# tum-vision/tandem

Hardware: AMD Instinct MI355X
Metric: depth-maps/sec @ 640×480×7-view×3-stage; TSDF voxels integrated/sec (higher is better)
Workload: dtype f32; 1 GPU; 640x480 ref+6-src keyframe window, 3-stage cascade (48/32/8 hypotheses), view aggregation, fp32; independent windows, 4 in flight per GPU (one DrMvsnet engine each) x 1 GPU replica(s); trained weights recovered from the reference's exported tandem_512x320 model (same architecture), inputs resident in HBM; height=480, width=640, views=7, parallelism=replicas x1, 4 engines per GPU

## Files before the change

include/dr_mi355x.h:

```cpp
#ifndef DR_MI355X_H
#define DR_MI355X_H

#include <stddef.h>
#include <stdint.h>

#ifdef __cplusplus
extern "C" {
#endif

enum {
  DR_OK = 0,
  DR_ERR_ARG = 1,
  DR_ERR_PROTOCOL = 2,
  DR_ERR_DEVICE = 3,
  DR_ERR_IO = 4,
  DR_ERR_CAPACITY = 5,
  DR_ERR_UNSUPPORTED = 6
};

const char *dr_last_error(void);
const char *dr_version(void);

typedef struct drm_s drm_t;

int drm_create(const char *weights_path, int device, drm_t **out);
void drm_destroy(drm_t *h);
int drm_call_async(drm_t *h, int height, int width, int view_num, int ref_index,
                   const uint8_t *const *bgrs, const float *K9, const float *const *c2ws,
                   float depth_min, float depth_max, float discard_percentage);
int drm_ready(drm_t *h);
int drm_wait(drm_t *h);
int drm_get_result(drm_t *h, float *depth, float *confidence, float *depth_dense, float *confidence_dense);
int drm_get_result_view(drm_t *h, const float **depth, const float **confidence, const float **depth_dense, const float **confidence_dense);
void *drm_host_alloc(size_t bytes);
void drm_host_free(void *p);

int drm_set_feature_cache(drm_t *h, int capacity);
int drm_feature_cache_stats(drm_t *h, uint64_t out[6]);

int drm_upload(drm_t *h, int height, int width, int view_num, int ref_index, const uint8_t *const *bgrs,
               const float *K9, const float *const *c2ws, float depth_min, float depth_max,
               float discard_percentage);
int drm_forward(drm_t *h, int iters, float *ms_total);
int drm_autotune(drm_t *h, int max_candidates, float *before_ms, float *after_ms);
int drm_set_view_shard(drm_t *h, int nsrc_total);
int drm_forward_phase(drm_t *h, int phase);
int drm_comm_available(void);
int drm_comm_unique_id(uint8_t id[128]);
int drm_comm_init(drm_t *h, int rank, int world, const uint8_t id[128]);
int drm_comm_destroy(drm_t *h);
int drm_comm_count(drm_t *h, int *nranks);
int drm_device_tensor(drm_t *h, const char *name, void **dptr, size_t *nfloats);
int drm_download(drm_t *h, float *depth, float *confidence, float *depth_dense, float *confidence_dense);
int drm_get_stage_output(drm_t *h, int stage, float *depth, float *confidence);
int drm_get_tensor(drm_t *h, const char *name, float *out, size_t n_max, size_t *n, int dims[4]);
int drm_profile(drm_t *h, char *names, size_t names_cap, float *ms, int cap, int *count);
int drm_work(drm_t *h, double *flops, double *bytes);

int drm_debug_conv(int device, const float *in, int D, int H, int W, int Cin, const float *weight, int Cout,
                   int kd, int kh, int kw, int sd, int sh, int sw, int transposed, const float *scale,
                   const float *bias, int relu, const float *add, int add_up2, float *out, int out_dims[3]);

int drm_debug_tail(int device, const float *x, const float *skip, const float *w_deconv, const float *scale8, const float *bias8, const float *w_prob, int D,
                   int h, int w, int qy, int zchunk, int form, float *out);

typedef struct {
  float voxel_size;
  int num_buckets;
  int bucket_size;
  int num_blocks;
  int block_size;
  int max_sdf_weight;
  float truncation_distance;
  float max_sensor_depth;
  float min_sensor_depth;
  int num_render_streams;
  float fx, fy, cx, cy;
  int height, width;
} drf_options_t;

typedef struct drf_s drf_t;

int drf_create(const drf_options_t *opt, int device, drf_t **out);
void drf_destroy(drf_t *h);
int drf_integrate_scan_async(drf_t *h, const uint8_t *bgr, const float *depth, const float *pose16);
int drf_render_async(drf_t *h, const float *const *poses16, int n);
int drf_get_render_result(drf_t *h, uint8_t **bgr, float **depth, int n);
int drf_extract_mesh_async(drf_t *h, const float lower[3], const float upper[3]);
int drf_get_mesh_sync(drf_t *h, size_t num_max, size_t *num, float *vert, float *cols);
int drf_mesh_num_triangles(drf_t *h, size_t *ntri);
int drf_save_mesh(drf_t *h, const char *filename, const float lower[3], const float upper[3]);
int drf_get_render_device(drf_t *h, int stream, const uint8_t **d_bgr, const float **d_depth);
int drf_synchronize(drf_t *h);

int drf_stats(drf_t *h, uint64_t out[4]);
int drf_visited_blocks(drf_t *h, uint64_t *total);
int drf_export_blocks(drf_t *h, int max_blocks, int32_t *coords, uint8_t *voxels, int *n);
int drf_fast_div_status(drf_t *h, int *enabled, uint64_t *mismatches);
int drf_test_combine(drf_t *h, size_t n, const uint8_t *a, const uint8_t *b, int max_weight, uint8_t *out);
int drf_integrate_device(drf_t *h, const void *d_bgr, const void *d_depth, const float *pose16);
int dr_device_alloc(int device, size_t bytes, void **dptr);
int dr_device_free(void *dptr);
int dr_memcpy_h2d(void *dptr, const void *src, size_t bytes);
int dr_memcpy_d2h(void *dst, const void *dptr, size_t bytes);
int dr_memcpy_d2d(void *dst, const void *src, size_t bytes);
int drf_bench_integrate(drf_t *h, const void *d_bgr, const void *d_depth, const float *poses16, int nscans,
                        float *ms, float *kernel_ms);

int drf_bench_sequence(drf_t *h, const void *d_bgr, const void *d_depth, const float *poses16, int nframes, int render, float ms[6]);
int drf_bench_render_host(drf_t *h, int stream, int back, const uint8_t **bgr, const float **depth);

int drf_streaming_min_radius(const drf_options_t *o, float *radius);
int drf_set_streaming(drf_t *h, float radius, size_t host_capacity_blocks);
int drf_stream_out_region(drf_t *h, const float lower[3], const float upper[3]);
int drf_stream_in_region(drf_t *h, const float lower[3], const float upper[3]);
int drf_streaming_stats(drf_t *h, uint64_t out[6]);
int drf_export_host_blocks(drf_t *h, int max_blocks, int32_t *coords, uint8_t *voxels, int *n);
enum { DRF_MESH_RESIDENT = 0, DRF_MESH_MAP = 1 };
int drf_set_mesh_scope(drf_t *h, int scope);
enum { DRF_RENDER_RESIDENT = 0, DRF_RENDER_MAP = 1 };
int drf_set_render_scope(drf_t *h, int scope, size_t stage_capacity_blocks);
int drf_render_stats(drf_t *h, uint64_t out[4]);
int drf_mesh_stats(drf_t *h, uint64_t out[3]);

int drf_map_info(const char *path, float *voxel_size, uint64_t *n_blocks);
int drf_save_map(drf_t *h, const char *path, size_t chunk_blocks);
int drf_load_map(drf_t *h, const char *path, size_t chunk_blocks);

#define DRF_MESH_UPDATE_MAX_SCANS 16
int drf_extract_mesh_update_async(drf_t *h, const float lower[3], const float upper[3]);
int drf_mesh_update_size(drf_t *h, size_t *nblk, size_t *ntri, int *full);
int drf_get_mesh_update_sync(drf_t *h, size_t max_blocks, size_t num_max, size_t *nblk, int32_t *coords, uint64_t *first, size_t *num,
                             float *vert, float *cols, int *full);
int drf_mesh_update_reset(drf_t *h);
int drf_mesh_update_stats(drf_t *h, uint64_t out[4]);

typedef struct drt_s drt_t;
int drt_create(int w, int h, float setting_huberTH, float setting_coarseCutoffTH, int device, drt_t **out);
void drt_destroy(drt_t *t);
int drt_set_k(drt_t *t, int w, int h, float fx, float fy, float cx, float cy);
int drt_init(drt_t *t, int n_max);
int drt_set_reference(drt_t *t, int n, const float *pc_u, const float *pc_v, const float *pc_idepth, const float *pc_color,
                      float ref_exposure, const double ref_aff_g2l[2]);
int drt_set_new(drt_t *t, const float *dInew);
int drt_calc_res(drt_t *t, const double refToNew[16], float new_exposure, const double aff_g2l[2], float cutoffTH, double out6[6],
                 double sums7[7]);
int drt_calc_g(drt_t *t, double H_out[64], double b_out[8], float new_exposure, const double aff_g2l[2], double raw45[45]);
int drt_append_dense_reference(drt_t *t, const float *depth, const float KRKi[9], const float Kt[3], int step, int dense_only,
                               const float *idepth0, const float *dIp0, int on_device, int *n_out);
int drt_synchronize(drt_t *t);
int drt_start_timing(drt_t *t);
int drt_end_timing_ms(drt_t *t, float *ms);
int drt_get_points(drt_t *t, float *pc_u, float *pc_v, float *pc_idepth, float *pc_color, int cap, int *n);
int drt_get_warped(drt_t *t, int which, float *out, int cap);
int drt_get_zbuffer(drt_t *t, float *out);

#ifdef __cplusplus
}
#endif
#endif
```

tandem_amd/_lib.py:

```python
import ctypes as C
import os

_HERE = os.path.dirname(os.path.abspath(__file__))
LIB_PATH = os.environ.get("DR_MI355X_LIB") or os.path.join(_HERE, "libdr_mi355x.so")

DR_OK = 0
ERR_NAMES = {1: "DR_ERR_ARG", 2: "DR_ERR_PROTOCOL", 3: "DR_ERR_DEVICE", 4: "DR_ERR_IO", 5: "DR_ERR_CAPACITY",
             6: "DR_ERR_UNSUPPORTED"}


class DrError(RuntimeError):
    def __init__(self, code, msg):
        super().__init__("%s: %s" % (ERR_NAMES.get(code, code), msg))
        self.code = code


class FusionOptions(C.Structure):
    _fields_ = [("voxel_size", C.c_float), ("num_buckets", C.c_int), ("bucket_size", C.c_int),
                ("num_blocks", C.c_int), ("block_size", C.c_int), ("max_sdf_weight", C.c_int),
                ("truncation_distance", C.c_float), ("max_sensor_depth", C.c_float),
                ("min_sensor_depth", C.c_float), ("num_render_streams", C.c_int),
                ("fx", C.c_float), ("fy", C.c_float), ("cx", C.c_float), ("cy", C.c_float),
                ("height", C.c_int), ("width", C.c_int)]


_lib = None
u8p, f32p, vp = C.POINTER(C.c_uint8), C.POINTER(C.c_float), C.c_void_p
f64p = C.POINTER(C.c_double)

SIGNATURES = {
    "dr_last_error": (C.c_char_p, []),
    "dr_version": (C.c_char_p, []),
    "drm_create": (C.c_int, [C.c_char_p, C.c_int, C.POINTER(vp)]),
    "drm_destroy": (None, [vp]),
    "drm_call_async": (C.c_int, [vp, C.c_int, C.c_int, C.c_int, C.c_int, C.POINTER(u8p), f32p, C.POINTER(f32p),
                                 C.c_float, C.c_float, C.c_float]),
    "drm_ready": (C.c_int, [vp]),
    "drm_wait": (C.c_int, [vp]),
    "drm_get_result": (C.c_int, [vp, f32p, f32p, f32p, f32p]),
    "drm_get_result_view": (C.c_int, [vp, C.POINTER(f32p), C.POINTER(f32p), C.POINTER(f32p), C.POINTER(f32p)]),
    "drm_host_alloc": (vp, [C.c_size_t]),
    "drm_host_free": (None, [vp]),
    "drm_upload": (C.c_int, [vp, C.c_int, C.c_int, C.c_int, C.c_int, C.POINTER(u8p), f32p, C.POINTER(f32p),
                             C.c_float, C.c_float, C.c_float]),
    "drm_forward": (C.c_int, [vp, C.c_int, f32p]),
    "drm_download": (C.c_int, [vp, f32p, f32p, f32p, f32p]),
    "drm_get_stage_output": (C.c_int, [vp, C.c_int, f32p, f32p]),
    "drm_get_tensor": (C.c_int, [vp, C.c_char_p, f32p, C.c_size_t, C.POINTER(C.c_size_t), C.POINTER(C.c_int)]),
    "drm_profile": (C.c_int, [vp, C.c_char_p, C.c_size_t, f32p, C.c_int, C.POINTER(C.c_int)]),
    "drm_work": (C.c_int, [vp, C.POINTER(C.c_double), C.POINTER(C.c_double)]),
    "drm_debug_conv": (C.c_int, [C.c_int, f32p, C.c_int, C.c_int, C.c_int, C.c_int, f32p, C.c_int, C.c_int, C.c_int,
                                 C.c_int, C.c_int, C.c_int, C.c_int, C.c_int, f32p, f32p, C.c_int, f32p, C.c_int,
                                 f32p, C.POINTER(C.c_int)]),
    "drm_debug_tail": (C.c_int, [C.c_int, f32p, f32p, f32p, f32p, f32p, f32p, C.c_int, C.c_int, C.c_int, C.c_int, C.c_int, C.c_int, f32p]),
    "drm_autotune": (C.c_int, [vp, C.c_int, C.POINTER(C.c_float), C.POINTER(C.c_float)]),
    "drm_set_view_shard": (C.c_int, [vp, C.c_int]),
    "drm_forward_phase": (C.c_int, [vp, C.c_int]),
    "drm_comm_available": (C.c_int, []),
    "drm_comm_unique_id": (C.c_int, [u8p]),
    "drm_comm_init": (C.c_int, [vp, C.c_int, C.c_int, u8p]),
    "drm_comm_destroy": (C.c_int, [vp]),
    "drm_comm_count": (C.c_int, [vp, C.POINTER(C.c_int)]),
    "drm_device_tensor": (C.c_int, [vp, C.c_char_p, C.POINTER(vp), C.POINTER(C.c_size_t)]),
    "drf_create": (C.c_int, [C.POINTER(FusionOptions), C.c_int, C.POINTER(vp)]),
    "drf_destroy": (None, [vp]),
    "drf_integrate_scan_async": (C.c_int, [vp, u8p, f32p, f32p]),
    "drf_render_async": (C.c_int, [vp, C.POINTER(f32p), C.c_int]),
    "drf_get_render_result": (C.c_int, [vp, C.POINTER(u8p), C.POINTER(f32p), C.c_int]),
    "drf_extract_mesh_async": (C.c_int, [vp, f32p, f32p]),
    "drf_get_mesh_sync": (C.c_int, [vp, C.c_size_t, C.POINTER(C.c_size_t), f32p, f32p]),
    "drf_mesh_num_triangles": (C.c_int, [vp, C.POINTER(C.c_size_t)]),
    "drf_save_mesh": (C.c_int, [vp, C.c_char_p, f32p, f32p]),
    "drf_get_render_device": (C.c_int, [vp, C.c_int, C.POINTER(vp), C.POINTER(vp)]),
    "drf_synchronize": (C.c_int, [vp]),
    "drf_stats": (C.c_int, [vp, C.POINTER(C.c_uint64)]),
    "drf_export_blocks": (C.c_int, [vp, C.c_int, C.POINTER(C.c_int32), u8p, C.POINTER(C.c_int)]),
    "drf_fast_div_status": (C.c_int, [vp, C.POINTER(C.c_int), C.POINTER(C.c_uint64)]),
    "drf_test_combine": (C.c_int, [vp, C.c_size_t, u8p, u8p, C.c_int, u8p]),
    "drf_integrate_device": (C.c_int, [vp, vp, vp, f32p]),
    "drt_create": (C.c_int, [C.c_int, C.c_int, C.c_float, C.c_float, C.c_int, C.POINTER(vp)]),
    "drt_destroy": (None, [vp]),
    "drt_set_k": (C.c_int, [vp, C.c_int, C.c_int, C.c_float, C.c_float, C.c_float, C.c_float]),
    "drt_init": (C.c_int, [vp, C.c_int]),
    "drt_set_reference": (C.c_int, [vp, C.c_int, f32p, f32p, f32p, f32p, C.c_float, f64p]),
    "drt_set_new": (C.c_int, [vp, f32p]),
    "drt_calc_res": (C.c_int, [vp, f64p, C.c_float, f64p, C.c_float, f64p, f64p]),
    "drt_calc_g": (C.c_int, [vp, f64p, f64p, C.c_float, f64p, f64p]),
    "drt_append_dense_reference": (C.c_int, [vp, vp, f32p, f32p, C.c_int, C.c_int, vp, vp, C.c_int, C.POINTER(C.c_int)]),
    "drt_synchronize": (C.c_int, [vp]),
    "drt_start_timing": (C.c_int, [vp]),
    "drt_end_timing_ms": (C.c_int, [vp, C.POINTER(C.c_float)]),
    "drt_get_points": (C.c_int, [vp, f32p, f32p, f32p, f32p, C.c_int, C.POINTER(C.c_int)]),
    "drt_get_warped": (C.c_int, [vp, C.c_int, f32p, C.c_int]),
    "drt_get_zbuffer": (C.c_int, [vp, f32p]),
    "dr_device_alloc": (C.c_int, [C.c_int, C.c_size_t, C.POINTER(vp)]),
    "dr_device_free": (C.c_int, [vp]),
    "dr_memcpy_d2d": (C.c_int, [vp, vp, C.c_size_t]),
    "dr_memcpy_h2d": (C.c_int, [vp, vp, C.c_size_t]),
    "dr_memcpy_d2h": (C.c_int, [vp, vp, C.c_size_t]),
    "drm_set_feature_cache": (C.c_int, [vp, C.c_int]),
    "drm_feature_cache_stats": (C.c_int, [vp, C.POINTER(C.c_uint64)]),
    "drf_bench_sequence": (C.c_int, [vp, vp, vp, f32p, C.c_int, C.c_int, f32p]),
    "drf_visited_blocks": (C.c_int, [vp, C.POINTER(C.c_uint64)]),
    "drf_bench_render_host": (C.c_int, [vp, C.c_int, C.c_int, C.POINTER(vp), C.POINTER(vp)]),
    "drf_bench_integrate": (C.c_int, [vp, vp, vp, f32p, C.c_int, f32p, f32p]),
    "drf_streaming_min_radius": (C.c_int, [C.POINTER(FusionOptions), f32p]),
    "drf_set_streaming": (C.c_int, [vp, C.c_float, C.c_size_t]),
    "drf_stream_out_region": (C.c_int, [vp, f32p, f32p]),
    "drf_stream_in_region": (C.c_int, [vp, f32p, f32p]),
    "drf_streaming_stats": (C.c_int, [vp, C.POINTER(C.c_uint64)]),
    "drf_export_host_blocks": (C.c_int, [vp, C.c_int, C.POINTER(C.c_int32), u8p, C.POINTER(C.c_int)]),
    "drf_set_render_scope": (C.c_int, [vp, C.c_int, C.c_size_t]),
    "drf_render_stats": (C.c_int, [vp, C.POINTER(C.c_uint64)]),
    "drf_set_mesh_scope": (C.c_int, [vp, C.c_int]),
    "drf_mesh_stats": (C.c_int, [vp, C.POINTER(C.c_uint64)]),
    "drf_extract_mesh_update_async": (C.c_int, [vp, f32p, f32p]),
    "drf_mesh_update_size": (C.c_int, [vp, C.POINTER(C.c_size_t), C.POINTER(C.c_size_t), C.POINTER(C.c_int)]),
    "drf_get_mesh_update_sync": (C.c_int, [vp, C.c_size_t, C.c_size_t, C.POINTER(C.c_size_t), C.POINTER(C.c_int32), C.POINTER(C.c_uint64),
                                           C.POINTER(C.c_size_t), f32p, f32p, C.POINTER(C.c_int)]),
    "drf_mesh_update_reset": (C.c_int, [vp]),
    "drf_mesh_update_stats": (C.c_int, [vp, C.POINTER(C.c_uint64)]),
    "drf_map_info": (C.c_int, [C.c_char_p, f32p, C.POINTER(C.c_uint64)]),
    "drf_save_map": (C.c_int, [vp, C.c_char_p, C.c_size_t]),
    "drf_load_map": (C.c_int, [vp, C.c_char_p, C.c_size_t]),
}


HOOKS_LIB_PATH = os.path.join(_HERE, "libdr_mi355x_hooks.so")
_loaded = {}


def switch(path=None):
    global _lib, LIB_PATH
    LIB_PATH = path or os.environ.get("DR_MI355X_LIB") or os.path.join(_HERE, "libdr_mi355x.so")
    _lib = _loaded.get(LIB_PATH)


def lib():
    global _lib
    if _lib is None:
        if not os.path.isfile(LIB_PATH):
            raise ImportError("tandem_amd: %s not built -- run `python -c 'import __graft_entry__ as g; g.build()'` "
                              "(hipcc --offload-arch=gfx950). There is no CPU fallback." % LIB_PATH)
        L = C.CDLL(LIB_PATH, mode=C.RTLD_GLOBAL)
        for name, (res, args) in SIGNATURES.items():
            fn = getattr(L, name)
            fn.restype, fn.argtypes = res, args
        _lib = _loaded[LIB_PATH] = L
    return _lib


def check(code):
    if code != DR_OK:
        raise DrError(code, lib().dr_last_error().decode(errors="replace"))


def fptr(a):
    return a.ctypes.data_as(f32p)
```

tandem_amd/csrc/conv_mfma.h:

```cpp
#pragma once
#include <algorithm>
#include <atomic>
#include <functional>

#include "dr_common.h"

namespace dr {

typedef float floatx4 __attribute__((ext_vector_type(4)));

struct ConvClass {
  int NU;
  int tap_base;
  int w_base;
  int ooz, ooy, oox;
};

struct ConvArgs {
  const float *in;
  float *out;
  const float4 *wpk;
  const float *scale, *bias, *add;
  const int *tapoff;
  const ConvClass *cls;
  int inD, inH, inW, inC;
  int outD, outH, outW, outC;
  int nPD, nPH, nPW;
  int sz, sy, sx, pz, py, px;
  int omz, omy, omx;
  int TZ, TY, TXT, TZI, TYI, TXI;
  int npass, ctTot, rows_valid, relu, add_mode, addH, addW;
  int par_rows, par_map;
  unsigned magicX, magicY;
  int nuMax;
  int tilesD, tilesH, tilesW;
  const float *fz_x, *fz_w, *fz_b, *fz_coarse;
  int pass_stride;
  const float *zero16;
  int a_slots;
  int a_wbufs;
  int class_loop;
};

constexpr int kConvThreads = 256;
constexpr size_t kConvMaxLds = 160 * 1024;

template <int CT>
__device__ inline void conv_load_affine(const ConvArgs &a, int g, int ct0, float4 (&sc)[CT], float4 (&bi)[CT]) {
#pragma unroll
  for (int ct = 0; ct < CT; ++ct) {
    sc[ct] = *reinterpret_cast<const float4 *>(a.scale + (ct0 + ct) * 16 + 4 * g);
    bi[ct] = *reinterpret_cast<const float4 *>(a.bias + (ct0 + ct) * 16 + 4 * g);
  }
}
template <int CT, int PT, bool ADD = true>
__device__ inline void conv_epilogue(const ConvArgs &a, const ConvClass &cls, floatx4 (&acc)[CT][PT], const float4 (&scv)[CT], const float4 (&biv)[CT],
                                     int wave, int j, int g, int ct0, int pz0, int py0, int px0) {
#ifdef DR_EPILOGUE_PER_ENTRY
  constexpr int NE = CT * PT, GB = 1;
#else
  constexpr int NE = CT * PT, GB = NE < 4 ? NE : 4;
#endif
#pragma unroll
  for (int e0 = 0; e0 < NE; e0 += GB) {
    size_t obase[GB];
    float4 r[GB];
    bool ok[GB];
#pragma unroll
    for (int k = 0; k < GB; ++k) {
      const int e = e0 + k, pt = e / CT, ct = e - pt * CT;
      const int tau = wave * PT + pt;
      const int xt = tau % a.TXT, yt = (tau / a.TXT) % a.TY, zt = tau / (a.TXT * a.TY);
      const int qz = pz0 + zt, qy = py0 + yt, qx = px0 + xt * 16 + j;
      const int c0 = (ct0 + ct) * 16 + 4 * g;
      ok[k] = e < NE && qz < a.nPD && qy < a.nPH && qx < a.nPW && c0 < a.rows_valid;
      int oz = qz * a.omz + cls.ooz, oy = qy * a.omy + cls.ooy, ox = qx * a.omx + cls.oox, ch = c0;
      if (a.par_rows) {
        const int q = c0 / a.par_rows, bits = (a.par_map >> (3 * q)) & 7;
        ch = c0 - q * a.par_rows;
        oz += (bits >> 2) & 1; oy += (bits >> 1) & 1; ox += bits & 1;
      }
      obase[k] = (((size_t)oz * a.outH + oy) * a.outW + ox) * a.outC + ch;
      size_t abase = obase[k];
      if (a.add_mode == 2) abase = (((size_t)oz * a.addH + (oy >> 1)) * a.addW + (ox >> 1)) * a.outC + ch;
      r[k] = make_float4(0.f, 0.f, 0.f, 0.f);
      if (ADD && a.add_mode && ok[k]) r[k] = *reinterpret_cast<const float4 *>(a.add + abase);
    }
#pragma unroll
    for (int k = 0; k < GB; ++k) {
      const int e = e0 + k, pt = e / CT, ct = e - pt * CT;
      if (e >= NE || !ok[k]) continue;
      const float4 sc = scv[ct], bi = biv[ct];
      float4 v;
      v.x = acc[ct][pt][0] * sc.x + bi.x;
      v.y = acc[ct][pt][1] * sc.y + bi.y;
      v.z = acc[ct][pt][2] * sc.z + bi.z;
      v.w = acc[ct][pt][3] * sc.w + bi.w;
      if (a.relu) {
        v.x = fmaxf(v.x, 0.f); v.y = fmaxf(v.y, 0.f); v.z = fmaxf(v.z, 0.f); v.w = fmaxf(v.w, 0.f);
      }
      if (ADD && a.add_mode) { v.x += r[k].x; v.y += r[k].y; v.z += r[k].z; v.w += r[k].w; }
      *reinterpret_cast<float4 *>(a.out + obase[k]) = v;
    }
  }
}

template <int CT, int PT>
__device__ inline void conv_chunk_mfma(const float4 (&av)[CT], const float4 (&bv)[PT], floatx4 (&acc)[CT][PT]) {
#pragma unroll
  for (int ct = 0; ct < CT; ++ct)
#pragma unroll
    for (int pt = 0; pt < PT; ++pt) acc[ct][pt] = __builtin_amdgcn_mfma_f32_16x16x4f32(av[ct].x, bv[pt].x, acc[ct][pt], 0, 0, 0);
#pragma unroll
  for (int ct = 0; ct < CT; ++ct)
#pragma unroll
    for (int pt = 0; pt < PT; ++pt) acc[ct][pt] = __builtin_amdgcn_mfma_f32_16x16x4f32(av[ct].y, bv[pt].y, acc[ct][pt], 0, 0, 0);
#pragma unroll
  for (int ct = 0; ct < CT; ++ct)
#pragma unroll
    for (int pt = 0; pt < PT; ++pt) acc[ct][pt] = __builtin_amdgcn_mfma_f32_16x16x4f32(av[ct].z, bv[pt].z, acc[ct][pt], 0, 0, 0);
#pragma unroll
  for (int ct = 0; ct < CT; ++ct)
#pragma unroll
    for (int pt = 0; pt < PT; ++pt) acc[ct][pt] = __builtin_amdgcn_mfma_f32_16x16x4f32(av[ct].w, bv[pt].w, acc[ct][pt], 0, 0, 0);
}
template <int CT, int PT>
__device__ inline void conv_chunk_load(const float *lds, const float4 *wp, int toff, int u, const int (&base)[PT], float4 (&av)[CT],
                                       float4 (&bv)[PT]) {
#pragma unroll
  for (int ct = 0; ct < CT; ++ct) av[ct] = wp[(u * CT + ct) * 64];
#pragma unroll
  for (int pt = 0; pt < PT; ++pt) bv[pt] = *reinterpret_cast<const float4 *>(lds + base[pt] + toff);
}
template <int CT, int PT>
__device__ inline void conv_chunk_anchor(const float4 (&av)[CT], const float4 (&bv)[PT], int toff) {
#pragma unroll
  for (int ct = 0; ct < CT; ++ct) asm volatile("" ::"v"(av[ct].x), "v"(av[ct].y), "v"(av[ct].z), "v"(av[ct].w));
#pragma unroll
  for (int pt = 0; pt < PT; ++pt) asm volatile("" ::"v"(bv[pt].x), "v"(bv[pt].y), "v"(bv[pt].z), "v"(bv[pt].w));
  asm volatile("" ::"v"(toff));
}
template <int CT, int PT>
__device__ inline void conv_kloop(const float *lds, const float4 *wl, const int *tp, int TPC, int NU, int lane, const int (&base)[PT],
                                  floatx4 (&acc)[CT][PT]) {
  const float4 *wp = wl + lane;
  float4 a0[CT], b0[PT], a1[CT], b1[PT];
  int tA = tp[0], tB = tp[min(1, NU - 1) * TPC];
  conv_chunk_load<CT, PT>(lds, wp, tA, 0, base, a0, b0);
  int u = 0;
  for (; u + 1 < NU; u += 2) {
    conv_chunk_load<CT, PT>(lds, wp, tB, u + 1, base, a1, b1);
    tA = tp[min(u + 2, NU - 1) * TPC];
    __builtin_amdgcn_sched_barrier(0);
    conv_chunk_mfma<CT, PT>(a0, b0, acc);
    __builtin_amdgcn_sched_barrier(0);
    conv_chunk_anchor<CT, PT>(a1, b1, tA);
    conv_chunk_load<CT, PT>(lds, wp, tA, min(u + 2, NU - 1), base, a0, b0);
    tB = tp[min(u + 3, NU - 1) * TPC];
    __builtin_amdgcn_sched_barrier(0);
    conv_chunk_mfma<CT, PT>(a1, b1, acc);
    __builtin_amdgcn_sched_barrier(0);
    conv_chunk_anchor<CT, PT>(a0, b0, tB);
  }
  if (u < NU) conv_chunk_mfma<CT, PT>(a0, b0, acc);
}

template <int CT, int PT>
__device__ inline void conv_chunk_mfma2(const float4 (&av)[CT], const float4 (&bv)[PT], floatx4 (&acc)[CT][PT], floatx4 (&acc2)[CT][PT]) {
  if constexpr (CT * PT == 1) {
    acc[0][0] = __builtin_amdgcn_mfma_f32_16x16x4f32(av[0].x, bv[0].x, acc[0][0], 0, 0, 0);
    acc2[0][0] = __builtin_amdgcn_mfma_f32_16x16x4f32(av[0].y, bv[0].y, acc2[0][0], 0, 0, 0);
    acc[0][0] = __builtin_amdgcn_mfma_f32_16x16x4f32(av[0].z, bv[0].z, acc[0][0], 0, 0, 0);
    acc2[0][0] = __builtin_amdgcn_mfma_f32_16x16x4f32(av[0].w, bv[0].w, acc2[0][0], 0, 0, 0);
  } else conv_chunk_mfma<CT, PT>(av, bv, acc);
}
template <int CT, int PT, class Load>
__device__ inline void conv_kloop_narrow(const int *tp, int TPC, int NU, floatx4 (&acc)[CT][PT], Load load) {
  float4 a0[CT], b0[PT], a1[CT], b1[PT], a2[CT], b2[PT];
  floatx4 acc2[CT][PT];
#pragma unroll
  for (int ct = 0; ct < CT; ++ct)
#pragma unroll
    for (int pt = 0; pt < PT; ++pt) acc2[ct][pt] = floatx4{0.f, 0.f, 0.f, 0.f};
  auto tap = [&](int u) { return tp[min(u, NU - 1) * TPC]; };
  int t0 = tap(0), t1 = tap(1), t2 = tap(2);
  load(t0, 0, a0, b0);
  load(t1, min(1, NU - 1), a1, b1);
  int u = 0;
  for (; u + 2 < NU; u += 3) {
    load(t2, u + 2, a2, b2);
    t0 = tap(u + 3);
    __builtin_amdgcn_sched_barrier(0);
    conv_chunk_mfma2<CT, PT>(a0, b0, acc, acc2);
    __builtin_amdgcn_sched_barrier(0);
// ... 391 lines not shown
    conv_a_load<CI, CT, PT>(tile, wp, tB, u + 1, c4, bpos, a1, b1);
    tA = tp[min(u + 2, NU - 1) * TPC];
    __builtin_amdgcn_sched_barrier(0);
    conv_chunk_mfma<CT, PT>(a0, b0, acc);
    __builtin_amdgcn_sched_barrier(0);
    conv_chunk_anchor<CT, PT>(a1, b1, tA);
    conv_a_load<CI, CT, PT>(tile, wp, tA, min(u + 2, NU - 1), c4, bpos, a0, b0);
    tB = tp[min(u + 3, NU - 1) * TPC];
    __builtin_amdgcn_sched_barrier(0);
    conv_chunk_mfma<CT, PT>(a1, b1, acc);
    __builtin_amdgcn_sched_barrier(0);
    conv_chunk_anchor<CT, PT>(a0, b0, tB);
  }
  if (u < NU) conv_chunk_mfma<CT, PT>(a0, b0, acc);
}

template <int CI, int CT, int PT>
__global__ __launch_bounds__(kConvAThreads) void k_conv_a(const ConvArgs a) {
  extern __shared__ float4 lds4[];
  constexpr int TPC = 16 / CI;
  const int tid = threadIdx.x, lane = tid & 63, wave = __builtin_amdgcn_readfirstlane(tid >> 6), j = lane & 15, g = lane >> 4;
  const ConvClass cls = a.cls[0];
  const int ct0 = blockIdx.z * CT;
  const int NP = a.TZI * a.TYI * a.TXI, NU = cls.NU, n_w = NU * CT * 64;

  float4 *tile0 = lds4, *tile1 = lds4 + a.a_slots;
  float4 *wb0 = lds4 + 2 * (size_t)a.a_slots;
  int *tapl = reinterpret_cast<int *>(wb0 + (size_t)a.a_wbufs * n_w);
  for (int i = tid; i < NU * TPC; i += kConvAThreads) tapl[i] = a.tapoff[cls.tap_base + i];
  const int *tp = tapl + (4 * g) / CI;
  const int c4 = ((4 * g) % CI) / 4;

  int bpos[PT];
#pragma unroll
  for (int pt = 0; pt < PT; ++pt) {
    const int tau = wave * PT + pt;
    const int xt = tau % a.TXT, yt = (tau / a.TXT) % a.TY, zt = tau / (a.TXT * a.TY);
    bpos[pt] = ((zt * a.sz) * a.TYI + yt * a.sy) * a.TXI + (xt * 16 + j) * a.sx;
  }

  const int ntiles = a.tilesD * a.tilesH * a.tilesW, per_xcd = (ntiles + 7) >> 3;
  const int xcd = blockIdx.x & 7, wi = blockIdx.x >> 3, nw = gridDim.x >> 3;
  const int t_lo = xcd * per_xcd, t_hi = min(ntiles, t_lo + per_xcd);
  const int my_tiles = t_lo + wi < t_hi ? (t_hi - t_lo - wi + nw - 1) / nw : 0;
  const int n_units = my_tiles * a.npass;
  auto tile_origin = [&](int k, int &pz0, int &py0, int &px0) {
    int b = t_lo + wi + k * nw;
    const int tw = b % a.tilesW;
    b /= a.tilesW;
    pz0 = (b / a.tilesH) * a.TZ; py0 = (b % a.tilesH) * a.TY; px0 = tw * a.TXT * 16;
  };
  auto issue = [&](int unit) {
    const int k = unit / a.npass, p = unit - k * a.npass;
    int pz0, py0, px0;
    tile_origin(k, pz0, py0, px0);
    conv_a_issue<CI, CT>(a, (unit & 1) ? tile1 : tile0, wb0 + (size_t)(p % a.a_wbufs) * n_w, unit < a.npass || a.npass > a.a_wbufs, NP, NU, p, ct0, cls.w_base,
                         pz0 * a.sz - a.pz, py0 * a.sy - a.py, px0 * a.sx - a.px, wave, lane);
  };

  floatx4 acc[CT][PT];
#pragma unroll
  for (int ct = 0; ct < CT; ++ct)
#pragma unroll
    for (int pt = 0; pt < PT; ++pt) acc[ct][pt] = floatx4{0.f, 0.f, 0.f, 0.f};

  float4 scv[CT], biv[CT];
  conv_load_affine<CT>(a, g, ct0, scv, biv);
  if (n_units > 0) issue(0);
  int done_tile = -1;
  for (int i = 0; i < n_units; ++i) {
    conv_a_wait_dma();
    __syncthreads();
#ifndef DR_ABL_NO_STAGE
#ifndef DR_CONV_A_ISSUE_LATE
    const bool early = a.add_mode == 0;
#else
    const bool early = false;
#endif
    if (early && i + 1 < n_units) issue(i + 1);
#endif
#ifdef DR_ABL_NO_EPI
    if (done_tile >= 0 && a.npass < 0) {
#else
    if (done_tile >= 0) {
#endif
      int pz0, py0, px0;
      tile_origin(done_tile, pz0, py0, px0);
      if (a.add_mode) conv_epilogue<CT, PT, true>(a, cls, acc, scv, biv, wave, j, g, ct0, pz0, py0, px0);
      else conv_epilogue<CT, PT, false>(a, cls, acc, scv, biv, wave, j, g, ct0, pz0, py0, px0);
#pragma unroll
      for (int ct = 0; ct < CT; ++ct)
#pragma unroll
        for (int pt = 0; pt < PT; ++pt) acc[ct][pt] = floatx4{0.f, 0.f, 0.f, 0.f};
      done_tile = -1;
    }
#ifndef DR_ABL_NO_STAGE
    if (!early && i + 1 < n_units) issue(i + 1);
#endif
#ifndef DR_ABL_NO_KLOOP
#ifdef DR_NO_NARROW_KLOOP
    if constexpr (false) {
#else
    if constexpr (CT * PT <= 2) {
#endif
      const float4 *tile = (i & 1) ? tile1 : tile0, *wp = wb0 + (size_t)((i % a.npass) % a.a_wbufs) * n_w + lane;
      conv_kloop_narrow<CT, PT>(tp, TPC, NU, acc, [&](int toff, int u, float4 (&av)[CT], float4 (&bv)[PT]) { conv_a_load<CI, CT, PT>(tile, wp, toff, u, c4, bpos, av, bv); });
    } else conv_a_kloop<CI, CT, PT>((i & 1) ? tile1 : tile0, wb0 + (size_t)((i % a.npass) % a.a_wbufs) * n_w, tp, TPC, NU, lane, c4, bpos, acc);
#endif
    if ((i + 1) % a.npass == 0) done_tile = i / a.npass;
  }
  if (done_tile >= 0) {
    int pz0, py0, px0;
    tile_origin(done_tile, pz0, py0, px0);
    conv_epilogue<CT, PT>(a, cls, acc, scv, biv, wave, j, g, ct0, pz0, py0, px0);
  }
}

}
#include "conv_wino.h"
namespace dr {
template <int CI> __host__ __device__ inline int conv_a_unit(int pos, int c4);
}
#include "conv_march.h"
namespace dr {


enum ConvMode { CONV_NORMAL = 0, CONV_XPAIR = 1, CONV_X8 = 2 };

struct ConvLayer {
  int Cin = 0, Cout = 0;
  int kd = 1, kh = 1, kw = 1;
  int sd = 1, sh = 1, sw = 1;
  bool transposed = false;
  int up2 = 0;
  const float *weight = nullptr;
  std::vector<float> scale, bias;
  bool relu = false;
  int out_pad = 0;
};

struct ConvFuse {
  const float *x, *w, *b, *coarse;
  int cin;
};

struct ConvLaunch {
  ConvArgs args;
  int ci, ct, pt, fz = 0;
  int async = 0;
  MarchArgs march{};
  int nup = 0;
  int ncw = 8;
  int bf3 = 0;
  dim3 grid;
  size_t lds_bytes;
  double flops;
};

struct DimTaps {
  std::vector<int> t, off;
  int s = 1, p = 0, om = 1, oo = 0, npos = 0;
  int par = -1;
};

inline int parity_kernel_index(int parity, int off) {
  if (parity == 0) return off == 0 ? 1 : -1;
  return off == 0 ? 2 : 0;
}
inline std::vector<DimTaps> axis_classes_up2(int in_size, bool split) {
  std::vector<DimTaps> r;
  if (!split) { DimTaps d; d.t = {0, 1, 2}; d.off = {0, 1, 2}; d.p = 1; d.om = 2; d.npos = in_size; r.push_back(d); return r; }
  DimTaps e; e.t = {0, 1}; e.off = {0, 1}; e.p = 1; e.om = 2; e.oo = 0; e.npos = in_size; e.par = 0; r.push_back(e);
  DimTaps o; o.t = {1, 2}; o.off = {1, 2}; o.p = 1; o.om = 2; o.oo = 1; o.npos = in_size; o.par = 1; r.push_back(o);
  return r;
}
inline int up2_kernel_set(int parity, int off, int (&k)[2]) {
  if (parity == 0) { if (off == 0) { k[0] = 0; return 1; } if (off == 1) { k[0] = 1; k[1] = 2; return 2; } return 0; }
  if (off == 1) { k[0] = 0; k[1] = 1; return 2; }
  if (off == 2) { k[0] = 2; return 1; }
  return 0;
}
inline void prune_taps(DimTaps &d, int in_size) {
  std::vector<int> t, off;
  for (size_t i = 0; i < d.t.size(); ++i) {
    bool used = false;
    for (int pos = 0; pos < d.npos && !used; ++pos) { const int x = pos * d.s - d.p + d.off[i]; used = x >= 0 && x < in_size; }
    if (used) { t.push_back(d.t[i]); off.push_back(d.off[i]); }
  }
  if (t.empty() || t.size() == d.t.size()) return;
  const int mo = *std::min_element(off.begin(), off.end());
  for (int &o : off) o -= mo;
  d.p -= mo;
  d.t = t; d.off = off;
}
inline std::vector<DimTaps> axis_classes_unpruned(int k, int s, bool transposed, int in_size, bool split);
inline std::vector<DimTaps> axis_classes(int k, int s, bool transposed, int in_size, bool split = false, bool prune = false) {
  std::vector<DimTaps> r = axis_classes_unpruned(k, s, transposed, in_size, split);
  if (prune && !hook_env("DR_CONV_NO_TAP_PRUNE"))
    for (DimTaps &d : r) prune_taps(d, in_size);
  return r;
}
inline std::vector<DimTaps> axis_classes_unpruned(int k, int s, bool transposed, int in_size, bool split) {
  std::vector<DimTaps> r;
  if (!transposed) {
    DimTaps d;
    for (int t = 0; t < k; ++t) { d.t.push_back(t); d.off.push_back(t); }
    d.s = s; d.p = k / 2; d.npos = (in_size + 2 * (k / 2) - k) / s + 1;
    r.push_back(d);
  } else if (k == 1) {
    DimTaps d; d.t = {0}; d.off = {0}; d.npos = in_size; r.push_back(d);
  } else if (s == 1) {
    DimTaps d;
    for (int t = 0; t < k; ++t) { d.t.push_back(t); d.off.push_back(2 - t); }
    d.p = 1; d.npos = in_size;
    r.push_back(d);
  } else if (!split) {
    DimTaps d; d.t = {0, 1}; d.off = {0, 1}; d.om = 2; d.oo = 0; d.npos = in_size; r.push_back(d);
  } else {
    DimTaps e; e.t = {0}; e.off = {0}; e.om = 2; e.oo = 0; e.npos = in_size; e.par = 0; r.push_back(e);
    DimTaps o; o.t = {0, 1}; o.off = {0, 1}; o.om = 2; o.oo = 1; o.npos = in_size; o.par = 1; r.push_back(o);
  }
  return r;
}

struct ConvPlanOut {
  std::vector<ConvLaunch> launches;
  int outD, outH, outW;
  int ncand = 0;
};

struct DeviceArena {
  std::vector<void *> ptrs;
  int *err_flag = nullptr;
  bool host_only = false;
  template <class T>
  T *upload(const std::vector<T> &h) {
    if (host_only) {
      T *d = static_cast<T *>(malloc(std::max<size_t>(h.size() * sizeof(T), 16)));
      memcpy(d, h.data(), h.size() * sizeof(T));
      ptrs.push_back(d);
      return d;
    }
    T *d = dalloc<T>(h.size());
    DR_HIP(hipMemcpy(d, h.data(), h.size() * sizeof(T), hipMemcpyHostToDevice));
    ptrs.push_back(d);
    return d;
  }
  ~DeviceArena() { for (void *p : ptrs) { if (host_only) free(p); else (void)hipFree(p); } }
};

struct ConvTuned {
  int Cin, Cout, kd, kh, kw, sd, sh, sw, transposed, mode, inD, inH, inW;
  int ci, ct, pt, tz, ty, txt;
  int async_;
};
#include "conv_tuned.h"

inline bool conv_instance_exists(int ci, int ct) {
  return (ci == 4 && ct == 1) || ((ci == 8 || ci == 16) && (ct == 1 || ct == 2 || ct == 4));
}
inline bool conv_a_instance_exists(int ci, int ct, int pt) {
  return (pt == 1 || pt == 2 || pt == 4) && ((ci == 4 && ct == 1 && pt != 1) || ((ci == 8 || ci == 16) && (ct == 1 || ct == 2)));
}
#define DR_MARCH_INSTANCES(X)                                                                                         \
  X(8, 6, 1, 2, 8) X(8, 6, 1, 4, 8) X(8, 6, 1, 1, 12) X(8, 6, 1, 2, 12)                                               \
  X(16, 12, 1, 2, 8) X(16, 12, 1, 4, 8) X(16, 12, 1, 1, 12) X(16, 12, 1, 2, 12)                                       \
  X(16, 9, 1, 2, 8) X(16, 9, 1, 4, 8) X(16, 9, 1, 1, 12) X(16, 9, 1, 2, 12) X(16, 9, 2, 2, 8)                         \
  X(8, 2, 1, 1, 8) X(8, 2, 1, 2, 8) X(8, 2, 1, 4, 8) X(8, 2, 1, 1, 10) X(8, 2, 1, 2, 10)                              \
  X(16, 4, 1, 1, 8) X(16, 4, 1, 2, 8) X(16, 4, 1, 4, 8) X(16, 4, 1, 1, 10) X(16, 4, 1, 2, 10)                         \
  X(16, 3, 1, 1, 8) X(16, 3, 1, 2, 8) X(16, 3, 1, 4, 8) X(16, 3, 1, 1, 10) X(16, 3, 1, 2, 10)                         \
  X(16, 3, 2, 1, 8) X(16, 3, 2, 2, 8) X(16, 3, 2, 1, 10) X(16, 3, 2, 2, 10)
#define DR_MARCH_W_INSTANCES(X) X(8, 6, 1, 1, 8) X(16, 12, 1, 1, 8) X(16, 9, 1, 1, 8)
inline bool conv_m_instance_exists(int ci, int nup, int ct, int pt, int ncw, bool wino = false) {
#define DR_X(CI_, NUP_, CT_, PT_, NCW_) if (ci == CI_ && nup == NUP_ && ct == CT_ && pt == PT_ && ncw == NCW_) return true;
  if (wino) { DR_MARCH_W_INSTANCES(DR_X) return false; }
  DR_MARCH_INSTANCES(DR_X)
#undef DR_X
  return false;
}
inline int conv_march_policy() {
  if (const char *e = getenv("DR_CONV_MARCH")) return atoi(e);
  return 1;
}
inline int conv_rowmarch_policy() {
  if (const char *e = getenv("DR_CONV_ROWMARCH")) return atoi(e);
  return 1;
}
struct MarchShape {
  int nup, npi, npo, ns, tyi, txi, np, ps, r, ncw;
  size_t wbytes, lds_bytes;
  long long steps;
  int grid;
  bool ok;
};
inline MarchShape march_shape(int KZ, int ntp, int Cin, int ci, int ct, int pt, int ty, int txt, int SX, int exy, int exx, int nPD, int nPH, int nPW, int CTtot,
                              bool rm = false, bool wino = false) {
  MarchShape m{};
  const int tpc = 16 / ci;
  if (Cin % ci || ntp % tpc || CTtot % ct || (ty * txt) % pt || (rm && (ty != 1 || KZ != 1)) || (wino && (KZ != 3 || rm || (ntp / 3) % tpc))) return m;
  m.ncw = ty * txt / pt;
  m.nup = ntp / tpc;
  if (!conv_m_instance_exists(ci, m.nup, ct, pt, m.ncw, wino)) return m;
  const int npass = Cin / ci, kz = rm ? 3 : KZ;
  if (npass > 2) return m;
  m.npi = KZ == 1 ? npass : 1; m.npo = KZ == 1 ? 1 : npass; m.ns = kz * m.npi;
  m.tyi = rm ? 1 : (wino ? 2 * ty + 2 : ty - 1 + exy); m.txi = (txt * 16 - 1) * SX + exx; m.np = m.tyi * m.txi;
// ... 401 lines not shown
          if (kx >= 0 && kx < L.kw) v = weight_at(co, cin, tz[tap], ky >= 0 ? ky : ty[tap], kx);
        }
      }
      return v;
    };
    pk.resize(w0 + (size_t)npass * NU * CTtot * 64 * 4 * (bf3 ? 2 : 1), 0.f);
    if (bf3) {
      unsigned short *pb = reinterpret_cast<unsigned short *>(pk.data() + w0);
      for (int p = 0; p < npass; ++p) for (int u = 0; u < NU; ++u) for (int ct = 0; ct < CTtot; ++ct)
        for (int l = 0; l < 64; ++l) for (int s = 0; s < 8; ++s) {
          const int g = l >> 4, i = l & 15, k32 = 8 * g + s;
          const float v = weight_of(u * TPC + k32 / CI, p * CI + k32 % CI, ct * 16 + i);
          const unsigned short hi = bf16_rne(v), lo = bf16_rne(v - bf16_value(hi));
          const size_t frag = (((size_t)p * NU + u) * CTtot + ct) * 2;
          pb[((frag + 0) * 64 + l) * 8 + s] = hi;
          pb[((frag + 1) * 64 + l) * 8 + s] = lo;
        }
    } else if (wino_raw) {
      for (int p = 0; p < npass; ++p) for (int u = 0; u < NR; ++u) for (int k = 0; k < 3; ++k) for (int ct = 0; ct < CTtot; ++ct)
        for (int l = 0; l < 64; ++l) for (int s = 0; s < 4; ++s) {
          const int g = l >> 4, i = l & 15, k16 = 4 * g + s;
          pk[w0 + ((((size_t)p * NU + u * 3 + k) * CTtot + ct) * 64 + l) * 4 + s] = (k == 1 ? 0.5f : 1.f) * weight_of(u * TPC + k16 / CI, p * CI + k16 % CI, ct * 16 + i, k);
        }
    } else if (wino) {
      for (int p = 0; p < npass; ++p) for (int u = 0; u < NR; ++u) for (int pp = 0; pp < 4; ++pp) for (int ct = 0; ct < CTtot; ++ct)
        for (int l = 0; l < 64; ++l) for (int s = 0; s < 4; ++s) {
          const int g = l >> 4, i = l & 15, k16 = 4 * g + s;
          double v = 0;
          for (int ky = 0; ky < 3; ++ky) v += conv_wino_g(pp, ky) * (double)weight_of(u * TPC + k16 / CI, p * CI + k16 % CI, ct * 16 + i, ky);
          pk[w0 + ((((size_t)p * NU + u * 4 + pp) * CTtot + ct) * 64 + l) * 4 + s] = (float)v;
        }
    } else
    for (int p = 0; p < npass; ++p) for (int u = 0; u < NU; ++u) for (int ct = 0; ct < CTtot; ++ct)
      for (int l = 0; l < 64; ++l) for (int s = 0; s < 4; ++s) {
        const int g = l >> 4, i = l & 15, k16 = 4 * g + s;
        pk[w0 + ((((size_t)p * NU + u) * CTtot + ct) * 64 + l) * 4 + s] = weight_of(u * TPC + k16 / CI, p * CI + k16 % CI, ct * 16 + i);
      }
    if (L.up2) flops += ic == 0 ? 2.0 * nPD * nPH * nPW * 16.0 * L.Cin * L.Cout : 0.0;
    else if (L.transposed) flops += ic == 0 ? 2.0 * nPD * nPH * nPW * (double)L.kd * L.kh * L.kw * L.Cin * L.Cout : 0.0;
    else flops += 2.0 * nPD * (wino ? 2 * nPH : nPH) * nPW * (mode == CONV_NORMAL ? 1 : shifts) * (double)ntz * (wino ? 3 : nty) * (mode == CONV_NORMAL ? ntx : L.kw) * L.Cin * L.Cout;
  }

  ConvLaunch cl{};
  ConvArgs &a = cl.args;
  a.in = in; a.out = out; a.wpk = reinterpret_cast<const float4 *>(arena.upload(pk));
  a.scale = arena.upload(sc); a.bias = arena.upload(bi); a.add = add; a.tapoff = arena.upload(tapoff);
  a.cls = arena.upload(cls);
  a.inD = inD; a.inH = inH; a.inW = inW; a.inC = in_split ? in_split : inC;
  a.pass_stride = in_split ? (int)((size_t)inD * inH * inW * in_split) : CI;
  if (in_split && (size_t)inD * inH * inW * in_split >= (1ull << 31)) fail(DR_ERR_ARG, "plan_conv: split input too large");
  a.outD = R.outD; a.outH = R.outH + 2 * L.out_pad; a.outW = outWv; a.outC = outCv;
  if (L.out_pad) {
    if ((2 * L.out_pad) % shifts) fail(DR_ERR_ARG, "plan_conv: an output border of %d pixels does not fit the %d-wide output groups", L.out_pad, shifts);
    a.outW = outWv + 2 * L.out_pad / shifts;
  }
  a.nPD = nPD; a.nPH = nPH; a.nPW = nPW;
  a.sz = SZ; a.sy = SY; a.sx = SX; a.pz = PZ; a.py = PY; a.px = PX;
  a.omz = cz[0].om; a.omy = cy[0].om; a.omx = cx[0].om;
  a.par_rows = parity_layer ? L.Cout : 0; a.par_map = par_map;
  a.TZ = TZ; a.TY = TY; a.TXT = TXT; a.TZI = TZI; a.TYI = TYI; a.TXI = TXI;
  a.magicX = TXI == 1 ? 0u : (unsigned)((0x100000000ull + TXI - 1) / TXI);
  a.magicY = TYI == 1 ? 0u : (unsigned)((0x100000000ull + TYI - 1) / TYI);
  if ((size_t)TZI * TYI * TXI >= 65536) fail(DR_ERR_ARG, "plan_conv: halo tile too large");
  a.npass = npass; a.ctTot = CTtot; a.rows_valid = rows_valid; a.relu = L.relu ? 1 : 0;
  a.add_mode = add ? add_mode : 0;
  a.addH = R.outH / 2; a.addW = (mode == CONV_NORMAL ? R.outW : outWv) / 2;
  a.tilesD = cdiv(nPD, TZ); a.tilesH = cdiv(nPH, TY); a.tilesW = cdiv(nPW, TXT * 16);
  cl.ci = CI; cl.ct = CT; cl.pt = PT;
  a.fz_x = a.fz_w = a.fz_b = a.fz_coarse = nullptr;
  if (fz) {
    if (fz->cin != 8 || L.transposed || SZ != 1 || SY != 1) fail(DR_ERR_ARG, "plan_conv: fused skip needs an 8-channel source and a stride-1 layer");
    a.fz_x = fz->x; a.fz_w = fz->w; a.fz_b = fz->b; a.fz_coarse = fz->coarse; cl.fz = fz->cin;
  }
  cl.grid = dim3(8 * cdiv(a.tilesD * a.tilesH * a.tilesW, 8), ncls, CTtot / CT);
  int nu_max = 0;
  for (auto &c : cls) nu_max = std::max(nu_max, c.NU);
  a.nuMax = nu_max;
  cl.lds_bytes = (size_t)TZI * TYI * TXI * CIS * 4 + (size_t)nu_max * CT * (bf3 ? 2048 : 1024) + (size_t)nu_max * TPC * 4 + 64;
  cl.bf3 = bf3 ? 1 : 0;
  a.zero16 = nullptr; a.a_slots = 0; a.a_wbufs = 1; a.class_loop = 0;
  if (ASYNC == 0 && !bf3 && !fz && ncls > 1 && npass == 1 && conv_c_instance_exists(CI, CT, PT) && !hook_env("DR_CONV_NO_CLASS_LOOP")) {
    const size_t with_loop = cl.lds_bytes + (size_t)nu_max * CT * 1024 + (size_t)(ncls - 1) * nu_max * TPC * 4;
    if (with_loop <= kConvMaxLds) {
      a.class_loop = ncls;
      cl.lds_bytes = with_loop;
      cl.grid.y = 1;
    }
  }
  if (ASYNC == 0 && !bf3 && !fz && PT == 1 && CT <= 2 && npass >= 2 && (size_t)TZI * TYI * TXI * (CI / 4) <= 6 * kConvThreads && !hook_env("DR_CONV_NO_PIPE") &&
      cl.lds_bytes + (size_t)nu_max * CT * 1024 <= kConvMaxLds) {
    a.a_wbufs = 2;
    cl.lds_bytes += (size_t)nu_max * CT * 1024;
  }
  if (ASYNC == 4) cl.async = 4;
  if (ASYNC == 1) {
    cl.async = 1;
    a.zero16 = arena.upload(std::vector<float>(4, 0.f));
    a.a_slots = (int)conv_a_slots(TZI * TYI * TXI, CI);
    a.a_wbufs = npass;
    cl.lds_bytes = 2 * (size_t)a.a_slots * 16 + (size_t)a.a_wbufs * nu_max * CT * 1024 + (size_t)nu_max * TPC * 4 + 64;
    if (cl.lds_bytes > kConvMaxLds) {
      a.a_wbufs = std::min(npass, 2);
      cl.lds_bytes = 2 * (size_t)a.a_slots * 16 + (size_t)a.a_wbufs * nu_max * CT * 1024 + (size_t)nu_max * TPC * 4 + 64;
    }
    const int ntiles = a.tilesD * a.tilesH * a.tilesW, split = CTtot / CT;
    const int wpc = cl.lds_bytes * 2 <= kConvMaxLds ? 2 : 1;
    const int want = std::max(1, std::min(ntiles, 256 * wpc / split));
    cl.grid = dim3(8 * cdiv(want, 8), 1, split);
  }
  if (ASYNC == 2 || ASYNC == 3 || ASYNC == 5) {
    const bool rm = ASYNC == 3;
    const MarchShape ms = rm ? march_shape(L.kd, row_ntp, L.Cin, CI, CT, PT, 1, TXT, SX, exy, exx, nPD, nPH, nPW, CTtot, true)
                             : march_shape(L.kd, march_ntp, L.Cin, CI, CT, PT, TY, TXT, SX, exy, exx, nPD, nPH, nPW, CTtot, false, wino_raw);
    if (!ms.ok) fail(DR_ERR_ARG, "plan_conv: inconsistent k_conv_m plan");
    cl.async = 2; cl.nup = ms.nup; cl.ncw = ms.ncw;
    a.zero16 = arena.upload(std::vector<float>(4, 0.f));
    a.a_slots = 0; a.a_wbufs = 0;
    MarchArgs &m = cl.march;
    const int kz = rm ? 3 : L.kd;
    std::vector<int> tap2d((size_t)ms.nup * TPC, 0);
    {
      const DimTaps &Y = *classes[0].y, &X = *classes[0].x;
      int n = 0;
      if (rm) for (size_t ix = 0; ix < X.t.size(); ++ix, ++n) tap2d[n] = X.off[ix];
      else for (size_t iy = 0; iy < Y.t.size(); ++iy) for (size_t ix = 0; ix < X.t.size(); ++ix, ++n) tap2d[n] = Y.off[iy] * TXI + X.off[ix];
    }
    m.tap2d = arena.upload(tap2d);
    m.geo.KZ = kz; m.geo.NPI = ms.npi; m.geo.Dc = rm ? nPH : (L.kd == 3 ? nPD : 1);
    m.NPO = ms.npo;
    m.colsH = rm ? 1 : cdiv(nPH, TY); m.colsW = cdiv(nPW, TXT * 16);
    m.ncols = (L.kd == 3 ? 1 : nPD) * m.colsH * m.colsW;
    m.R = ms.r; m.PS = ms.ps; m.NP = ms.np; m.nit = ms.ps / 128;
    m.wsec = ms.nup * CT * 64; m.NU = kz * ms.nup;
    m.steps = (int)ms.steps;
    m.ncw = ms.ncw;
    m.rm = rm ? 1 : 0;
    m.wino = wino_raw ? 1 : 0;
    const long long iplane = (long long)a.inH * a.inW * a.inC, oplane = (long long)a.outH * a.outW * a.outC;
    if (iplane * std::max(1, a.inD) >= (1ll << 31) || oplane * std::max(1, a.outD) >= (1ll << 31)) fail(DR_ERR_ARG, "plan_conv: tensor too large for k_conv_m's 32-bit strides");
    m.i_sv = L.kd == 3 ? 0 : (int)iplane; m.i_sz = rm ? a.inW * a.inC : (L.kd == 3 ? (int)iplane : 0); m.i_sy = rm ? 0 : a.inW * a.inC;
    m.o_sv = L.kd == 3 ? 0 : (int)oplane; m.o_sz = rm ? a.outW * a.outC : (L.kd == 3 ? (int)oplane : 0); m.o_sy = rm ? 0 : a.outW * a.outC;
    m.inHp = rm ? 1 : a.inH;
    m.err = arena.err_flag;
    m.depth = rm ? 3 : 2;
    if (const char *e = hook_env("DR_MARCH_PDEPTH")) m.depth = std::max(1, std::min(4, atoi(e)));
    cl.lds_bytes = ms.lds_bytes;
    cl.grid = dim3(ms.grid, 1, CTtot / CT);
  }
  cl.flops = flops;
  R.launches.push_back(cl);
  return R;
}

inline void conv_allow_big_lds(const void *fn, std::atomic<unsigned long long> &done, size_t lds_bytes) {
  if (lds_bytes <= 64 * 1024) return;
  int dev = 0;
  DR_HIP(hipGetDevice(&dev));
  const unsigned long long bit = 1ull << (dev & 63);
  if (done.load(std::memory_order_acquire) & bit) return;
  DR_HIP(hipFuncSetAttribute(fn, hipFuncAttributeMaxDynamicSharedMemorySize, (int)kConvMaxLds));
  done.fetch_or(bit, std::memory_order_release);
}
template <int CI, int CT, int PT, int FZ = 0>
inline void launch_conv_inst(const ConvLaunch &c, hipStream_t st) {
  static std::atomic<unsigned long long> done{0};
  conv_allow_big_lds(reinterpret_cast<const void *>(&k_conv<CI, CT, PT, FZ>), done, c.lds_bytes);
  hipLaunchKernelGGL((k_conv<CI, CT, PT, FZ>), c.grid, dim3(kConvThreads), c.lds_bytes, st, c.args);
}
#ifdef DR_PARITY_HOOKS
template <int CI, int CT, int PT>
inline void launch_conv_b_inst(const ConvLaunch &c, hipStream_t st) {
  static std::atomic<unsigned long long> done{0};
  conv_allow_big_lds(reinterpret_cast<const void *>(&k_conv_b<CI, CT, PT>), done, c.lds_bytes);
  hipLaunchKernelGGL((k_conv_b<CI, CT, PT>), c.grid, dim3(kConvThreads), c.lds_bytes, st, c.args);
}
#endif
template <int CI, int CT, int PT>
inline void launch_conv_c_inst(const ConvLaunch &c, hipStream_t st) {
  static std::atomic<unsigned long long> done{0};
  conv_allow_big_lds(reinterpret_cast<const void *>(&k_conv_c<CI, CT, PT>), done, c.lds_bytes);
  hipLaunchKernelGGL((k_conv_c<CI, CT, PT>), c.grid, dim3(kConvThreads), c.lds_bytes, st, c.args);
}
template <int CI, int CT, int PT>
inline void launch_conv_a_inst(const ConvLaunch &c, hipStream_t st) {
  static std::atomic<unsigned long long> done{0};
  conv_allow_big_lds(reinterpret_cast<const void *>(&k_conv_a<CI, CT, PT>), done, c.lds_bytes);
  hipLaunchKernelGGL((k_conv_a<CI, CT, PT>), c.grid, dim3(kConvAThreads), c.lds_bytes, st, c.args);
}
template <int CI, int CT, int PT>
inline void launch_conv_w_inst(const ConvLaunch &c, hipStream_t st) {
  static std::atomic<unsigned long long> done{0};
  conv_allow_big_lds(reinterpret_cast<const void *>(&k_conv_w<CI, CT, PT>), done, c.lds_bytes);
  hipLaunchKernelGGL((k_conv_w<CI, CT, PT>), c.grid, dim3(kConvThreads), c.lds_bytes, st, c.args);
}
template <int CI, int NUP, int CT, int PT, int FZ = 0, int NCW = 8, int W = 0>
inline void launch_conv_m_inst(const ConvLaunch &c, hipStream_t st) {
  static std::atomic<unsigned long long> done{0};
  conv_allow_big_lds(reinterpret_cast<const void *>(&k_conv_m<CI, NUP, CT, PT, FZ, NCW, W>), done, c.lds_bytes);
  hipLaunchKernelGGL((k_conv_m<CI, NUP, CT, PT, FZ, NCW, W>), c.grid, dim3(64 * (NCW + (FZ ? kMarchFzProducers : kMarchProducers))), c.lds_bytes, st, c.args, c.march);
}
inline void launch_conv(const ConvLaunch &c, hipStream_t st) {
#ifndef DR_PARITY_HOOKS
  if (c.bf3) fail(DR_ERR_UNSUPPORTED, "launch_conv: the bf16 x 3 kernel is built with -DDR_PARITY_HOOKS only");
#else
  if (c.bf3) {
#define DR_CONV_B_CASE(CI_, CT_)                                                \
  if (c.ci == CI_ && c.ct == CT_ && !c.async && !c.fz) {                        \
    if (c.pt == 4) launch_conv_b_inst<CI_, CT_, 4>(c, st);                      \
    else launch_conv_b_inst<CI_, CT_, 1>(c, st);                                \
    return;                                                                     \
  }
    DR_CONV_B_CASE(8, 1)
    DR_CONV_B_CASE(8, 2)
    DR_CONV_B_CASE(8, 4)
    DR_CONV_B_CASE(16, 1)
    DR_CONV_B_CASE(16, 2)
    DR_CONV_B_CASE(16, 4)
#undef DR_CONV_B_CASE
    fail(DR_ERR_ARG, "launch_conv: no bf16x3 instance CI=%d CT=%d", c.ci, c.ct);
  }
#endif
#ifndef DR_PARITY_HOOKS
  if (c.fz) fail(DR_ERR_UNSUPPORTED, "launch_conv: fused-skip kernels are built with -DDR_PARITY_HOOKS only");
#else
  if (c.async == 2 && c.fz) {
    if (c.fz != 8 || c.ci != 16 || c.nup != 12 || c.ct != 1 || c.ncw != 8) fail(DR_ERR_ARG, "launch_conv: no fused-skip marching instance FZ=%d CI=%d NUP=%d CT=%d", c.fz, c.ci, c.nup, c.ct);
    if (c.pt == 4) launch_conv_m_inst<16, 12, 1, 4, 8>(c, st);
    else launch_conv_m_inst<16, 12, 1, 2, 8>(c, st);
    return;
  }
#endif
  if (c.async == 2 && c.march.wino) {
#define DR_X(CI_, NUP_, CT_, PT_, NCW_) \
  if (c.ci == CI_ && c.nup == NUP_ && c.ct == CT_ && c.pt == PT_ && c.ncw == NCW_) { launch_conv_m_inst<CI_, NUP_, CT_, PT_, 0, NCW_, 1>(c, st); return; }
    DR_MARCH_W_INSTANCES(DR_X)
#undef DR_X
    fail(DR_ERR_ARG, "launch_conv: no Winograd marching instance CI=%d NUP=%d CT=%d PT=%d waves=%d", c.ci, c.nup, c.ct, c.pt, c.ncw);
  }
  if (c.async == 2) {
#define DR_X(CI_, NUP_, CT_, PT_, NCW_) \
  if (c.ci == CI_ && c.nup == NUP_ && c.ct == CT_ && c.pt == PT_ && c.ncw == NCW_) { launch_conv_m_inst<CI_, NUP_, CT_, PT_, 0, NCW_>(c, st); return; }
    DR_MARCH_INSTANCES(DR_X)
#undef DR_X
    fail(DR_ERR_ARG, "launch_conv: no marching instance CI=%d NUP=%d CT=%d PT=%d waves=%d", c.ci, c.nup, c.ct, c.pt, c.ncw);
  }
  if (c.async == 4) {
#define DR_CONV_W_CASE(CI_, CT_, PT_) if (c.ci == CI_ && c.ct == CT_ && c.pt == PT_) { launch_conv_w_inst<CI_, CT_, PT_>(c, st); return; }
    DR_CONV_W_CASE(16, 1, 1) DR_CONV_W_CASE(16, 1, 2) DR_CONV_W_CASE(16, 2, 1) DR_CONV_W_CASE(16, 2, 2)
    DR_CONV_W_CASE(8, 1, 1) DR_CONV_W_CASE(8, 1, 2)
#undef DR_CONV_W_CASE
    fail(DR_ERR_ARG, "launch_conv: no Winograd instance CI=%d CT=%d PT=%d", c.ci, c.ct, c.pt);
  }
  if (c.async) {
#define DR_CONV_A_CASE(CI_, CT_)                                                \
  if (c.ci == CI_ && c.ct == CT_) {                                             \
    if (c.pt == 4) launch_conv_a_inst<CI_, CT_, 4>(c, st);                      \
    else if (c.pt == 2) launch_conv_a_inst<CI_, CT_, 2>(c, st);                 \
    else launch_conv_a_inst<CI_, CT_, 1>(c, st);                                \
    return;                                                                     \
  }
    if (c.ci == 4 && c.ct == 1 && c.pt == 1) fail(DR_ERR_ARG, "launch_conv: no async instance CI=4 PT=1");
    DR_CONV_A_CASE(4, 1)
    DR_CONV_A_CASE(8, 1)
    DR_CONV_A_CASE(8, 2)
    DR_CONV_A_CASE(16, 1)
    DR_CONV_A_CASE(16, 2)
#undef DR_CONV_A_CASE
    fail(DR_ERR_ARG, "launch_conv: no async instance CI=%d CT=%d PT=%d", c.ci, c.ct, c.pt);
  }
#ifdef DR_PARITY_HOOKS
  if (c.fz) {
    if (c.fz != 8 || c.ci != 16 || c.ct != 1) fail(DR_ERR_ARG, "launch_conv: no fused-skip instance FZ=%d CI=%d CT=%d", c.fz, c.ci, c.ct);
    if (c.pt == 4) launch_conv_inst<16, 1, 4, 8>(c, st);
    else launch_conv_inst<16, 1, 1, 8>(c, st);
    return;
  }
#endif
  if (c.args.class_loop > 0) {
#define DR_CONV_C_CASE(CI_, CT_)                                                \
  if (c.ci == CI_ && c.ct == CT_) {                                             \
    if (c.pt == 4) launch_conv_c_inst<CI_, CT_, 4>(c, st);                      \
    else launch_conv_c_inst<CI_, CT_, 1>(c, st);                                \
    return;                                                                     \
  }
    DR_CONV_C_CASE(8, 1)
    DR_CONV_C_CASE(8, 2)
    DR_CONV_C_CASE(16, 1)
    DR_CONV_C_CASE(16, 2)
#undef DR_CONV_C_CASE
    fail(DR_ERR_ARG, "launch_conv: no class-loop instance CI=%d CT=%d PT=%d", c.ci, c.ct, c.pt);
  }
#define DR_CONV_CASE(CI_, CT_)                                                  \
  if (c.ci == CI_ && c.ct == CT_) {                                             \
    if (c.pt == 4) launch_conv_inst<CI_, CT_, 4>(c, st);                        \
    else launch_conv_inst<CI_, CT_, 1>(c, st);                                  \
    return;                                                                     \
  }
  DR_CONV_CASE(4, 1)
  DR_CONV_CASE(8, 1)
  DR_CONV_CASE(8, 2)
  DR_CONV_CASE(8, 4)
  DR_CONV_CASE(16, 1)
  DR_CONV_CASE(16, 2)
  DR_CONV_CASE(16, 4)
#undef DR_CONV_CASE
  fail(DR_ERR_ARG, "launch_conv: no instance CI=%d CT=%d", c.ci, c.ct);
}

}
```

tandem_amd/csrc/conv_wino.h:

```cpp
#pragma once

namespace dr {

template <int CT, int PT>
__device__ inline void conv_w_load(const float *lds, const float4 *wp, int toff, int r, const int (&base)[PT], int rs, float4 (&av)[4][CT], float4 (&dv)[4][PT]) {
#pragma unroll
  for (int p = 0; p < 4; ++p)
#pragma unroll
    for (int ct = 0; ct < CT; ++ct) av[p][ct] = wp[((r * 4 + p) * CT + ct) * 64];
#pragma unroll
  for (int pt = 0; pt < PT; ++pt) {
    const float *b = lds + base[pt] + toff;
#pragma unroll
    for (int q = 0; q < 4; ++q) dv[q][pt] = *reinterpret_cast<const float4 *>(b + q * rs);
  }
}
template <int CT, int PT>
__device__ inline void conv_w_anchor(const float4 (&av)[4][CT], const float4 (&dv)[4][PT], int toff) {
#pragma unroll
  for (int p = 0; p < 4; ++p) {
#pragma unroll
    for (int ct = 0; ct < CT; ++ct) asm volatile("" ::"v"(av[p][ct].x), "v"(av[p][ct].y), "v"(av[p][ct].z), "v"(av[p][ct].w));
#pragma unroll
    for (int pt = 0; pt < PT; ++pt) asm volatile("" ::"v"(dv[p][pt].x), "v"(dv[p][pt].y), "v"(dv[p][pt].z), "v"(dv[p][pt].w));
  }
  asm volatile("" ::"v"(toff));
}
template <int PT>
__device__ inline void conv_w_transform(float4 (&d)[4][PT]) {
#pragma unroll
  for (int pt = 0; pt < PT; ++pt) {
    const float4 d1 = d[1][pt], d2 = d[2][pt];
    d[0][pt] = make_float4(d[0][pt].x - d2.x, d[0][pt].y - d2.y, d[0][pt].z - d2.z, d[0][pt].w - d2.w);
    d[3][pt] = make_float4(d1.x - d[3][pt].x, d1.y - d[3][pt].y, d1.z - d[3][pt].z, d1.w - d[3][pt].w);
    d[1][pt] = make_float4(d1.x + d2.x, d1.y + d2.y, d1.z + d2.z, d1.w + d2.w);
    d[2][pt] = make_float4(d2.x - d1.x, d2.y - d1.y, d2.z - d1.z, d2.w - d1.w);
  }
}
template <int CT, int PT>
__device__ inline void conv_w_mfma(const float4 (&av)[4][CT], const float4 (&v)[4][PT], floatx4 (&acc)[4][CT][PT]) {
#define DR_W_STEP(S)                                                                                                        \
  _Pragma("unroll") for (int p = 0; p < 4; ++p) _Pragma("unroll") for (int ct = 0; ct < CT; ++ct) _Pragma("unroll") for (int pt = 0; pt < PT; ++pt) \
      acc[p][ct][pt] = __builtin_amdgcn_mfma_f32_16x16x4f32(av[p][ct].S, v[p][pt].S, acc[p][ct][pt], 0, 0, 0);
  DR_W_STEP(x) DR_W_STEP(y) DR_W_STEP(z) DR_W_STEP(w)
#undef DR_W_STEP
}
template <int CT, int PT>
__device__ inline void conv_w_kloop(const float *lds, const float4 *wl, const int *tp, int TPC, int NR, int lane, const int (&base)[PT], int rs,
                                    floatx4 (&acc)[4][CT][PT]) {
  const float4 *wp = wl + lane;
  float4 a0[4][CT], d0[4][PT], a1[4][CT], d1[4][PT];
  int tA = tp[0], tB = tp[min(1, NR - 1) * TPC];
  conv_w_load<CT, PT>(lds, wp, tA, 0, base, rs, a0, d0);
  int r = 0;
  for (; r + 1 < NR; r += 2) {
    conv_w_load<CT, PT>(lds, wp, tB, r + 1, base, rs, a1, d1);
    tA = tp[min(r + 2, NR - 1) * TPC];
    __builtin_amdgcn_sched_barrier(0);
    conv_w_transform<PT>(d0);
    conv_w_mfma<CT, PT>(a0, d0, acc);
    __builtin_amdgcn_sched_barrier(0);
    conv_w_anchor<CT, PT>(a1, d1, tA);
    conv_w_load<CT, PT>(lds, wp, tA, min(r + 2, NR - 1), base, rs, a0, d0);
    tB = tp[min(r + 3, NR - 1) * TPC];
    __builtin_amdgcn_sched_barrier(0);
    conv_w_transform<PT>(d1);
    conv_w_mfma<CT, PT>(a1, d1, acc);
    __builtin_amdgcn_sched_barrier(0);
    conv_w_anchor<CT, PT>(a0, d0, tB);
  }
  if (r < NR) {
    conv_w_transform<PT>(d0);
    conv_w_mfma<CT, PT>(a0, d0, acc);
  }
}

template <int CT, int PT>
__device__ inline void conv_w_epilogue(const ConvArgs &a, const ConvClass &cls, floatx4 (&acc)[4][CT][PT], const float4 (&scv)[CT], const float4 (&biv)[CT],
                                       int wave, int j, int g, int ct0, int pz0, int py0, int px0) {
#pragma unroll
  for (int pt = 0; pt < PT; ++pt) {
    const int tau = wave * PT + pt;
    const int xt = tau % a.TXT, yt = (tau / a.TXT) % a.TY, zt = tau / (a.TXT * a.TY);
    const int qz = pz0 + zt, qy = py0 + yt, qx = px0 + xt * 16 + j;
    if (qz >= a.nPD || qy >= a.nPH || qx >= a.nPW) continue;
#pragma unroll
    for (int ct = 0; ct < CT; ++ct) {
      const int c0 = (ct0 + ct) * 16 + 4 * g;
      if (c0 >= a.rows_valid) continue;
      const floatx4 m0 = acc[0][ct][pt], m1 = acc[1][ct][pt], m2 = acc[2][ct][pt], m3 = acc[3][ct][pt];
      const floatx4 o[2] = {(m0 + m1) + m2, (m1 - m2) - m3};
      const float4 sc = scv[ct], bi = biv[ct];
      const int oz = qz * a.omz + cls.ooz, ox = qx * a.omx + cls.oox;
      size_t obase[2];
      float4 ad[2];
#pragma unroll
      for (int r = 0; r < 2; ++r) {
        const int oy = qy * 2 + r;
        obase[r] = (((size_t)oz * a.outH + oy) * a.outW + ox) * a.outC + c0;
        size_t abase = obase[r];
        if (a.add_mode == 2) abase = (((size_t)oz * a.addH + (oy >> 1)) * a.addW + (ox >> 1)) * a.outC + c0;
        ad[r] = make_float4(0.f, 0.f, 0.f, 0.f);
        if (a.add_mode) ad[r] = *reinterpret_cast<const float4 *>(a.add + abase);
      }
#pragma unroll
      for (int r = 0; r < 2; ++r) {
        float4 v;
        v.x = o[r][0] * sc.x + bi.x;
        v.y = o[r][1] * sc.y + bi.y;
        v.z = o[r][2] * sc.z + bi.z;
        v.w = o[r][3] * sc.w + bi.w;
        if (a.relu) { v.x = fmaxf(v.x, 0.f); v.y = fmaxf(v.y, 0.f); v.z = fmaxf(v.z, 0.f); v.w = fmaxf(v.w, 0.f); }
        if (a.add_mode) { v.x += ad[r].x; v.y += ad[r].y; v.z += ad[r].z; v.w += ad[r].w; }
        *reinterpret_cast<float4 *>(a.out + obase[r]) = v;
      }
    }
  }
}

template <int CI, int CT, int PT>
__global__ __launch_bounds__(kConvThreads, (CT * PT == 1 ? 4 : (CT * PT == 2 ? 3 : 2))) void k_conv_w(const ConvArgs a) {
  extern __shared__ float4 lds4[];
  float *lds = reinterpret_cast<float *>(lds4);
  constexpr int CIS = CI + 4, TPC = 16 / CI, C4 = CI / 4;
  const int tid = threadIdx.x, lane = tid & 63, wave = tid >> 6, j = lane & 15, g = lane >> 4;
  const ConvClass cls = a.cls[0];
  const int ct0 = blockIdx.z * CT;
  const int ntiles = a.tilesD * a.tilesH * a.tilesW, per_xcd = (ntiles + 7) >> 3;
  int b = (int)(blockIdx.x & 7u) * per_xcd + (int)(blockIdx.x >> 3);
  if (b >= ntiles) return;
  const int tw = b % a.tilesW;
  b /= a.tilesW;
  const int th = b % a.tilesH, td = b / a.tilesH;
  const int pz0 = td * a.TZ, py0 = th * a.TY, px0 = tw * a.TXT * 16;
  const int iz0 = pz0 * a.sz - a.pz, iy0 = py0 * a.sy - a.py, ix0 = px0 * a.sx - a.px;
  const int rs = a.TXI * CIS;

  int base[PT];
#pragma unroll
  for (int pt = 0; pt < PT; ++pt) {
    const int tau = wave * PT + pt;
    const int xt = tau % a.TXT, yt = (tau / a.TXT) % a.TY, zt = tau / (a.TXT * a.TY);
    base[pt] = (((zt * a.sz) * a.TYI + yt * a.sy) * a.TXI + (xt * 16 + j) * a.sx) * CIS + (4 * g) % CI;
  }
  const int sub = (4 * g) / CI;

  floatx4 acc[4][CT][PT];
#pragma unroll
  for (int p = 0; p < 4; ++p)
#pragma unroll
    for (int ct = 0; ct < CT; ++ct)
#pragma unroll
      for (int pt = 0; pt < PT; ++pt) acc[p][ct][pt] = floatx4{0.f, 0.f, 0.f, 0.f};

  const int NP = a.TZI * a.TYI * a.TXI, NU = cls.NU, NR = NU >> 2;
  float4 *wl = lds4 + ((size_t)NP * CIS) / 4;
  int *tapl = reinterpret_cast<int *>(wl + (size_t)a.nuMax * CT * 64);
  for (int i = tid; i < NR * TPC; i += kConvThreads) tapl[i] = a.tapoff[cls.tap_base + i] * CIS;
  const int *tp = tapl + sub;
  const unsigned total = (unsigned)NP * C4;
  for (int p = 0; p < a.npass; ++p) {
    __builtin_amdgcn_s_setprio(2);
    const float4 *wsrc = a.wpk + cls.w_base + ((size_t)p * NU * a.ctTot + ct0) * 64;
    for (int e = wave; e < NU * CT; e += kConvThreads / 64) {
      const int u = e / CT, ct = e - u * CT;
      conv_a_dma16(wsrc + ((size_t)u * a.ctTot + ct) * 64 + lane, __builtin_amdgcn_readfirstlane(conv_a_lds_addr(wl + (size_t)e * 64)));
    }
    constexpr int kStageBatch = 12;
    for (unsigned e0 = 0; e0 < total; e0 += kConvThreads * kStageBatch) {
      float4 v[kStageBatch];
      int dst[kStageBatch];
#pragma unroll
      for (int k = 0; k < kStageBatch; ++k) {
        const unsigned e = e0 + k * kConvThreads + tid;
        const unsigned pos = e / C4, c4 = e - pos * C4;
        const unsigned t = a.magicX ? __umulhi(pos, a.magicX) : pos, x = pos - t * a.TXI;
        const unsigned z = a.magicY ? __umulhi(t, a.magicY) : t, y = t - z * a.TYI;
        const int gz = iz0 + (int)z, gy = iy0 + (int)y, gx = ix0 + (int)x;
        v[k] = make_float4(0.f, 0.f, 0.f, 0.f);
        dst[k] = e < total ? (int)(pos * CIS + c4 * 4) : -1;
        if (e < total && gz >= 0 && gz < a.inD && gy >= 0 && gy < a.inH && gx >= 0 && gx < a.inW)
          v[k] = *reinterpret_cast<const float4 *>(a.in + (((size_t)gz * a.inH + gy) * a.inW + gx) * a.inC + (size_t)p * a.pass_stride + c4 * 4);
      }
#pragma unroll
      for (int k = 0; k < kStageBatch; ++k)
        if (dst[k] >= 0) *reinterpret_cast<float4 *>(lds + dst[k]) = v[k];
    }
    conv_a_wait_dma();
    __builtin_amdgcn_s_setprio(0);
    __syncthreads();
    conv_w_kloop<CT, PT>(lds, wl, tp, TPC, NR, lane, base, rs, acc);
    __syncthreads();
  }
  float4 scv[CT], biv[CT];
  conv_load_affine<CT>(a, g, ct0, scv, biv);
  conv_w_epilogue<CT, PT>(a, cls, acc, scv, biv, wave, j, g, ct0, pz0, py0, px0);
}

}
```

tandem_amd/csrc/dr_mvsnet.hip:

```cpp
#include <cmath>
#include <atomic>
#include <condition_variable>
#include <functional>
#include <map>
#include <memory>
#include <mutex>
#include <thread>

#include <dlfcn.h>
#include <rccl/rccl.h>

#include "conv_mfma.h"
#include "mvs_kernels.h"
#ifdef DR_PARITY_HOOKS
#include "tail_kernels.h"
#endif
#include "fn_front.h"
#include "fn_head3.h"

namespace dr {

std::string &last_error_slot() {
  thread_local std::string s;
  return s;
}

struct HostTensor {
  std::vector<int> dims;
  std::vector<float> data;
};
struct Blob {
  int depth_num[3];
  float ratio[3];
  int view_aggregation, base;
  std::map<std::string, HostTensor> t;
  const HostTensor &at(const std::string &k) const {
    auto it = t.find(k);
    if (it == t.end()) fail(DR_ERR_IO, "weight blob: missing tensor %s", k.c_str());
    return it->second;
  }
};

static Blob load_blob(const char *path) {
  FILE *f = fopen(path, "rb");
  if (!f) fail(DR_ERR_IO, "cannot open weight blob %s", path);
  Blob b;
  char magic[8];
  auto rd = [&](void *p, size_t n) {
    if (fread(p, 1, n, f) != n) { fclose(f); fail(DR_ERR_IO, "weight blob %s truncated", path); }
  };
  rd(magic, 8);
  if (memcmp(magic, "TDMW0001", 8)) { fclose(f); fail(DR_ERR_IO, "%s is not a TDMW blob", path); }
  rd(b.depth_num, 12); rd(b.ratio, 12); rd(&b.view_aggregation, 4); rd(&b.base, 4);
  uint32_t n;
  rd(&n, 4);
  for (uint32_t i = 0; i < n; ++i) {
    uint32_t ln, nd;
    rd(&ln, 4);
    std::string name(ln, '\0');
    rd(&name[0], ln);
    rd(&nd, 4);
    HostTensor t;
    size_t cnt = 1;
    for (uint32_t k = 0; k < nd; ++k) { uint32_t d; rd(&d, 4); t.dims.push_back((int)d); cnt *= d; }
    t.data.resize(cnt);
    rd(t.data.data(), cnt * 4);
    b.t[name] = std::move(t);
  }
  fclose(f);
  if (b.base != 8) fail(DR_ERR_UNSUPPORTED, "only feature_net_base_channels=8 is supported (got %d)", b.base);
  return b;
}

static void inv4(const double *m, double *o) {
  double a[4][8];
  for (int i = 0; i < 4; ++i) for (int j = 0; j < 4; ++j) { a[i][j] = m[4 * i + j]; a[i][4 + j] = i == j; }
  for (int c = 0; c < 4; ++c) {
    int piv = c;
    for (int r = c + 1; r < 4; ++r) if (std::fabs(a[r][c]) > std::fabs(a[piv][c])) piv = r;
    if (piv != c) for (int j = 0; j < 8; ++j) std::swap(a[c][j], a[piv][j]);
    const double d = a[c][c];
    for (int j = 0; j < 8; ++j) a[c][j] /= d;
    for (int r = 0; r < 4; ++r) if (r != c) { const double f = a[r][c]; for (int j = 0; j < 8; ++j) a[r][j] -= f * a[c][j]; }
  }
  for (int i = 0; i < 4; ++i) for (int j = 0; j < 4; ++j) o[4 * i + j] = a[i][4 + j];
}
static void mul4(const double *a, const double *b, double *o) {
  for (int i = 0; i < 4; ++i) for (int j = 0; j < 4; ++j) { double s = 0; for (int k = 0; k < 4; ++k) s += a[4 * i + k] * b[4 * k + j]; o[4 * i + j] = s; }
}
static void world_to_pixel(const float *K9, const double *w2c, double *o) {
  for (int i = 0; i < 3; ++i) for (int j = 0; j < 4; ++j) { double s = 0; for (int k = 0; k < 3; ++k) s += (double)K9[3 * i + k] * w2c[4 * k + j]; o[4 * i + j] = s; }
  o[12] = w2c[12]; o[13] = w2c[13]; o[14] = w2c[14]; o[15] = w2c[15];
}

struct DevTensor {
  float *d = nullptr;
  int D = 0, H = 0, W = 0, C = 0;
  int pad = 0;
  int split = 0;
  size_t n() const { return (size_t)D * (H + 2 * pad) * (W + 2 * pad) * C; }
  float *interior() const { return d + ((size_t)pad * (W + 2 * pad) + pad) * C; }
};

struct Op {
  enum Kind { PREPROCESS, CONV, SKIPUP, PROB, COSTVOL, REGRESS, EDGE, HIST, SCAN, APPLY, BORDERFIX, TAIL, FRONT, HEAD3 } kind;
  const float *p0 = nullptr, *p1 = nullptr, *p3 = nullptr, *p4 = nullptr;
  float *p2 = nullptr;
  int d0 = 0, d1 = 0, d2 = 0;
  std::string name;
  ConvLaunch conv;
#ifdef DR_PARITY_HOOKS
  TailArgs tail{};
#endif
  FrontArgs front{};
  Head3Args head3{};
  std::function<ConvLaunch(int)> replan;
  std::string sig;
  int ncand = 0;
  int stage = 0, shift = 0, bits = 0;
  double flops = 0, bytes = 0;
};

struct Rccl {
  void *lib = nullptr;
  decltype(&ncclGetUniqueId) GetUniqueId = nullptr;
  decltype(&ncclCommInitRank) CommInitRank = nullptr;
  decltype(&ncclCommDestroy) CommDestroy = nullptr;
  decltype(&ncclAllReduce) AllReduce = nullptr;
  decltype(&ncclReduce) Reduce = nullptr;
  decltype(&ncclBroadcast) Broadcast = nullptr;
  decltype(&ncclGetErrorString) GetErrorString = nullptr;
  decltype(&ncclCommCount) CommCount = nullptr;
  static Rccl &get() {
    static Rccl r;
    static std::mutex m;
    std::lock_guard<std::mutex> g(m);
    if (!r.lib) {
      if (const char *e = getenv("DR_RCCL_LIB")) r.lib = dlopen(e, RTLD_NOW | RTLD_GLOBAL);
      else
      for (const char *n : {"librccl.so.1", "librccl.so", "/opt/rocm/lib/librccl.so.1"})
        if ((r.lib = dlopen(n, RTLD_NOW | RTLD_GLOBAL))) break;
      if (!r.lib) fail(DR_ERR_UNSUPPORTED, "RCCL not found (librccl.so.1): %s", dlerror());
      r.GetUniqueId = reinterpret_cast<decltype(r.GetUniqueId)>(dlsym(r.lib, "ncclGetUniqueId"));
      r.CommInitRank = reinterpret_cast<decltype(r.CommInitRank)>(dlsym(r.lib, "ncclCommInitRank"));
      r.CommDestroy = reinterpret_cast<decltype(r.CommDestroy)>(dlsym(r.lib, "ncclCommDestroy"));
      r.AllReduce = reinterpret_cast<decltype(r.AllReduce)>(dlsym(r.lib, "ncclAllReduce"));
      r.Reduce = reinterpret_cast<decltype(r.Reduce)>(dlsym(r.lib, "ncclReduce"));
      r.Broadcast = reinterpret_cast<decltype(r.Broadcast)>(dlsym(r.lib, "ncclBroadcast"));
      r.GetErrorString = reinterpret_cast<decltype(r.GetErrorString)>(dlsym(r.lib, "ncclGetErrorString"));
      r.CommCount = reinterpret_cast<decltype(r.CommCount)>(dlsym(r.lib, "ncclCommCount"));
      if (!r.GetUniqueId || !r.CommInitRank || !r.CommDestroy || !r.AllReduce || !r.Reduce || !r.Broadcast || !r.GetErrorString) {
        r.lib = nullptr;
        fail(DR_ERR_UNSUPPORTED, "RCCL: missing symbols in librccl");
      }
    }
    return r;
  }
  void check(ncclResult_t e, const char *what) const {
    if (e != ncclSuccess) fail(DR_ERR_DEVICE, "RCCL %s: %s", what, GetErrorString(e));
  }
};

__global__ __launch_bounds__(256) void k_publish4(const float4 *__restrict__ a, const float4 *__restrict__ b, const float4 *__restrict__ c,
                                                  const float4 *__restrict__ d, float4 *__restrict__ host, size_t n4) {
  const size_t nt = (size_t)gridDim.x * blockDim.x;
  for (size_t i = (size_t)blockIdx.x * blockDim.x + threadIdx.x; i < 4 * n4; i += nt) {
    const size_t k = i / n4, j = i - k * n4;
    host[i] = (k == 0 ? a : (k == 1 ? b : (k == 2 ? c : d)))[j];
  }
}

struct MvsSwitches {
  static int num(const char *name, int dflt) { const char *e = getenv(name); return e ? atoi(e) : dflt; }
  static bool on(const char *name) { return getenv(name) != nullptr; }
  static int hnum(const char *name, int dflt) { const char *e = hook_env(name); return e ? atoi(e) : dflt; }
  static bool hon(const char *name) { return hook_env(name) != nullptr; }
  bool side_stream = !on("DR_MVS_NO_SIDE_STREAM");
  int conv_print = num("DR_CONV_PRINT", 0);
  std::string autotune_only = getenv("DR_AUTOTUNE_ONLY") ? getenv("DR_AUTOTUNE_ONLY") : "";
  int cv_dchunk[3] = {num("DR_CV_DCHUNK1", 0), num("DR_CV_DCHUNK2", 0), num("DR_CV_DCHUNK3", 0)};
  int prob_zchunk = num("DR_PROB_ZCHUNK", 0);
  int hist_blocks = std::max(1, num("DR_HIST_BLOCKS", 128));
  int prob_rows = hnum("DR_PROB_ROWS", 0);
  bool costvol_v2 = hon("DR_COSTVOL_V2");
  bool regress_generic = hon("DR_REGRESS_GENERIC");
  bool shard_allreduce = hon("DR_SHARD_ALLREDUCE");
  int tail_fused = hnum("DR_TAIL_FUSED", 0);
  int tail_qy = hnum("DR_TAIL_QY", 0), tail_zchunk = hnum("DR_TAIL_ZCHUNK", 0);
  bool fn_front = hnum("DR_FN_FRONT", 1) != 0;
  bool fn_head3 = hnum("DR_FN_HEAD3", 1) != 0;
  bool filter_fused = hnum("DR_FILTER_FUSED", 1) != 0;
  bool prob_regress = hnum("DR_PROB_REGRESS", 1) != 0;
  bool vol_split = !hon("DR_VOL_NO_SPLIT");
  bool costvol_v1 = hon("DR_COSTVOL_V1");
  bool costvol_v3 = hon("DR_COSTVOL_V3");
  int costvol_cpl = hnum("DR_COSTVOL_CPL", 4) == 8 ? 8 : 4;
  bool prob_v1 = hon("DR_PROB_V1");
  int prob_block = std::max(64, std::min(256, hnum("DR_PROB_BLOCK", 256) / 64 * 64)), prob_xo = hnum("DR_PROB_XO", 1);
  bool prob_launch_order = hon("DR_PROB_LAUNCH_ORDER"), prob_on_conv = hon("DR_PROB_ON_CONV");
  bool skip_on_conv = hon("DR_SKIP_ON_CONV"), no_skip_fusion = hon("DR_NO_SKIP_FUSION");
  bool out3_folded = hnum("DR_OUT3_FOLDED", 1) != 0;
  bool d2h_copy = hook_env("DR_MVS_D2H") && !strcmp(hook_env("DR_MVS_D2H"), "copy");
  int cv5_rows = hnum("DR_CV5_ROWS", 0);
  bool cv5_reuse = hnum("DR_CV5_REUSE", 1) != 0;
  int cv5_abl = hnum("DR_CV5_ABL", 0);
  int cv4_stages = hnum("DR_CV4_STAGES", 0);
  int cv4_sp8 = hnum("DR_CV4_SP8", 0);
};

class HostCopier {
 public:
  HostCopier() : th_(&HostCopier::loop, this) {}
  ~HostCopier() {
    { std::lock_guard<std::mutex> lk(mu_); quit_ = true; }
    cv_.notify_all();
    th_.join();
  }
  void run(std::function<void()> job) {
    { std::lock_guard<std::mutex> lk(mu_); job_ = std::move(job); busy_ = true; }
    cv_.notify_all();
  }
  void wait() {
    std::unique_lock<std::mutex> lk(mu_);
    done_.wait(lk, [&] { return !busy_; });
    if (!error_.empty()) { std::string e = error_; error_.clear(); fail(DR_ERR_DEVICE, "%s", e.c_str()); }
  }
  void wait_quiet() {
    std::unique_lock<std::mutex> lk(mu_);
    done_.wait(lk, [&] { return !busy_; });
    error_.clear();
  }

 private:
  void loop() {
    std::unique_lock<std::mutex> lk(mu_);
    for (;;) {
      cv_.wait(lk, [&] { return busy_ || quit_; });
      if (quit_) return;
      std::function<void()> job = std::move(job_);
      lk.unlock();
      std::string err;
      try { job(); } catch (const std::exception &e) { err = e.what(); }
      lk.lock();
      error_ = err;
      busy_ = false;
      done_.notify_all();
    }
  }
  std::mutex mu_;
  std::condition_variable cv_, done_;
  std::function<void()> job_;
  std::string error_;
  bool busy_ = false, quit_ = false;
  std::thread th_;
};

static const char *conv_kind_name(const ConvLaunch &c) {
  return c.async == 2 ? (c.march.rm ? "rowmarch" : (c.march.wino ? "winomarch" : "march")) : (c.async == 4 ? "wino" : (c.async ? "async" : ""));
}

class MvsEngine {
 public:
  MvsEngine(const char *path, int device) : device_(device), blob_(load_blob(path)) {
    int n = 0;
    if (hipGetDeviceCount(&n) != hipSuccess || n <= device) fail(DR_ERR_DEVICE, "DrMvsnet: no HIP device %d (found %d) -- the MI355X path has no CPU fallback", device, n);
    DR_HIP(hipSetDevice(device_));
    DR_HIP(hipStreamCreateWithFlags(&stream_, hipStreamNonBlocking));
    DR_HIP(hipStreamCreateWithFlags(&side_, hipStreamNonBlocking));
    for (auto *e : {&ev_fork_, &ev_feat2_, &ev_feat3_}) DR_HIP(hipEventCreateWithFlags(e, hipEventDisableTiming));
    side_enabled_ = sw_.side_stream;
    std::vector<float> lut(256);
    for (int i = 0; i < 256; ++i) lut[i] = (float)((double)(float)i / 255.0);
    lut_ = consts_.upload(lut);
    DR_HIP(hipHostMalloc((void **)&march_err_, sizeof(int), hipHostMallocDefault));
    *march_err_ = 0;
    worker_ = std::thread(&MvsEngine::loop, this);
  }
  ~MvsEngine() {
    {
      std::unique_lock<std::mutex> lk(mu_);
      done_cv_.wait(lk, [&] { return !unprocessed_; });
      running_ = false;
      input_cv_.notify_all();
    }
    worker_.join();
    (void)hipSetDevice(device_);
    (void)hipStreamSynchronize(stream_);
    if (comm_) { Rccl::get().CommDestroy(comm_); comm_ = nullptr; }
    release();
    for (float *&h : h_out_) if (h) (void)hipHostFree(h);
    if (h_in_) (void)hipHostFree(h_in_);
    if (ev_h2d_) (void)hipEventDestroy(ev_h2d_);
    if (march_err_) (void)hipHostFree(march_err_);
    if (fc_flag_) (void)hipHostFree(fc_flag_);
    if (up_stream_) { (void)hipStreamSynchronize(up_stream_); (void)hipEventDestroy(ev_hits_); (void)hipStreamDestroy(up_stream_); }
    (void)hipStreamSynchronize(side_);
    for (auto e : {ev_fork_, ev_feat2_, ev_feat3_}) (void)hipEventDestroy(e);
    (void)hipStreamDestroy(side_);
    (void)hipStreamDestroy(stream_);
  }

  void call_async(int H, int W, int V, int ref, const uint8_t *const *bgrs, const float *K9, const float *const *c2ws,
                  float dmin, float dmax, float disc) {
    check_args(H, W, V, ref, bgrs, K9, c2ws);
    std::unique_lock<std::mutex> lk(mu_);
    done_cv_.wait(lk, [&] { return !unprocessed_; });
    stage_inputs(H, W, V, ref, bgrs, K9, c2ws, dmin, dmax, disc, true);
    unprocessed_ = true;
    input_cv_.notify_all();
  }
  bool ready() { return !unprocessed_; }
  void wait() {
    std::unique_lock<std::mutex> lk(mu_);
    done_cv_.wait(lk, [&] { return !unprocessed_; });
    rethrow_worker_error();
  }
  void get_result(float *depth, float *conf, float *depth_dense, float *conf_dense) {
    std::unique_lock<std::mutex> lk(mu_);
    done_cv_.wait(lk, [&] { return !unprocessed_; });
    rethrow_worker_error();
    if (!has_output_) fail(DR_ERR_PROTOCOL, "Output should be valid. Maybe you called GetResult more than once?");
    const size_t n = (size_t)H_ * W_;
    const float *src = h_out_[out_cur_];
    copier_.run([=] { memcpy(depth_dense, src + 2 * n, n * 4); memcpy(conf_dense, src + 3 * n, n * 4); });
    memcpy(depth, src, n * 4); memcpy(conf, src + n, n * 4);
    copier_.wait();
    has_output_ = false;
  }
  void get_result_view(const float **depth, const float **conf, const float **depth_dense, const float **conf_dense) {
    std::unique_lock<std::mutex> lk(mu_);
    done_cv_.wait(lk, [&] { return !unprocessed_; });
    rethrow_worker_error();
    if (!has_output_) fail(DR_ERR_PROTOCOL, "Output should be valid. Maybe you called GetResult more than once?");
    const size_t n = (size_t)H_ * W_;
    const float *src = h_out_[out_cur_];
    if (depth) *depth = src;
    if (conf) *conf = src + n;
    if (depth_dense) *depth_dense = src + 2 * n;
    if (conf_dense) *conf_dense = src + 3 * n;
    has_output_ = false;
  }

  void set_feature_cache(int capacity) {
    if (capacity < 0 || capacity > 64) fail(DR_ERR_ARG, "drm_set_feature_cache: capacity %d out of range (0 = off, up to 64 key frames)", capacity);
    std::unique_lock<std::mutex> lk(mu_);
    done_cv_.wait(lk, [&] { return !unprocessed_; });
    if (capacity == fcache_cap_) return;
    fcache_cap_ = capacity;
    if (H_) {
      DR_HIP(hipSetDevice(device_));
      const int H = H_, W = W_, V = V_;
      H_ = W_ = V_ = 0;
      configure(H, W, V);
      has_output_ = false;
// ... 41 lines not shown
      for (int i = 0; i < 2; ++i) launch_conv(c, stream_);
      DR_HIP(hipEventRecord(e0, stream_));
      for (int i = 0; i < 8; ++i) launch_conv(c, stream_);
      DR_HIP(hipEventRecord(e1, stream_));
      DR_HIP(hipEventSynchronize(e1));
      float t = 0;
      DR_HIP(hipEventElapsedTime(&t, e0, e1));
      return t / 8;
    };
    double t_before = 0, t_after = 0;
    const bool print = sw_.conv_print > 0;
    const char *only = sw_.autotune_only.empty() ? nullptr : sw_.autotune_only.c_str();
    for (Op &o : ops_) {
      if (o.kind != Op::CONV || !o.replan || (only && o.name.find(only) == std::string::npos)) continue;
      const float t0 = time_launch(o.conv);
      float best = t0;
      int best_rank = 0;
      ConvLaunch best_c = o.conv;
      for (int r = 1; r < std::min(k, o.ncand); ++r) {
        const ConvLaunch c = o.replan(r);
        const float t = time_launch(c);
        if (sw_.conv_print > 1)
          fprintf(stderr, "  cand %-12s rank %2d %s<%d,%d,%d> tile %dx%dx%d lds %zu KB grid %u: %.4f ms\n", o.name.c_str(), r, conv_kind_name(c), c.ci, c.ct, c.pt,
                  c.args.TZ, c.args.TY, c.args.TXT * 16, c.lds_bytes >> 10, c.grid.x, t);
        if (t < best * 0.98f) { best = t; best_rank = r; best_c = c; }
      }
      if (print) fprintf(stderr, "autotune %-12s model %.4f ms %s<%d,%d,%d> tile %dx%dx%d -> rank %d %.4f ms %s<%d,%d,%d> tile %dx%dx%d\n", o.name.c_str(), t0,
                         conv_kind_name(o.conv), o.conv.ci, o.conv.ct, o.conv.pt, o.conv.args.TZ, o.conv.args.TY, o.conv.args.TXT * 16, best_rank, best,
                         conv_kind_name(best_c), best_c.ci, best_c.ct, best_c.pt, best_c.args.TZ, best_c.args.TY, best_c.args.TXT * 16);
      if (print && best_rank != 0)
        fprintf(stderr, "TUNED    {%s,   %d, %d, %d, %d, %d, %d, %d},  // %s %.4f -> %.4f ms\n", o.sig.c_str(), best_c.ci, best_c.ct, best_c.pt, best_c.args.TZ,
                best_c.args.TY, best_c.args.TXT, best_c.async == 2 ? (best_c.march.rm ? 3 : (best_c.march.wino ? 5 : 2)) : best_c.async, o.name.c_str(), t0, best);
      o.conv = best_c;
      t_before += t0; t_after += best;
    }
    (void)hipEventDestroy(e0); (void)hipEventDestroy(e1);
    DR_HIP(hipStreamSynchronize(stream_));
    check_march();
    if (before_ms) *before_ms = (float)t_before;
    if (after_ms) *after_ms = (float)t_after;
    if (fn1_ok_ && !match_fn1()) { fn1_ok_ = false; fc_fast_ = false; }
  }

  void set_view_shard(int nsrc_total) {
    std::unique_lock<std::mutex> lk(mu_);
    if (nsrc_total < 0 || nsrc_total > kMaxSrc) fail(DR_ERR_ARG, "set_view_shard: %d source views unsupported (0..%d)", nsrc_total, kMaxSrc);
    shard_nsrc_ = nsrc_total;
  }
  void comm_init(int rank, int world, const void *unique_id) {
    std::unique_lock<std::mutex> lk(mu_);
    if (comm_) fail(DR_ERR_PROTOCOL, "comm_init: a communicator is already set");
    if (!unique_id || rank < 0 || rank >= world) fail(DR_ERR_ARG, "comm_init: bad rank %d of %d", rank, world);
    Rccl &r = Rccl::get();
    DR_HIP(hipSetDevice(device_));
    ncclUniqueId id;
    memcpy(&id, unique_id, sizeof id);
    r.check(r.CommInitRank(&comm_, world, id, rank), "ncclCommInitRank");
    comm_world_ = world;
    comm_rank_ = rank;
  }
  int comm_count() {
    std::unique_lock<std::mutex> lk(mu_);
    if (!comm_) return 0;
    Rccl &r = Rccl::get();
    if (!r.CommCount) return -1;
    int n = 0;
    r.check(r.CommCount(comm_, &n), "ncclCommCount");
    return n;
  }
  void comm_destroy() {
    std::unique_lock<std::mutex> lk(mu_);
    if (!comm_) return;
    (void)hipSetDevice(device_);
    (void)hipStreamSynchronize(stream_);
    Rccl::get().CommDestroy(comm_);
    comm_ = nullptr;
    comm_world_ = 0;
  }
  void forward_phase(int phase) {
    std::unique_lock<std::mutex> lk(mu_);
    require_config();
    if (phase < 0 || phase > 3) fail(DR_ERR_ARG, "forward_phase: phase must be 0..3");
    DR_HIP(hipSetDevice(device_));
    std::vector<size_t> cut{0};
    for (size_t i = 0; i < ops_.size(); ++i) if (ops_[i].kind == Op::COSTVOL) cut.push_back(i + 1);
    cut.push_back(ops_.size());
    phase_mode_ = true;
    try { forward(nullptr, cut[phase], cut[phase + 1]); } catch (...) { phase_mode_ = false; throw; }
    phase_mode_ = false;
    DR_HIP(hipStreamSynchronize(stream_));
    check_march();
  }
  void device_tensor(const char *name, void **dptr, size_t *n) {
    std::unique_lock<std::mutex> lk(mu_);
    require_config();
    const DevTensor &t = T(name);
    if (dptr) *dptr = t.d;
    if (n) *n = t.n();
  }
  void download(float *depth, float *conf, float *depth_dense, float *conf_dense) {
    std::unique_lock<std::mutex> lk(mu_);
    require_config();
    DR_HIP(hipSetDevice(device_));
    const size_t n = (size_t)H_ * W_ * 4;
    DR_HIP(hipMemcpyAsync(depth, T("depth").d, n, hipMemcpyDeviceToHost, stream_));
    DR_HIP(hipMemcpyAsync(conf, T("confidence").d, n, hipMemcpyDeviceToHost, stream_));
    DR_HIP(hipMemcpyAsync(depth_dense, T("depth3").d, n, hipMemcpyDeviceToHost, stream_));
    DR_HIP(hipMemcpyAsync(conf_dense, T("conf3").d, n, hipMemcpyDeviceToHost, stream_));
    DR_HIP(hipStreamSynchronize(stream_));
    check_march();
  }
  void get_tensor(const char *name, float *out, size_t n_max, size_t *n, int dims[4]) {
    std::unique_lock<std::mutex> lk(mu_);
    require_config();
    DR_HIP(hipSetDevice(device_));
    const DevTensor &t = T(name);
    const size_t logical = (size_t)t.D * t.H * t.W * t.C;
    if (n) *n = logical;
    if (dims) { dims[0] = t.D; dims[1] = t.H; dims[2] = t.W; dims[3] = t.C; }
    if (out) {
      if (logical > n_max) fail(DR_ERR_ARG, "get_tensor(%s): need %zu floats, have %zu", name, logical, n_max);
      DR_HIP(hipStreamSynchronize(stream_));
      check_march();
      if (t.split) {
        const size_t npos = (size_t)t.D * t.H * t.W;
        for (int k = 0; k < t.C / t.split; ++k)
          DR_HIP(hipMemcpy2D(out + (size_t)k * t.split, (size_t)t.C * 4, t.d + (size_t)k * npos * t.split, (size_t)t.split * 4, (size_t)t.split * 4, npos, hipMemcpyDeviceToHost));
      } else if (!t.pad) DR_HIP(hipMemcpy(out, t.d, logical * 4, hipMemcpyDeviceToHost));
      else
        for (int z = 0; z < t.D; ++z)
          DR_HIP(hipMemcpy2D(out + (size_t)z * t.H * t.W * t.C, (size_t)t.W * t.C * 4, t.interior() + (size_t)z * (t.H + 2 * t.pad) * (t.W + 2 * t.pad) * t.C,
                             (size_t)(t.W + 2 * t.pad) * t.C * 4, (size_t)t.W * t.C * 4, t.H, hipMemcpyDeviceToHost));
    }
  }
  void profile(std::string &names, std::vector<float> &ms) {
    std::unique_lock<std::mutex> lk(mu_);
    require_config();
    if (comm_ && shard_nsrc_) fail(DR_ERR_PROTOCOL, "profile(): a view-sharded engine enqueues collectives -- every rank would have to profile in lockstep");
    DR_HIP(hipSetDevice(device_));
    forward(nullptr);
    std::vector<hipEvent_t> ev(ops_.size() + 1);
    for (auto &e : ev) DR_HIP(hipEventCreate(&e));
    forward(&ev);
    DR_HIP(hipStreamSynchronize(stream_));
    check_march();
    names.clear(); ms.clear();
    for (size_t i = 0; i < ops_.size(); ++i) {
      float t = 0;
      DR_HIP(hipEventElapsedTime(&t, ev[i], ev[i + 1]));
      ms.push_back(t);
      const Op &o = ops_[i];
      char kn[64] = "misc";
      if (o.kind == Op::CONV && o.conv.async == 2) snprintf(kn, sizeof kn, "k_conv_m<%d,%d,%d,%d,%d,%d,%d>", o.conv.ci, o.conv.nup, o.conv.ct, o.conv.pt, o.conv.fz, o.conv.ncw, o.conv.march.wino);
      else if (o.kind == Op::CONV && o.conv.async == 4) snprintf(kn, sizeof kn, "k_conv_w<%d,%d,%d>", o.conv.ci, o.conv.ct, o.conv.pt);
      else if (o.kind == Op::CONV && o.conv.async) snprintf(kn, sizeof kn, "k_conv_a<%d,%d,%d>", o.conv.ci, o.conv.ct, o.conv.pt);
      else if (o.kind == Op::CONV && o.conv.bf3) snprintf(kn, sizeof kn, "k_conv_b<%d,%d,%d>", o.conv.ci, o.conv.ct, o.conv.pt);
      else if (o.kind == Op::CONV && o.conv.args.class_loop > 0) snprintf(kn, sizeof kn, "k_conv_c<%d,%d,%d>", o.conv.ci, o.conv.ct, o.conv.pt);
      else if (o.kind == Op::CONV) snprintf(kn, sizeof kn, "k_conv<%d,%d,%d,%d>", o.conv.ci, o.conv.ct, o.conv.pt, o.conv.fz);
      else if (o.kind == Op::COSTVOL) {
        const CostVolArgs &ca = cv_[o.stage - 1];
        const int Cc = 32 >> (o.stage - 1), dch = ca.planes.D >= 8 ? 8 : 4;
        const bool v4 = cv4_applies(o.stage);
        if (v4) snprintf(kn, sizeof kn, "k_costvol4<%d,%d>", Cc, dch);
        else if (cv5_applies(o.stage)) snprintf(kn, sizeof kn, "k_costvol5<%d,%d>", Cc, cv_[o.stage - 1].dchunk);
        else snprintf(kn, sizeof kn, sw_.costvol_v1 ? "k_costvol<%d>" : (sw_.costvol_v2 ? "k_costvol2<%d>" : "k_costvol3<%d>"), Cc);
      }
      else if (o.kind == Op::PROB) {
        if (sw_.prob_v1) snprintf(kn, sizeof kn, "k_prob");
        else if (o.stage >= 1 && o.stage <= 3 && prob_fused_last_[o.stage - 1]) snprintf(kn, sizeof kn, "k_prob2_regress<8>");
        else snprintf(kn, sizeof kn, "k_prob2<%d>", sw_.prob_rows == 2 || sw_.prob_rows == 4 ? sw_.prob_rows : 1);
      }
#ifdef DR_PARITY_HOOKS
      else if (o.kind == Op::TAIL) snprintf(kn, sizeof kn, o.tail.wmf ? "k_tail_m<%d>" : "k_tail<%d>", std::max(3, tail_nout(o.tail.QY, o.tail.QX)));
#endif
      else if (o.kind == Op::REGRESS) snprintf(kn, sizeof kn, "k_regress");
      else if (o.kind == Op::PREPROCESS) snprintf(kn, sizeof kn, "k_preprocess");
      else if (o.kind == Op::FRONT) snprintf(kn, sizeof kn, "k_fn_front");
      else if (o.kind == Op::HEAD3) snprintf(kn, sizeof kn, "k_fn_head3");
      else if (o.kind == Op::SKIPUP) snprintf(kn, sizeof kn, "k_skip_up<%d>", o.stage);
      else if (o.kind == Op::BORDERFIX) snprintf(kn, sizeof kn, "k_out3_border");
      else snprintf(kn, sizeof kn, "k_filter");
      char line[256];
      snprintf(line, sizeof line, "%s\t%s\t%.6e\t%.6e\n", o.name.c_str(), kn, o.flops, o.bytes);
      names += line;
    }
    for (auto &e : ev) (void)hipEventDestroy(e);
  }
  void work(double *flops, double *bytes) {
    std::unique_lock<std::mutex> lk(mu_);
    require_config();
    double f = 0, b = 0;
    for (auto &o : ops_) { f += o.flops; b += o.bytes; }
    if (flops) *flops = f;
    if (bytes) *bytes = b;
  }

 private:
  void check_args(int H, int W, int V, int ref, const uint8_t *const *bgrs, const float *K9, const float *const *c2ws) {
    if (!bgrs || !K9 || !c2ws) fail(DR_ERR_ARG, "CallAsync: null pointer argument");
    const int vmin = shard_nsrc_ ? 1 : 2;
    if (V < vmin || V > kMaxSrc + 1) fail(DR_ERR_ARG, "CallAsync: view_num=%d unsupported (%d..%d)", V, vmin, kMaxSrc + 1);
    if (ref < 0 || ref >= V) fail(DR_ERR_ARG, "CallAsync: ref_index=%d out of range", ref);
    if (H <= 0 || W <= 0 || H % 32 || W % 32) fail(DR_ERR_ARG, "CallAsync: height/width must be positive multiples of 32 (got %dx%d)", H, W);
    for (int i = 0; i < V - 1; ++i) for (int j = i + 1; j < V; ++j)
      if (bgrs[i] == bgrs[j] || c2ws[i] == c2ws[j])
        fail(DR_ERR_ARG, "ERROR: In Call Async passing the same data for index %d and %d", i, j);
  }
  void require_config() { if (!H_) fail(DR_ERR_PROTOCOL, "no window uploaded yet"); }
  void rethrow_worker_error() {
    if (!worker_error_.empty()) { std::string e = worker_error_; worker_error_.clear(); fail(DR_ERR_DEVICE, "%s", e.c_str()); }
  }
  static std::atomic<int> &windows_in_flight(int device) {
    static std::atomic<int> n[16];
    return n[device & 15];
  }
  struct InFlight {
    int dev;
    InFlight(int d, bool counted_already) : dev(d) { if (!counted_already) windows_in_flight(dev).fetch_add(1, std::memory_order_relaxed); }
    ~InFlight() { windows_in_flight(dev).fetch_sub(1, std::memory_order_relaxed); }
  };
  void loop() {
    std::unique_lock<std::mutex> lk(mu_);
    while (running_) {
      if (unprocessed_) {
        try {
          DR_HIP(hipSetDevice(device_));
          InFlight window(device_, prelaunched_);
          if (prelaunched_) prelaunched_ = false;
          else forward(nullptr);
          const size_t n = (size_t)H_ * W_ * 4;
          const int blk = out_cur_ ^ 1;
          float *ho = h_out_[blk];
          if (sw_.d2h_copy) {
            DR_HIP(hipMemcpyAsync(ho, T("depth").d, n, hipMemcpyDeviceToHost, stream_));
            DR_HIP(hipMemcpyAsync(ho + n / 4, T("confidence").d, n, hipMemcpyDeviceToHost, stream_));
            DR_HIP(hipMemcpyAsync(ho + 2 * (n / 4), T("depth3").d, n, hipMemcpyDeviceToHost, stream_));
            DR_HIP(hipMemcpyAsync(ho + 3 * (n / 4), T("conf3").d, n, hipMemcpyDeviceToHost, stream_));
          } else {
            hipLaunchKernelGGL(k_publish4, dim3(256), dim3(256), 0, stream_, (const float4 *)T("depth").d, (const float4 *)T("confidence").d,
                               (const float4 *)T("depth3").d, (const float4 *)T("conf3").d, (float4 *)h_out_dev_[blk], n / 16);
          }
          DR_HIP(hipStreamSynchronize(stream_));
          if (cache_mismatch_recovered()) {
            hipLaunchKernelGGL(k_publish4, dim3(256), dim3(256), 0, stream_, (const float4 *)T("depth").d, (const float4 *)T("confidence").d,
                               (const float4 *)T("depth3").d, (const float4 *)T("conf3").d, (float4 *)h_out_dev_[blk], n / 16);
            DR_HIP(hipStreamSynchronize(stream_));
          }
          check_march();
          out_cur_ = blk;
          has_output_ = true;
        } catch (const std::exception &e) { worker_error_ = e.what(); }
        unprocessed_ = false;
        done_cv_.notify_all();
      }
      input_cv_.wait(lk, [&] { return unprocessed_ || !running_; });
    }
  }

  DevTensor &T(const std::string &name) {
    auto it = tensors_.find(tprefix_.empty() ? name : tprefix_ + name);
    if (it == tensors_.end()) fail(DR_ERR_ARG, "unknown tensor '%s'", name.c_str());
    return it->second;
  }
  DevTensor &alloc(const std::string &name, int D, int H, int W, int C, int pad = 0) {
    DevTensor t; t.D = D; t.H = H; t.W = W; t.C = C; t.pad = pad;
    t.d = dalloc<float>(t.n());
    if (pad) DR_HIP(hipMemset(t.d, 0, t.n() * 4));
    const std::string key = tprefix_.empty() ? name : tprefix_ + name;
    tensors_[key] = t;
    return tensors_[key];
  }
  void release() {
    for (auto &kv : tensors_) (void)hipFree(kv.second.d);
    tensors_.clear();
    ops_.clear();
    ops1_.clear(); fcache_.clear(); fn1_ok_ = false; fc_fast_ = fc_fill_ = false;
    plan_arena_.reset();
    for (void *p : misc_) (void)hipFree(p);
    misc_.clear();
  }

  void fold_bn(const std::string &p, int C, std::vector<float> &sc, std::vector<float> &bi) {
    const auto &g = blob_.at(p + ".weight").data, &b = blob_.at(p + ".bias").data;
    const auto &m = blob_.at(p + ".running_mean").data, &v = blob_.at(p + ".running_var").data;
    sc.resize(C); bi.resize(C);
    for (int c = 0; c < C; ++c) {
      const double s = (double)g[c] / std::sqrt((double)v[c] + 1e-5);
      sc[c] = (float)s;
      bi[c] = (float)((double)b[c] - (double)m[c] * s);
    }
  }
  DevTensor &add_skip(const std::string &opname, const std::string &wname, const DevTensor &in, const std::string &outname, const DevTensor &coarse) {
    const HostTensor &w = blob_.at(wname + ".weight");
    if (!kParityHooks || sw_.skip_on_conv || w.dims[0] != 32 || w.dims[1] != in.C || in.C != 8 || coarse.C != 32 ||
        coarse.H * 2 != in.H || coarse.W * 2 != in.W)
      return add_conv(opname, wname, "", true, false, in, outname, 1, 1, 1, 1, 1, 1, false, CONV_NORMAL, &coarse, 2);
    DevTensor &out = alloc(outname, in.D, in.H, in.W, 32);
    Op o; o.kind = Op::SKIPUP; o.name = opname;
    o.p0 = in.d; o.p1 = plan_arena_->upload(w.data); o.p2 = out.d; o.d0 = in.D; o.d1 = in.H; o.d2 = in.W; o.stage = in.C;
    o.p3 = plan_arena_->upload(blob_.at(wname + ".bias").data); o.p4 = coarse.d;
    o.flops = 2.0 * in.C * 32 * in.n() / in.C; o.bytes = 4.0 * (in.n() + coarse.n() + out.n());
    ops_.push_back(o);
    return out;
  }
  DevTensor &add_conv(const std::string &opname, const std::string &wname, const std::string &bnname, bool conv_bias, bool relu,
                      const DevTensor &in, const std::string &outname, int k3d, int kh, int kw, int sd, int sh, int sw,
                      bool transposed, ConvMode mode, const DevTensor *add, int add_mode, const ConvFuse *fz = nullptr, int out_pad = 0) {
    const HostTensor &w = blob_.at(wname + ".weight");
    ConvLayer L;
    L.transposed = transposed;
    const int c_out = transposed ? w.dims[1] : w.dims[0], c_in_real = transposed ? w.dims[0] : w.dims[1];
    L.Cout = c_out; L.Cin = in.C;
    L.kd = k3d; L.kh = kh; L.kw = kw; L.sd = sd; L.sh = sh; L.sw = sw; L.relu = relu; L.out_pad = out_pad;
    std::vector<float> padded;
    if (c_in_real != in.C) {
      if (transposed || c_in_real > in.C) fail(DR_ERR_ARG, "%s: channel mismatch", opname.c_str());
      const int taps = k3d * kh * kw;
      padded.assign((size_t)c_out * in.C * taps, 0.f);
      for (int co = 0; co < c_out; ++co) for (int ci = 0; ci < c_in_real; ++ci) for (int t = 0; t < taps; ++t)
        padded[((size_t)co * in.C + ci) * taps + t] = w.data[((size_t)co * c_in_real + ci) * taps + t];
      L.weight = padded.data();
    } else L.weight = w.data.data();
    if (!bnname.empty()) fold_bn(bnname, c_out, L.scale, L.bias);
    else if (conv_bias) L.bias = blob_.at(wname + ".bias").data;
    ConvPlanOut P0;
    {
      auto cz = axis_classes(k3d, sd, transposed, in.D), cy = axis_classes(kh, sh, transposed, in.H), cx = axis_classes(kw, sw, transposed, in.W);
      P0.outD = transposed ? in.D * sd : cz[0].npos; P0.outH = transposed ? in.H * sh : cy[0].npos; P0.outW = transposed ? in.W * sw : cx[0].npos;
    }
    DevTensor &out = alloc(outname, P0.outD, P0.outH, P0.outW, c_out, out_pad);
    emit_conv(opname, L, mode, in, out, add ? add->d : nullptr, add_mode, add ? (add_mode == 2 ? add->n() : out.n()) : 0, fz);
    return out;
  }
  void emit_conv(const std::string &opname, const ConvLayer &L, ConvMode mode, const DevTensor &in, DevTensor &out, const float *add_d, int add_mode,
                 size_t add_n, const ConvFuse *fz = nullptr) {
    const int k3d = L.kd, kh = L.kh, kw = L.kw;
    ConvFuse fzc{};
    if (fz) fzc = *fz;
    const bool fused = fz != nullptr;
    ConvPlanOut P = plan_conv(L, mode, in.d, in.D, in.H, in.W, in.C, out.interior(), add_d, add_mode, *plan_arena_, 0, fz, in.split);
    auto keep = std::make_shared<std::vector<float>>(L.weight, L.weight + (size_t)L.Cout * L.Cin * k3d * kh * kw);
    ConvLayer Lc = L;
    const float *in_d = in.d;
    float *out_d = out.interior();
    const int iD = in.D, iH = in.H, iW = in.W, iC = in.C, iS = in.split, ncand = P.ncand;
    auto replan = [this, keep, Lc, mode, in_d, iD, iH, iW, iC, iS, out_d, add_d, add_mode, fzc, fused](int rank) mutable {
      Lc.weight = keep->data();
      return plan_conv(Lc, mode, in_d, iD, iH, iW, iC, out_d, add_d, add_mode, *plan_arena_, rank, fused ? &fzc : nullptr, iS).launches.at(0);
    };
    int idx = 0;
    for (auto &cl : P.launches) {
      Op o; o.kind = Op::CONV; o.conv = cl; o.name = opname + (P.launches.size() > 1 ? "." + std::to_string(idx) : "");
      if (P.launches.size() == 1) {
        o.replan = replan; o.ncand = ncand;
        char sig[160];
        snprintf(sig, sizeof sig, "%d, %d, %d, %d, %d, %d, %d, %d, %d, %d, %d, %d, %d", L.Cin, L.Cout, k3d, kh, kw, L.sd, L.sh, L.sw, L.transposed ? 1 : (L.up2 ? 1 + L.up2 : 0),
                 (int)mode + (fused ? 8 : 0) + (iS ? 16 : 0), iD, iH, iW);
        o.sig = sig;
      }
      o.flops = cl.flops;
      if (idx == 0) o.bytes = 4.0 * ((fused ? in.n() / in.C * fzc.cin + in.n() / 4 : in.n()) + out.n() + add_n);
      if (fused) o.flops += 2.0 * fzc.cin * in.C * (in.n() / in.C);
      ops_.push_back(o);
      ++idx;
    }
  }
  bool lds_fits(size_t bytes) const {
    int optin = 0;
    if (hipDeviceGetAttribute(&optin, hipDeviceAttributeSharedMemPerBlockOptin, device_) != hipSuccess || optin <= 0) {
      (void)hipGetLastError();
      if (hipDeviceGetAttribute(&optin, hipDeviceAttributeMaxSharedMemoryPerBlock, device_) != hipSuccess) { (void)hipGetLastError(); return false; }
    }
    return (size_t)optin >= bytes;
  }
  DevTensor &front_block(const std::string &fn, int V, int H, int W) {
    const HostTensor &wa = blob_.at(fn + "conv0.0.conv.weight"), &wb = blob_.at(fn + "conv0.1.conv.weight");
    const bool shape_ok = wa.dims.size() == 4 && wa.dims[0] == 8 && wa.dims[1] == 3 && wa.dims[2] == 3 && wa.dims[3] == 3 &&
                          wb.dims.size() == 4 && wb.dims[0] == 8 && wb.dims[1] == 8 && wb.dims[2] == 3 && wb.dims[3] == 3;
    const bool fits32 = (double)V * H * W * 32.0 < 2147483648.0 && ((uintptr_t)d_bgr_ & 3) == 0;
    if (!sw_.fn_front || conv_bf3_policy() || !shape_ok || !fits32 || !lds_fits(kFrontLdsBytes)) {
      DevTensor &img = alloc("image", V, H, W, 4);
      { Op o; o.kind = Op::PREPROCESS; o.name = "preprocess"; o.bytes = (double)V * H * W * (3 + 16); ops_.push_back(o); }
      DevTensor &c3a = cbr2("fn.conv0.0", fn + "conv0.0", img, 3, 1, CONV_XPAIR);
      return cbr2("fn.conv0.1", fn + "conv0.1", c3a, 3, 1, CONV_XPAIR);
    }
    DevTensor &c3 = alloc("fn.conv0.1", V, H, W, 8);
    Op o; o.kind = Op::FRONT; o.name = "fn.front";
    FrontArgs &a = o.front;
    a.bgr = d_bgr_; a.lut = lut_; a.out = c3.d;
    a.w1 = reinterpret_cast<const float4 *>(plan_arena_->upload(front_pack(wa.data.data(), 3, 4)));
    a.w2 = reinterpret_cast<const float4 *>(plan_arena_->upload(front_pack(wb.data.data(), 8, 8)));
    auto affine = [&](const std::string &bn) {
      std::vector<float> sc, bi, sb(32);
      fold_bn(bn, 8, sc, bi);
      for (int r = 0; r < 16; ++r) { sb[r] = sc[r & 7]; sb[16 + r] = bi[r & 7]; }
      return plan_arena_->upload(sb);
    };
    a.sb1 = affine(fn + "conv0.0.bn"); a.sb2 = affine(fn + "conv0.1.bn");
    a.V = V; a.H = H; a.W = W;
    a.tilesY = cdiv(H, kFrontTY); a.tilesX = cdiv(W, kFrontTXP); a.ntiles = V * a.tilesY * a.tilesX;
    o.flops = 2.0 * V * H * W * 9.0 * (4 * 8 + 8 * 8);
    o.bytes = (double)V * H * W * (3 + 32);
    ops_.push_back(o);
    return c3;
  }
  DevTensor &cbr2(const std::string &name, const std::string &p, const DevTensor &in, int k, int s, ConvMode m) {
    return add_conv(name, p + ".conv", p + ".bn", false, true, in, name, 1, k, k, 1, s, s, false, m, nullptr, 0);
  }
  DevTensor &cbr3(const std::string &name, const std::string &p, const DevTensor &in, int sd, int shw, ConvMode m) {
    return add_conv(name, p + ".conv", p + ".bn", false, true, in, name, 3, 3, 3, sd, shw, shw, false, m, nullptr, 0);
  }
  DevTensor &dbr3(const std::string &name, const std::string &p, const DevTensor &in, int sd, const DevTensor &skip) {
    return add_conv(name, p + ".conv", p + ".bn", false, true, in, name, 3, 3, 3, sd, 2, 2, true, CONV_NORMAL, &skip, 1);
  }

  void configure(int H, int W, int V) {
    if (H == H_ && W == W_ && V == V_) return;
    DR_HIP(hipStreamSynchronize(stream_));
    release();
    H_ = W_ = V_ = 0;
    memset(cv_, 0, sizeof cv_);
    memset(rg_, 0, sizeof rg_);
    try {
      build_plan(H, W, V);
    } catch (...) {
      release();
      throw;
    }
    H_ = H; W_ = W; V_ = V;
  }
  void build_featurenet(int V, int H, int W) {
    const std::string fn = "feature_net.";
    DevTensor &c3 = front_block(fn, V, H, W);
    DevTensor &c2a = cbr2("fn.conv1.0", fn + "conv1.0", c3, 5, 2, CONV_NORMAL);
    DevTensor &c2b = cbr2("fn.conv1.1", fn + "conv1.1", c2a, 3, 1, CONV_NORMAL);
    DevTensor &c2 = cbr2("fn.conv1.2", fn + "conv1.2", c2b, 3, 1, CONV_NORMAL);
    DevTensor &c1a = cbr2("fn.conv2.0", fn + "conv2.0", c2, 5, 2, CONV_NORMAL);
    DevTensor &c1b = cbr2("fn.conv2.1", fn + "conv2.1", c1a, 3, 1, CONV_NORMAL);
    DevTensor &c1 = cbr2("fn.conv2.2", fn + "conv2.2", c1b, 3, 1, CONV_NORMAL);
    const int fpad = sw_.costvol_v1 ? 0 : 1;
    add_conv("fn.out1", fn + "out.stage1", "", false, false, c1, "feat1", 1, 1, 1, 1, 1, 1, false, CONV_NORMAL, nullptr, 0, nullptr, fpad);
    fork_lo_ = ops_.size();
    DevTensor &i2 = add_skip("fn.skip2", fn + "skip.stage2", c2, "inter2", c1);
    add_conv("fn.out2", fn + "out.stage2", "", false, false, i2, "feat2", 1, 3, 3, 1, 1, 1, false, CONV_NORMAL, nullptr, 0, nullptr, fpad);
    feat2_op_ = ops_.size() - 1;
    const HostTensor &w3 = blob_.at(fn + "skip.stage3.weight");
    const HostTensor &wo3 = blob_.at(fn + "out.stage3.weight");
    if (sw_.out3_folded && !sw_.no_skip_fusion && !sw_.skip_on_conv && w3.dims[0] == 32 && w3.dims[1] == 8 && c3.C == 8 &&
        i2.C == 32 && wo3.dims[0] == 8 && wo3.dims[1] == 32 && i2.H * 2 == c3.H && i2.W * 2 == c3.W) {
      const std::vector<float> &b3 = blob_.at(fn + "skip.stage3.bias").data;
      std::vector<float> wa((size_t)8 * 8 * 9), T(9 * 8), bint(8, 0.f);
      for (int co = 0; co < 8; ++co)
        for (int t = 0; t < 9; ++t) {
          for (int c8 = 0; c8 < 8; ++c8) {
            double acc = 0;
            for (int c = 0; c < 32; ++c) acc += (double)wo3.data[((size_t)co * 32 + c) * 9 + t] * (double)w3.data[(size_t)c * 8 + c8];
            wa[((size_t)co * 8 + c8) * 9 + t] = (float)acc;
          }
          double tb = 0;
          for (int c = 0; c < 32; ++c) tb += (double)wo3.data[((size_t)co * 32 + c) * 9 + t] * (double)b3[c];
          T[t * 8 + co] = (float)tb;
        }
      for (int co = 0; co < 8; ++co) { double b = 0; for (int t = 0; t < 9; ++t) b += (double)T[t * 8 + co]; bint[co] = (float)b; }
      DevTensor &f3 = alloc("feat3", c3.D, c3.H, c3.W, 8, fpad);
      if (sw_.fn_head3 && !conv_bf3_policy() && (double)f3.n() * 4.0 < 2147483648.0 && (double)i2.n() * 4.0 < 2147483648.0 && lds_fits(kH3LdsBytes)) {
        Op o; o.kind = Op::HEAD3; o.name = "fn.head3";
        Head3Args &a = o.head3;
        a.c0 = c3.d; a.i2 = i2.d;
        a.wa = reinterpret_cast<const float4 *>(plan_arena_->upload(h3_pack_a(wa.data())));
        a.wb = reinterpret_cast<const float4 *>(plan_arena_->upload(h3_pack_b(wo3.data.data())));
        std::vector<float> b16(16);
        for (int r = 0; r < 16; ++r) b16[r] = bint[r & 7];
        a.bias16 = plan_arena_->upload(b16); a.T = plan_arena_->upload(T);
        a.out = f3.interior(); a.V = c3.D; a.H = c3.H; a.W = c3.W;
        a.out_row = (f3.W + 2 * f3.pad) * 8; a.out_plane = (f3.H + 2 * f3.pad) * a.out_row;
        a.tilesY = cdiv(c3.H, kH3TY); a.tilesX = cdiv(c3.W, kH3TXP); a.ntiles = c3.D * a.tilesY * a.tilesX;
        o.flops = 2.0 * c3.D * c3.H * c3.W * (9.0 * 8 * 8 + 4.0 * 32 * 8);
        o.bytes = 4.0 * (c3.n() + i2.n() + (double)c3.D * c3.H * c3.W * 8);
        ops_.push_back(o);
      } else {
      ConvLayer LA; LA.Cin = 8; LA.Cout = 8; LA.kd = 1; LA.kh = 3; LA.kw = 3; LA.weight = wa.data(); LA.bias = bint; LA.out_pad = fpad;
      emit_conv("fn.out3a", LA, CONV_XPAIR, c3, f3, nullptr, 0, 0);
      for (int py = 0; py < 2; ++py) {
        ConvLayer LB; LB.Cin = 32; LB.Cout = 8; LB.kd = 1; LB.kh = 3; LB.kw = 3; LB.weight = wo3.data.data(); LB.up2 = 1 + py; LB.out_pad = fpad;
        emit_conv(py ? "fn.out3c" : "fn.out3b", LB, CONV_NORMAL, i2, f3, f3.interior(), 1, f3.n() / 2);
      }
      Op o; o.kind = Op::BORDERFIX; o.name = "fn.out3d"; o.p2 = f3.interior(); o.p1 = plan_arena_->upload(T); o.d0 = c3.D; o.d1 = c3.H; o.d2 = c3.W;
      o.stage = fpad; o.bytes = 64.0 * c3.D * (c3.H + c3.W);
      ops_.push_back(o);
      }
    } else
    if (!sw_.no_skip_fusion && !sw_.skip_on_conv && kParityHooks && w3.dims[0] == 32 && w3.dims[1] == 8 && c3.C == 8 && i2.C == 32 &&
        i2.H * 2 == c3.H && i2.W * 2 == c3.W) {
      ConvFuse fz{c3.d, plan_arena_->upload(w3.data), plan_arena_->upload(blob_.at(fn + "skip.stage3.bias").data), i2.d, 8};
      DevTensor virt; virt.D = c3.D; virt.H = c3.H; virt.W = c3.W; virt.C = 32; virt.d = nullptr;
      add_conv("fn.out3", fn + "out.stage3", "", false, false, virt, "feat3", 1, 3, 3, 1, 1, 1, false, CONV_XPAIR, nullptr, 0, &fz, fpad);
    } else {
      DevTensor &i3 = add_skip("fn.skip3", fn + "skip.stage3", c3, "inter3", i2);
      add_conv("fn.out3", fn + "out.stage3", "", false, false, i3, "feat3", 1, 3, 3, 1, 1, 1, false, CONV_XPAIR, nullptr, 0, nullptr, fpad);
    }
    fork_hi_ = ops_.size();
  }

  struct FnOut { size_t op; int stage; size_t offset; };
  struct FcEntry { uint64_t key[2] = {0, 0}; float *feat[3] = {nullptr, nullptr, nullptr}; uint8_t *bgr = nullptr; uint64_t used = 0; bool valid = false; };
  static bool same_instance(const ConvLaunch &a, const ConvLaunch &b) {
    return a.async == b.async && a.ci == b.ci && a.ct == b.ct && a.pt == b.pt && a.fz == b.fz && a.bf3 == b.bf3 && a.nup == b.nup && a.ncw == b.ncw &&
           a.march.wino == b.march.wino && a.march.rm == b.march.rm;
  }
  void build_fn1(int H, int W) {
    fn1_ok_ = false; ops1_.clear(); fcache_.clear();
    if (ops_.empty() || ops_[0].kind != Op::FRONT || sw_.costvol_v1 || shard_nsrc_) return;
    const size_t lo = fork_lo_, hi = fork_hi_, f2 = feat2_op_;
    std::vector<Op> batch;
    batch.swap(ops_);
    tprefix_ = "c1.";
    try { build_featurenet(1, H, W); } catch (...) { tprefix_.clear(); ops_.swap(batch); fork_lo_ = lo; fork_hi_ = hi; feat2_op_ = f2; throw; }
    tprefix_.clear();
    ops1_.swap(ops_); ops_.swap(batch);
    fork_lo_ = lo; fork_hi_ = hi; feat2_op_ = f2;
    if (!match_fn1()) { ops1_.clear(); return; }
    const size_t img_bytes = (size_t)H * W * 3;
    fcache_.resize(fcache_cap_);
    for (FcEntry &e : fcache_) {
      for (int s = 0; s < 3; ++s) {
        const DevTensor &t = T("c1.feat" + std::to_string(s + 1));
        e.feat[s] = dalloc<float>(t.n()); misc_.push_back(e.feat[s]);
        DR_HIP(hipMemset(e.feat[s], 0, t.n() * 4));
      }
      e.bgr = dalloc<uint8_t>(img_bytes + 16); misc_.push_back(e.bgr);
    }
    if (!fc_flag_) { DR_HIP(hipHostMalloc((void **)&fc_flag_, sizeof(int), hipHostMallocDefault)); *fc_flag_ = 0; }
    if (!up_stream_) { DR_HIP(hipStreamCreateWithFlags(&up_stream_, hipStreamNonBlocking)); DR_HIP(hipEventCreateWithFlags(&ev_hits_, hipEventDisableTiming)); }
    fn1_out_.clear();
    for (size_t i = 0; i < ops1_.size(); ++i) {
      Op &o = ops1_[i];
      float *out = o.kind == Op::CONV ? o.conv.args.out : (o.kind == Op::HEAD3 ? o.head3.out : nullptr);
      for (int s = 0; s < 3 && out; ++s) {
        const DevTensor &t = T("c1.feat" + std::to_string(s + 1));
        if (out >= t.d && out < t.d + t.n()) fn1_out_.push_back({i, s, (size_t)(out - t.d)});
      }
    }
    if (fn1_out_.size() != 3) { ops1_.clear(); fcache_.clear(); return; }
    fn1_ok_ = true;
  }
  bool match_fn1() {
    for (Op &o : ops1_) {
      const Op *b = nullptr;
      for (size_t i = 0; i < fork_hi_ && i < ops_.size(); ++i) if (ops_[i].name == o.name) b = &ops_[i];
      if (!b || b->kind != o.kind) return false;
      if (o.kind == Op::FRONT || o.kind == Op::HEAD3) continue;
      if (o.kind != Op::CONV) return false;
      if (same_instance(o.conv, b->conv)) continue;
      if (!o.replan) return false;
      bool found = false;
      for (int r = 0; r < o.ncand && !found; ++r) {
        const ConvLaunch c = o.replan(r);
        if (same_instance(c, b->conv)) { o.conv = c; found = true; }
      }
      if (!found) return false;
    }
    return true;
  }
  static void image_key(const uint8_t *p, size_t n, int H, int W, uint64_t key[2]) {
    uint64_t a = 0xcbf29ce484222325ull ^ (uint64_t)H, b = 0x9e3779b97f4a7c15ull ^ (uint64_t)W;
    auto mix = [&](uint64_t w) { a = (a ^ w) * 0x100000001b3ull; b = (b + w) * 0xff51afd7ed558ccdull; b ^= b >> 29; };
    auto word = [&](size_t off) { uint64_t w; memcpy(&w, p + off, 8); return w; };
    for (size_t o = 0; o < 64; o += 8) { mix(word(o)); mix(word(n - 64 + o)); }
    const size_t step = (n / 512) & ~(size_t)7;
    for (size_t k = 1; k < 512 && step; ++k) mix(word(k * step));
    key[0] = a; key[1] = b;
  }
  void plan_cache_use(int H, int W, int V, const uint8_t *const *bgrs, const std::vector<int> &order) {
    fc_fast_ = false; fc_fill_ = false; fc_miss_ = -1;
    if (!fn1_ok_ || (int)fcache_.size() < V + 1 || shard_nsrc_ || comm_ || phase_mode_) return;
    for (int s = 1; s <= 3; ++s) if (!cv5_applies(s)) return;
    const size_t img_bytes = (size_t)H * W * 3;
    uint64_t keys[8][2];
    int nmiss = 0;
    ++fc_clock_;
    for (int v = 0; v < V; ++v) {
      image_key(bgrs[order[v]], img_bytes, H, W, keys[v]);
      fc_slot_[v] = -1;
      for (size_t e = 0; e < fcache_.size(); ++e)
        if (fcache_[e].valid && fcache_[e].key[0] == keys[v][0] && fcache_[e].key[1] == keys[v][1]) { fc_slot_[v] = (int)e; break; }
      for (int u = 0; u < v; ++u) if (fc_slot_[v] >= 0 && fc_slot_[u] == fc_slot_[v]) fc_slot_[v] = -1;
      if (fc_slot_[v] < 0) { ++nmiss; fc_miss_ = v; } else fcache_[fc_slot_[v]].used = fc_clock_;
    }
    auto evict = [&]() {
      int best = -1;
      for (size_t e = 0; e < fcache_.size(); ++e) {
        bool in_window = false;
        for (int v = 0; v < V; ++v) in_window |= fc_slot_[v] == (int)e;
        if (!in_window && (best < 0 || !fcache_[e].valid || (fcache_[best].valid && fcache_[e].used < fcache_[best].used))) best = (int)e;
        if (best >= 0 && !fcache_[best].valid) break;
      }
      return best;
    };
    if (nmiss <= 1) {
      fc_fast_ = true;
      if (nmiss == 1) {
        const int e = evict();
        fcache_[e].valid = false;
        fcache_[e].key[0] = keys[fc_miss_][0]; fcache_[e].key[1] = keys[fc_miss_][1]; fcache_[e].used = fc_clock_;
        fc_slot_[fc_miss_] = e;
      }
      fc_hits_ += V - nmiss; fc_misses_ += nmiss;
    } else {
      fc_fill_ = true; fc_miss_ = -1;
      for (int v = 0; v < V; ++v) {
        if (fc_slot_[v] >= 0) continue;
        const int e = evict();
        fcache_[e].valid = false;
        fcache_[e].key[0] = keys[v][0]; fcache_[e].key[1] = keys[v][1]; fcache_[e].used = fc_clock_;
        fc_slot_[v] = e;
      }
      fc_misses_ += V; ++fc_batch_windows_;
    }
    for (int s = 0; s < 3; ++s)
      for (int v = 0; v < V; ++v)
        if (fc_fast_) cv_[s].vfeat[v] = fcache_[fc_slot_[v]].feat[s];
  }
  void launch_fn_op(const Op &o, hipStream_t st) {
    if (o.kind == Op::CONV) launch_conv(o.conv, st);
    else if (o.kind == Op::FRONT) launch_fn_front(o.front, st);
    else if (o.kind == Op::HEAD3) launch_fn_head3(o.head3, st);
    else fail(DR_ERR_UNSUPPORTED, "feature cache: op kind %d in the single-view plan", (int)o.kind);
  }
  void launch_cache_io() {
    const size_t img_bytes = (size_t)H_ * W_ * 3;
    CacheIoArgs io{};
    for (int v = 0; v < V_; ++v) {
      io.img[v] = reinterpret_cast<const uint4 *>(d_bgr_ + v * img_bytes);
      io.entry[v] = reinterpret_cast<uint4 *>(fcache_[fc_slot_[v]].bgr);
    }
    io.miss = fc_miss_; io.flag = fc_flag_dev(); io.n16 = img_bytes / 16;
    hipLaunchKernelGGL(k_cache_io, dim3(32, V_), dim3(256), 0, stream_, io);
  }
  void forward_cached_features() {
    const size_t img_bytes = (size_t)H_ * W_ * 3;
    if (!defer_cache_io_) launch_cache_io();
    if (fc_miss_ >= 0) {
      FcEntry &e = fcache_[fc_slot_[fc_miss_]];
      for (const FnOut &p : fn1_out_) {
        Op &o = ops1_[p.op];
        (o.kind == Op::CONV ? o.conv.args.out : o.head3.out) = e.feat[p.stage] + p.offset;
      }
      for (Op &o : ops1_) {
        if (o.kind == Op::FRONT) o.front.bgr = d_bgr_ + fc_miss_ * img_bytes;
        launch_fn_op(o, stream_);
      }
      e.valid = true;
    }
  }
  void fill_cache_from_batch() {
    const size_t img_bytes = (size_t)H_ * W_ * 3;
    for (int v = 0; v < V_; ++v) {
      FcEntry &e = fcache_[fc_slot_[v]];
      if (e.valid) continue;
      for (int s = 0; s < 3; ++s) {
        const DevTensor &t = T("feat" + std::to_string(s + 1));
        const size_t n1 = t.n() / t.D;
        DR_HIP(hipMemcpyAsync(e.feat[s], t.d + v * n1, n1 * 4, hipMemcpyDeviceToDevice, stream_));
      }
      DR_HIP(hipMemcpyAsync(e.bgr, d_bgr_ + v * img_bytes, img_bytes, hipMemcpyDeviceToDevice, stream_));
      e.valid = true;
    }
  }
  int *fc_flag_dev() { int *d = nullptr; DR_HIP(hipHostGetDevicePointer((void **)&d, fc_flag_, 0)); return d; }
  bool cache_mismatch_recovered() {
    if (!fc_flag_ || !*fc_flag_) return false;
    *fc_flag_ = 0;
    ++fc_collisions_;
    for (FcEntry &e : fcache_) e.valid = false;
    fc_fast_ = false; fc_fill_ = false;
    for (int s = 0; s < 3; ++s) set_batch_vfeat(s);
    forward(nullptr);
    DR_HIP(hipStreamSynchronize(stream_));
    return true;
  }
  void set_batch_vfeat(int s) {
    const DevTensor &t = T("feat" + std::to_string(s + 1));
    for (int v = 0; v < V_ && v <= kMaxSrc; ++v) cv_[s].vfeat[v] = t.d + (size_t)v * (t.n() / t.D);
  }

  void build_plan(int H, int W, int V) {
    plan_arena_.reset(new DeviceArena());
    plan_arena_->err_flag = march_err_;
    for (float *&h : h_out_) if (h) { (void)hipHostFree(h); h = nullptr; }
    if (h_in_) { (void)hipHostFree(h_in_); h_in_ = nullptr; }
    for (int b = 0; b < 2; ++b) {
      DR_HIP(hipHostMalloc((void **)&h_out_[b], (size_t)H * W * 16, hipHostMallocDefault));
      DR_HIP(hipHostGetDevicePointer((void **)&h_out_dev_[b], h_out_[b], 0));
    }
    has_output_ = false;
    DR_HIP(hipHostMalloc((void **)&h_in_, (size_t)V * H * W * 3, hipHostMallocDefault));
    d_bgr_ = dalloc<uint8_t>((size_t)V * H * W * 3 + 16); misc_.push_back(d_bgr_);
    d_state_ = dalloc<unsigned>(16); misc_.push_back(d_state_);
    d_hist_ = dalloc<unsigned>(3 * 2048); misc_.push_back(d_hist_);
    DR_HIP(hipMemset(d_hist_, 0, 3 * 2048 * 4));
    DR_HIP(hipMemset(d_state_, 0, 16 * 4));

    build_featurenet(V, H, W);
    if (fcache_cap_ > 0) build_fn1(H, W);

    for (int s = 1; s <= 3; ++s) {
      const int sc = 1 << (3 - s), h = H / sc, w = W / sc, D = blob_.depth_num[s - 1], C = 32 >> (s - 1);
      if (!(D == 4 || D % 8 == 0)) fail(DR_ERR_UNSUPPORTED, "depth_num[%d]=%d must be 4 or a multiple of 8", s - 1, D);
      const std::string S = std::to_string(s), cr = "cost_regularization_net.stage" + S + ".", pre = "s" + S + ".";
      DevTensor &vol = alloc("volume" + S, D, h, w, C);
      if (C == 32 && sw_.vol_split && !conv_bf3_policy()) vol.split = 16;
      {
        Op o; o.kind = Op::COSTVOL; o.stage = s; o.name = pre + "costvol";
        o.bytes = 4.0 * ((double)V * h * w * C + vol.n());
        o.flops = (double)(V - 1) * D * h * w * (3.0 * C + 2.0 * C + 8.0 * C);
        ops_.push_back(o);
      }
      const bool four = D == 4;
      DevTensor &c0 = cbr3(pre + "conv0", cr + "conv0", vol, 1, 1, CONV_XPAIR);
      DevTensor &k1 = cbr3(pre + "conv1", cr + "conv1", c0, 2, 2, CONV_NORMAL);
      DevTensor &k2 = cbr3(pre + "conv2", cr + "conv2", k1, 1, 1, CONV_NORMAL);
      DevTensor &k3 = cbr3(pre + "conv3", cr + "conv3", k2, 2, 2, CONV_NORMAL);
      DevTensor &k4 = cbr3(pre + "conv4", cr + "conv4", k3, 1, 1, CONV_NORMAL);
      DevTensor &k5 = cbr3(pre + "conv5", cr + "conv5", k4, four ? 1 : 2, 2, CONV_NORMAL);
      DevTensor &k6 = cbr3(pre + "conv6", cr + "conv6", k5, 1, 1, CONV_NORMAL);
      DevTensor &x7 = dbr3(pre + "conv7", cr + "conv7", k6, four ? 1 : 2, k4);
      DevTensor &x9 = dbr3(pre + "conv9", cr + "conv9", x7, 2, k2);
#ifdef DR_PARITY_HOOKS
      const HostTensor &w11 = blob_.at(cr + "conv11.conv.weight");
      const HostTensor &wpr = blob_.at(cr + "prob.weight");
      const bool tail = sw_.tail_fused && !sw_.prob_on_conv && !conv_bf3_policy() && w11.dims.size() == 5 && w11.dims[0] == 16 && w11.dims[1] == 8 && w11.dims[2] == 3 &&
                        w11.dims[3] == 3 && w11.dims[4] == 3 && x9.C == 16 && c0.C == 8 && x9.D * 2 == D && x9.H * 2 == h && x9.W * 2 == w && wpr.dims[0] == 1 && wpr.dims[1] == 8;
      if (tail) {
        std::vector<float> sc, bi;
        fold_bn(cr + "conv11.bn", 8, sc, bi);
        sc.insert(sc.end(), bi.begin(), bi.end());
        DevTensor &lg = alloc("logits" + S, D, h, w, 1);
        Op o; o.kind = Op::TAIL; o.stage = s; o.name = pre + "tail";
        TailArgs &t = o.tail;
        t.x = x9.d; t.skip = c0.d; t.out = lg.d; t.D = D; t.h = h; t.w = w;
        t.wd = plan_arena_->upload(tail_pack_deconv(w11.data.data()));
        t.sb = plan_arena_->upload(sc);
        t.wp = plan_arena_->upload(tail_pack_prob(wpr.data.data()));
        const bool mf = sw_.tail_fused == 1;
        t.wmf = mf ? plan_arena_->upload(tail_pack_deconv_mfma(w11.data.data())) : nullptr;
        tail_pick_tile(h, w, t.QY, t.QX, mf);
        if (sw_.tail_qy == 4 || sw_.tail_qy == 8 || sw_.tail_qy == 16 || (sw_.tail_qy == 32 && !mf)) { t.QY = sw_.tail_qy; t.QX = 256 / t.QY; }
        t.zchunk = sw_.tail_zchunk > 0 ? std::min(D, sw_.tail_zchunk) : tail_pick_zchunk(D, h, w, t.QY, t.QX);
        const double N = (double)D * h * w;
        o.flops = 2.0 * 3.375 * 16 * 8 * N + 2.0 * 216 * N;
        o.bytes = 4.0 * (x9.n() + c0.n() + lg.n());
        ops_.push_back(o);
      } else
#endif
      {
      DevTensor &x11 = dbr3(pre + "conv11", cr + "conv11", x9, 2, c0);
      if (sw_.prob_on_conv && w % 8 == 0) {
        add_conv(pre + "prob", cr + "prob", "", false, false, x11, "logits" + S, 3, 3, 3, 1, 1, 1, false, CONV_X8, nullptr, 0);
      } else {
        const HostTensor &pw = blob_.at(cr + "prob.weight");
        std::vector<float> wt(27 * 8);
        for (int ci = 0; ci < 8; ++ci) for (int t = 0; t < 27; ++t) wt[t * 8 + ci] = pw.data[ci * 27 + t];
        DevTensor &lg = alloc("logits" + S, D, h, w, 1);
        Op o; o.kind = Op::PROB; o.stage = s; o.name = pre + "prob";
        o.p0 = x11.d; o.p1 = plan_arena_->upload(wt); o.p2 = lg.d; o.d0 = D; o.d1 = h; o.d2 = w;
        o.flops = 2.0 * 216 * D * h * w; o.bytes = 4.0 * (x11.n() + lg.n());
        ops_.push_back(o);
      }
      }
      alloc("depth" + S, 1, h, w, 1);
      alloc("conf" + S, 1, h, w, 1);
      { Op o; o.kind = Op::REGRESS; o.stage = s; o.name = pre + "regress"; o.bytes = 4.0 * ((double)D * h * w + 2.0 * h * w); o.flops = 8.0 * D * h * w; ops_.push_back(o); }
    }
    alloc("edge", 1, H, W, 1);
    alloc("depth", 1, H, W, 1);
    alloc("confidence", 1, H, W, 1);
    { Op o; o.kind = Op::EDGE; o.name = "filter.edge"; o.bytes = 8.0 * H * W; ops_.push_back(o); }
    const int shifts[3] = {21, 10, 0}, bits[3] = {11, 11, 10};
    for (int i = 0; i < 3; ++i) {
      Op o; o.kind = Op::HIST; o.shift = shifts[i]; o.bits = bits[i]; o.stage = i; o.d0 = i ? shifts[i - 1] : 0; o.d1 = i ? bits[i - 1] : 0;
      o.name = "filter.hist" + std::to_string(i); o.bytes = 4.0 * H * W; ops_.push_back(o);
      if (sw_.filter_fused) continue;
      Op q; q.kind = Op::SCAN; q.shift = shifts[i]; q.bits = bits[i]; q.name = "filter.scan" + std::to_string(i); ops_.push_back(q);
    }
    { Op o; o.kind = Op::APPLY; o.name = "filter.apply"; o.shift = shifts[2]; o.bits = bits[2]; o.bytes = 20.0 * H * W; ops_.push_back(o); }
  }

  void stage_inputs(int H, int W, int V, int ref, const uint8_t *const *bgrs, const float *K9, const float *const *c2ws,
                    float dmin, float dmax, float disc, bool may_prelaunch = false) {
    DR_HIP(hipSetDevice(device_));
    configure(H, W, V);
    const size_t img_bytes = (size_t)H * W * 3;
    std::vector<int> order;
    order.push_back(ref);
    for (int i = 0; i < V; ++i) if (i != ref) order.push_back(i);
    bool pinned = true;
    for (int v = 0; v < V && pinned; ++v) {
      hipPointerAttribute_t at;
      hipDeviceptr_t base = nullptr;
// ... 245 lines not shown
          break;
        case Op::COSTVOL: {
          const CostVolArgs &a = cv_[o.stage - 1];
          const int C = 32 >> (o.stage - 1);
          if (a.V - 1 <= 0) {
            const DevTensor &vol0 = T("volume" + std::to_string(o.stage));
            DR_HIP(hipMemsetAsync(vol0.d, 0, vol0.n() * 4, stream_));
          }
          CostVolArgs b = a;
          b.gz = cdiv(a.planes.D, a.dchunk);
          b.abl = sw_.cv5_abl;
#ifdef DR_PARITY_HOOKS
          if (!a.fpad) {
            const int cpl = C >= 16 ? sw_.costvol_cpl : 4, pxb = 256 / (C / cpl);
            b.gx = cdiv(a.w, pxb); b.nwg = b.gx * b.gz * a.h;
            const dim3 grid1(8 * cdiv(b.nwg, 8));
            if (C == 32 && cpl == 8) hipLaunchKernelGGL((k_costvol<32, 8>), grid1, dim3(256), 0, stream_, b);
            else if (C == 32) hipLaunchKernelGGL((k_costvol<32, 4>), grid1, dim3(256), 0, stream_, b);
            else if (C == 16 && cpl == 8) hipLaunchKernelGGL((k_costvol<16, 8>), grid1, dim3(256), 0, stream_, b);
            else if (C == 16) hipLaunchKernelGGL((k_costvol<16, 4>), grid1, dim3(256), 0, stream_, b);
            else hipLaunchKernelGGL((k_costvol<8, 4>), grid1, dim3(256), 0, stream_, b);
          } else
#endif
          {
            b.gx = cdiv(a.w, 1024 / C); b.nwg = b.gx * b.gz * a.h;
            const dim3 grid(8 * cdiv(b.nwg, 8));
#ifdef DR_PARITY_HOOKS
            const int dch = a.planes.D >= 8 ? 8 : 4;
            const int tw = C == 8 ? 16 : 8, th = (1024 / C) / tw;
            if (cv4_applies(o.stage)) {
              CostVolArgs c4 = a;
              c4.gx = a.w / tw; c4.gz = a.planes.D / dch; c4.nwg = c4.gx * (a.h / th) * c4.gz;
              const dim3 g4(8 * cdiv(c4.nwg, 8));
              const bool sp8 = dch == 8 && C != 32 && ((sw_.cv4_sp8 >> (o.stage - 1)) & 1);
              if (C == 32 && dch == 8) hipLaunchKernelGGL((k_costvol4<32, 8, 4>), g4, dim3(256), 0, stream_, c4);
              else if (C == 32) hipLaunchKernelGGL((k_costvol4<32, 4, 4>), g4, dim3(256), 0, stream_, c4);
              else if (C == 16 && sp8) hipLaunchKernelGGL((k_costvol4<16, 8, 8>), g4, dim3(256), 0, stream_, c4);
              else if (C == 16 && dch == 8) hipLaunchKernelGGL((k_costvol4<16, 8, 4>), g4, dim3(256), 0, stream_, c4);
              else if (C == 16) hipLaunchKernelGGL((k_costvol4<16, 4, 4>), g4, dim3(256), 0, stream_, c4);
              else if (sp8) hipLaunchKernelGGL((k_costvol4<8, 8, 8>), g4, dim3(256), 0, stream_, c4);
              else if (dch == 8) hipLaunchKernelGGL((k_costvol4<8, 8, 4>), g4, dim3(256), 0, stream_, c4);
              else hipLaunchKernelGGL((k_costvol4<8, 4, 4>), g4, dim3(256), 0, stream_, c4);
            } else
#endif
            if (cv5_applies(o.stage)) {
              const bool d8 = a.dchunk == 8;
              CostVolArgs b4 = b;
              b4.gx = cdiv(a.w, 256 / C); b4.nwg = b4.gx * b4.gz * cdiv(a.h, 4);
              const dim3 grid4(8 * cdiv(b4.nwg, 8));
              [[maybe_unused]] const bool rows4 = sw_.cv5_rows ? sw_.cv5_rows == 4 : true;
#ifdef DR_PARITY_HOOKS
#define DR_CV5(CC, DD) do { if (!sw_.cv5_reuse) hipLaunchKernelGGL((k_costvol5<CC, DD, 0, 1>), grid, dim3(256), 0, stream_, b); \
                            else if (rows4) hipLaunchKernelGGL((k_costvol5<CC, DD, 1, 4>), grid4, dim3(256), 0, stream_, b4); \
                            else hipLaunchKernelGGL((k_costvol5<CC, DD, 1, 1>), grid, dim3(256), 0, stream_, b); } while (0)
#else
#define DR_CV5(CC, DD) hipLaunchKernelGGL((k_costvol5<CC, DD, 1, 4>), grid4, dim3(256), 0, stream_, b4)
#endif
              if (C == 32 && d8) DR_CV5(32, 8);
              else if (C == 32) DR_CV5(32, 4);
              else if (C == 16 && d8) DR_CV5(16, 8);
              else if (C == 16) DR_CV5(16, 4);
              else if (d8) DR_CV5(8, 8);
              else DR_CV5(8, 4);
#undef DR_CV5
            } else {
            const bool v3 = !sw_.costvol_v2 && a.dchunk % 4 == 0 && a.planes.D % 4 == 0;
            if (v3 && C == 32) hipLaunchKernelGGL((k_costvol3<32>), grid, dim3(256), 0, stream_, b);
            else if (v3 && C == 16) hipLaunchKernelGGL((k_costvol3<16>), grid, dim3(256), 0, stream_, b);
            else if (v3) hipLaunchKernelGGL((k_costvol3<8>), grid, dim3(256), 0, stream_, b);
            else if (C == 32) hipLaunchKernelGGL((k_costvol2<32>), grid, dim3(256), 0, stream_, b);
            else if (C == 16) hipLaunchKernelGGL((k_costvol2<16>), grid, dim3(256), 0, stream_, b);
            else hipLaunchKernelGGL((k_costvol2<8>), grid, dim3(256), 0, stream_, b);
            }
          }
          if (comm_ && shard_nsrc_ && !phase_mode_) {
            const DevTensor &vol = T("volume" + std::to_string(o.stage));
            Rccl &r = Rccl::get();
            if (rooted) {
              r.check(r.Reduce(vol.d, vol.d, vol.n(), ncclFloat, ncclSum, 0, comm_, stream_), "ncclReduce");
              idle_stage = comm_rank_ != 0;
            } else r.check(r.AllReduce(vol.d, vol.d, vol.n(), ncclFloat, ncclSum, comm_, stream_), "ncclAllReduce");
          }
          break;
        }
        case Op::REGRESS: {
          const RegressArgs &r = rg_[o.stage - 1];
          const bool done = regress_done_[o.stage - 1];
          regress_done_[o.stage - 1] = false;
          if (!idle_stage && !done) {
            const dim3 grid(cdiv(r.h * r.w, 256)), block(256);
            const int D = sw_.regress_generic ? 0 : r.planes.D;
            if (D == 48) hipLaunchKernelGGL(k_regress_r<48>, grid, block, 0, stream_, r);
            else if (D == 32) hipLaunchKernelGGL(k_regress_r<32>, grid, block, 0, stream_, r);
            else if (D == 8) hipLaunchKernelGGL(k_regress_r<8>, grid, block, 0, stream_, r);
            else if (D == 4) hipLaunchKernelGGL(k_regress_r<4>, grid, block, 0, stream_, r);
            else hipLaunchKernelGGL(k_regress, grid, block, 0, stream_, r);
          }
          if (rooted) {
            Rccl &c = Rccl::get();
            const DevTensor &dep = T("depth" + std::to_string(o.stage));
            c.check(c.Broadcast(dep.d, dep.d, dep.n(), ncclFloat, 0, comm_, stream_), "ncclBroadcast");
            if (o.stage == 3) {
              const DevTensor &cf = T("conf3");
              c.check(c.Broadcast(cf.d, cf.d, cf.n(), ncclFloat, 0, comm_, stream_), "ncclBroadcast");
            }
            idle_stage = false;
          }
          break;
        }
        case Op::EDGE:
          if (sw_.filter_fused) hipLaunchKernelGGL(k_edge2, dim3(cdiv(H_ * W_, 256)), dim3(256), 0, stream_, T("depth3").d, T("edge").d, H_, W_, d_state_, d_hist_, filter_rank_);
          else hipLaunchKernelGGL(k_edge, dim3(cdiv(H_ * W_, 256)), dim3(256), 0, stream_, T("depth3").d, T("edge").d, H_, W_, d_state_, filter_rank_);
          break;
        case Op::HIST:
          if (sw_.filter_fused && o.stage > 0)
            hipLaunchKernelGGL(k_hist_s, dim3(std::min(cdiv(H_ * W_, 256), sw_.hist_blocks)), dim3(256), 0, stream_, T("edge").d, H_ * W_, o.d0, o.d1, o.shift, o.bits, o.stage,
                               d_state_, d_hist_);
          else hipLaunchKernelGGL(k_hist, dim3(std::min(cdiv(H_ * W_, 256), sw_.hist_blocks)), dim3(256), 0, stream_, T("edge").d, H_ * W_, o.shift, o.bits, d_state_, d_hist_);
          break;
        case Op::SCAN:
          hipLaunchKernelGGL(k_scan, dim3(1), dim3(256), 0, stream_, d_state_, d_hist_, o.shift, o.bits);
          break;
        case Op::APPLY:
          if (sw_.filter_fused)
            hipLaunchKernelGGL(k_apply_s, dim3(cdiv(H_ * W_, 256)), dim3(256), 0, stream_, T("edge").d, d_state_, d_hist_, o.shift, o.bits, T("depth3").d, T("conf3").d,
                               T("depth").d, T("confidence").d, H_ * W_);
          else hipLaunchKernelGGL(k_apply, dim3(cdiv(H_ * W_, 256)), dim3(256), 0, stream_, T("edge").d, d_state_, T("depth3").d, T("conf3").d,
                                  T("depth").d, T("confidence").d, H_ * W_);
          break;
      }
      if (on_side && i - 1 == feat2_op_) DR_HIP(hipEventRecord(ev_feat2_, side_));
      if (on_side && i - 1 == fork_hi_ - 1) DR_HIP(hipEventRecord(ev_feat3_, side_));
    }
    if (fc_fill_ && first == 0 && last >= ops_.size()) fill_cache_from_batch();
    if (ev) DR_HIP(hipEventRecord((*ev)[i], stream_));
    DR_HIP(hipGetLastError());
  }

  bool cv5_applies(int stage) const {
    const CostVolArgs &a = cv_[stage - 1];
    return !sw_.costvol_v1 && !sw_.costvol_v2 && !sw_.costvol_v3 && a.fpad && a.view_aggregation && a.V > 1 && (a.dchunk == 4 || a.dchunk == 8) &&
           a.planes.D % a.dchunk == 0;
  }
  bool cv4_applies(int stage) const {
    const CostVolArgs &a = cv_[stage - 1];
    const int C = 32 >> (stage - 1), tw = C == 8 ? 16 : 8, th = (1024 / C) / tw, dch = a.planes.D >= 8 ? 8 : 4;
    return !sw_.costvol_v1 && !sw_.costvol_v2 && !sw_.costvol_v3 && ((sw_.cv4_stages >> (stage - 1)) & 1) && a.fpad && a.view_aggregation && a.V > 1 &&
           a.w % tw == 0 && a.h % th == 0 && a.planes.D % dch == 0;
  }
  hipStream_t side_ = nullptr;
  hipEvent_t ev_fork_ = nullptr, ev_feat2_ = nullptr, ev_feat3_ = nullptr;
  bool side_enabled_ = true;
  size_t fork_lo_ = 0, fork_hi_ = 0, feat2_op_ = 0;
  int fcache_cap_ = 0;
  std::vector<FcEntry> fcache_;
  std::vector<Op> ops1_;
  std::vector<FnOut> fn1_out_;
  std::string tprefix_;
  bool fn1_ok_ = false;
  bool fc_fast_ = false, fc_fill_ = false;
  int fc_miss_ = -1, fc_slot_[kMaxSrc + 1] = {};
  int *fc_flag_ = nullptr;
  hipStream_t up_stream_ = nullptr;
  hipEvent_t ev_hits_ = nullptr;
  bool prelaunched_ = false;
  bool defer_cache_io_ = false;
  uint64_t fc_clock_ = 0, fc_hits_ = 0, fc_misses_ = 0, fc_batch_windows_ = 0, fc_collisions_ = 0;

  const MvsSwitches sw_;
#ifdef DR_PARITY_HOOKS
  static constexpr bool kParityHooks = true;
#else
  static constexpr bool kParityHooks = false;
#endif
  int device_;
  int *march_err_ = nullptr;
  void check_march() {
    if (march_err_ && *march_err_) { const int c = *march_err_; *march_err_ = 0; fail(DR_ERR_DEVICE, "k_conv_m: a ring wait gave up (code %d): the LDS producer/consumer protocol stalled", c); }
  }
  Blob blob_;
  hipStream_t stream_ = nullptr;
  DeviceArena consts_;
  const float *lut_ = nullptr;
  std::unique_ptr<DeviceArena> plan_arena_;
  std::map<std::string, DevTensor> tensors_;
  std::vector<Op> ops_;
  std::vector<void *> misc_;
  CostVolArgs cv_[3];
  RegressArgs rg_[3];
  uint8_t *d_bgr_ = nullptr, *h_in_ = nullptr;
  float *h_out_[2] = {nullptr, nullptr}, *h_out_dev_[2] = {nullptr, nullptr};
  int out_cur_ = 0;
  hipEvent_t ev_h2d_ = nullptr;
  unsigned *d_state_ = nullptr, *d_hist_ = nullptr;
  unsigned filter_rank_ = 0;
  bool prob_fused_last_[3] = {false, false, false};
  bool regress_done_[3] = {false, false, false};
  int H_ = 0, W_ = 0, V_ = 0;
  int shard_nsrc_ = 0;
  ncclComm_t comm_ = nullptr;
  int comm_world_ = 0, comm_rank_ = 0;
  bool phase_mode_ = false;

  std::thread worker_;
  HostCopier copier_;
  std::mutex mu_;
  std::condition_variable input_cv_, done_cv_;
  bool running_ = true;
  std::atomic<bool> unprocessed_{false};
  bool has_output_ = false;
  std::string worker_error_;
};

}

using dr::guarded;
struct drm_s {
  std::unique_ptr<dr::MvsEngine> e;
};
static inline dr::MvsEngine *eng(drm_s *h) {
  if (!h || !h->e) dr::fail(DR_ERR_ARG, "NULL handle");
  return h->e.get();
}

extern "C" {

const char *dr_last_error(void) { return dr::last_error_slot().c_str(); }
const char *dr_version(void) { return "dr_mi355x 0.1 gfx950"; }

int drm_create(const char *weights_path, int device, drm_t **out) {
  return guarded([&] {
    if (!weights_path || !out) dr::fail(DR_ERR_ARG, "drm_create: null argument");
    auto *h = new drm_s();
    try { h->e.reset(new dr::MvsEngine(weights_path, device)); } catch (...) { delete h; throw; }
    *out = h;
  });
}
void drm_destroy(drm_t *h) { delete h; }
int drm_set_feature_cache(drm_t *h, int capacity) { return guarded([&] { eng(h)->set_feature_cache(capacity); }); }
int drm_feature_cache_stats(drm_t *h, uint64_t out[6]) {
  return guarded([&] { if (!out) dr::fail(DR_ERR_ARG, "drm_feature_cache_stats: null argument"); eng(h)->feature_cache_stats(out); });
}
int drm_call_async(drm_t *h, int height, int width, int view_num, int ref_index, const uint8_t *const *bgrs, const float *K9,
                   const float *const *c2ws, float depth_min, float depth_max, float discard_percentage) {
  return guarded([&] { eng(h)->call_async(height, width, view_num, ref_index, bgrs, K9, c2ws, depth_min, depth_max, discard_percentage); });
}
int drm_ready(drm_t *h) { return (h && h->e && h->e->ready()) ? 1 : 0; }
int drm_wait(drm_t *h) { return guarded([&] { eng(h)->wait(); }); }
int drm_get_result(drm_t *h, float *depth, float *confidence, float *depth_dense, float *confidence_dense) {
  return guarded([&] { eng(h)->get_result(depth, confidence, depth_dense, confidence_dense); });
}
int drm_get_result_view(drm_t *h, const float **depth, const float **confidence, const float **depth_dense, const float **confidence_dense) {
  return guarded([&] { eng(h)->get_result_view(depth, confidence, depth_dense, confidence_dense); });
}
void *drm_host_alloc(size_t bytes) {
  void *p = nullptr;
  if (hipHostMalloc(&p, bytes ? bytes : 1, hipHostMallocDefault) != hipSuccess) { (void)hipGetLastError(); return nullptr; }
  return p;
}
void drm_host_free(void *p) { if (p) (void)hipHostFree(p); }
int drm_upload(drm_t *h, int height, int width, int view_num, int ref_index, const uint8_t *const *bgrs, const float *K9,
               const float *const *c2ws, float depth_min, float depth_max, float discard_percentage) {
  return guarded([&] { eng(h)->upload(height, width, view_num, ref_index, bgrs, K9, c2ws, depth_min, depth_max, discard_percentage); });
}
int drm_forward(drm_t *h, int iters, float *ms_total) { return guarded([&] { eng(h)->forward_n(iters, ms_total); }); }
int drm_autotune(drm_t *h, int max_candidates, float *before_ms, float *after_ms) {
  return guarded([&] { eng(h)->autotune(max_candidates, before_ms, after_ms); });
}
int drm_set_view_shard(drm_t *h, int nsrc_total) { return guarded([&] { eng(h)->set_view_shard(nsrc_total); }); }
int drm_forward_phase(drm_t *h, int phase) { return guarded([&] { eng(h)->forward_phase(phase); }); }
int drm_comm_available(void) { return guarded([&] { (void)dr::Rccl::get(); }); }
int drm_comm_unique_id(uint8_t id[128]) {
  return guarded([&] {
    if (!id) dr::fail(DR_ERR_ARG, "drm_comm_unique_id: null argument");
    static_assert(sizeof(ncclUniqueId) == 128, "ncclUniqueId size");
    dr::Rccl &r = dr::Rccl::get();
    ncclUniqueId u;
    r.check(r.GetUniqueId(&u), "ncclGetUniqueId");
    memcpy(id, &u, 128);
  });
}
int drm_comm_init(drm_t *h, int rank, int world, const uint8_t id[128]) { return guarded([&] { eng(h)->comm_init(rank, world, id); }); }
int drm_comm_destroy(drm_t *h) { return guarded([&] { eng(h)->comm_destroy(); }); }
int drm_comm_count(drm_t *h, int *nranks) {
  return guarded([&] { if (!nranks) dr::fail(DR_ERR_ARG, "drm_comm_count: null pointer"); *nranks = eng(h)->comm_count(); });
}
int drm_device_tensor(drm_t *h, const char *name, void **dptr, size_t *nfloats) {
  return guarded([&] { if (!name) dr::fail(DR_ERR_ARG, "drm_device_tensor: null name"); eng(h)->device_tensor(name, dptr, nfloats); });
}
int drm_download(drm_t *h, float *depth, float *confidence, float *depth_dense, float *confidence_dense) {
  return guarded([&] { eng(h)->download(depth, confidence, depth_dense, confidence_dense); });
}
int drm_get_stage_output(drm_t *h, int stage, float *depth, float *confidence) {
  return guarded([&] {
    if (stage < 1 || stage > 3) dr::fail(DR_ERR_ARG, "stage must be 1..3");
    size_t n; int dims[4];
    eng(h)->get_tensor(("depth" + std::to_string(stage)).c_str(), nullptr, 0, &n, dims);
    eng(h)->get_tensor(("depth" + std::to_string(stage)).c_str(), depth, n, &n, dims);
    eng(h)->get_tensor(("conf" + std::to_string(stage)).c_str(), confidence, n, &n, dims);
  });
}
int drm_get_tensor(drm_t *h, const char *name, float *out, size_t n_max, size_t *n, int dims[4]) {
  return guarded([&] { eng(h)->get_tensor(name, out, n_max, n, dims); });
}
int drm_profile(drm_t *h, char *names, size_t names_cap, float *ms, int cap, int *count) {
  return guarded([&] {
    std::string nm; std::vector<float> t;
    eng(h)->profile(nm, t);
    if (count) *count = (int)t.size();
    if (names && names_cap) { strncpy(names, nm.c_str(), names_cap - 1); names[names_cap - 1] = 0; }
    for (int i = 0; i < (int)t.size() && i < cap; ++i) ms[i] = t[i];
  });
}
int drm_work(drm_t *h, double *flops, double *bytes) { return guarded([&] { eng(h)->work(flops, bytes); }); }

int drm_debug_conv(int device, const float *in, int D, int H, int W, int Cin, const float *weight, int Cout, int kd, int kh, int kw,
                   int sd, int sh, int sw, int transposed, const float *scale, const float *bias, int relu, const float *add,
                   int add_up2, float *out, int out_dims[3]) {
  return guarded([&] {
    using namespace dr;
    int n = 0;
    if (hipGetDeviceCount(&n) != hipSuccess || n <= device) fail(DR_ERR_DEVICE, "no HIP device %d", device);
    DR_HIP(hipSetDevice(device));
    DeviceArena arena;
    arena.err_flag = arena.upload(std::vector<int>(1, 0));
    ConvLayer L;
    L.Cin = Cin; L.Cout = Cout; L.kd = kd; L.kh = kh; L.kw = kw; L.sd = sd; L.sh = sh; L.sw = sw;
    L.transposed = transposed == 1; L.weight = weight; L.relu = relu != 0;
    const bool up2 = transposed == 2;
    if (scale) L.scale.assign(scale, scale + Cout);
    if (bias) L.bias.assign(bias, bias + Cout);
    const ConvMode mode = (!transposed && sw == 1 && Cout == 8) ? CONV_XPAIR : ((!transposed && sw == 1 && Cout == 1) ? CONV_X8 : CONV_NORMAL);
    auto cz = axis_classes(kd, sd, L.transposed, D), cy = axis_classes(kh, sh, L.transposed, H), cx = axis_classes(kw, sw, L.transposed, W);
    const int oD = L.transposed ? D * sd : cz[0].npos, oH = L.transposed ? H * sh : (up2 ? 2 * H : cy[0].npos), oW = L.transposed ? W * sw : (up2 ? 2 * W : cx[0].npos);
    std::vector<float> hin(in, in + (size_t)D * H * W * Cin);
    float *d_in = arena.upload(hin);
    const size_t on = (size_t)oD * oH * oW * Cout;
    std::vector<float> zero(on, 0.f);
    float *d_out = arena.upload(zero);
    float *d_add = nullptr;
    if (add) {
      const size_t an = add_up2 ? (size_t)oD * (oH / 2) * (oW / 2) * Cout : on;
      std::vector<float> ha(add, add + an);
      d_add = arena.upload(ha);
    }
    const char *rk = getenv("DR_CONV_RANK");
    ConvPlanOut P;
    for (int py = 0; py < (up2 ? 2 : 1); ++py) {
      L.up2 = up2 ? 1 + py : 0;
      P = plan_conv(L, mode, d_in, D, H, W, Cin, d_out, d_add, add_up2 ? 2 : 1, arena, rk ? atoi(rk) : 0);
      for (auto &cl : P.launches) launch_conv(cl, nullptr);
    }
    DR_HIP(hipDeviceSynchronize());
    DR_HIP(hipGetLastError());
    int march_err = 0;
    DR_HIP(hipMemcpy(&march_err, arena.err_flag, sizeof(int), hipMemcpyDeviceToHost));
    if (march_err) fail(DR_ERR_DEVICE, "k_conv_m: a ring wait gave up (code %d)", march_err);
    if (getenv("DR_CONV_PRINT")) {
      const ConvLaunch &c = P.launches.at(0);
      fprintf(stderr, "debug_conv: %s<%d,%d,%d> nup %d tile %dx%dx%d lds %zu grid %ux%u (%d candidates)%s\n", (c.async == 2 ? (c.march.rm ? "rowmarch" : (c.march.wino ? "winomarch" : "march")) : (c.async == 4 ? "wino" : (c.async ? "async" : (c.bf3 ? "bf16x3" : "sync")))), c.ci, c.ct, c.pt,
              c.nup, c.args.TZ, c.args.TY, c.args.TXT * 16, c.lds_bytes, c.grid.x, c.grid.z, P.ncand, c.args.class_loop ? ", class loop" : "");
    }
    DR_HIP(hipMemcpy(out, d_out, on * 4, hipMemcpyDeviceToHost));
    if (out_dims) { out_dims[0] = oD; out_dims[1] = oH; out_dims[2] = oW; }
  });
}

int drm_debug_tail(int device, const float *x, const float *skip, const float *w_deconv, const float *scale8, const float *bias8, const float *w_prob, int D, int h,
                   int w, int qy, int zchunk, int form, float *out) {
  return guarded([&] {
    using namespace dr;
#ifndef DR_PARITY_HOOKS
    fail(DR_ERR_UNSUPPORTED, "drm_debug_tail: k_tail / k_tail_m are built into the parity library (libdr_mi355x_hooks.so, -DDR_PARITY_HOOKS) only");
#else
    int n = 0;
    if (hipGetDeviceCount(&n) != hipSuccess || n <= device) fail(DR_ERR_DEVICE, "no HIP device %d", device);
    if (D <= 0 || h <= 0 || w <= 0 || (D | h | w) & 1) fail(DR_ERR_ARG, "drm_debug_tail: output dims must be positive and even");
    DR_HIP(hipSetDevice(device));
    DeviceArena arena;
    TailArgs t{};
    t.x = arena.upload(std::vector<float>(x, x + (size_t)(D / 2) * (h / 2) * (w / 2) * 16));
    t.skip = arena.upload(std::vector<float>(skip, skip + (size_t)D * h * w * 8));
    t.wd = arena.upload(tail_pack_deconv(w_deconv));
    std::vector<float> sb(scale8, scale8 + 8);
    sb.insert(sb.end(), bias8, bias8 + 8);
    t.sb = arena.upload(sb);
    t.wp = arena.upload(tail_pack_prob(w_prob));
    float *d_out = arena.upload(std::vector<float>((size_t)D * h * w, -12345.f));
    t.out = d_out; t.D = D; t.h = h; t.w = w;
    const bool mf = form == 1;
    t.wmf = mf ? arena.upload(tail_pack_deconv_mfma(w_deconv)) : nullptr;
    tail_pick_tile(h, w, t.QY, t.QX, mf);
    if (qy == 4 || qy == 8 || qy == 16 || (qy == 32 && !mf)) { t.QY = qy; t.QX = 256 / qy; }
    t.zchunk = zchunk > 0 ? std::min(D, zchunk) : tail_pick_zchunk(D, h, w, t.QY, t.QX);
    launch_tail(t, nullptr);
    DR_HIP(hipDeviceSynchronize());
    DR_HIP(hipGetLastError());
    DR_HIP(hipMemcpy(out, d_out, (size_t)D * h * w * 4, hipMemcpyDeviceToHost));
#endif
  });
}

}
```

tandem_amd/dr_mvsnet.py:

```python
import ctypes as C

import numpy as np

from . import _lib
from ._lib import check, fptr, u8p, f32p


class DrMvsnetOutput:

    def __init__(self, height, width):
        self.height, self.width = height, width
        self.depth = np.empty((height, width), np.float32)
        self.confidence = np.empty((height, width), np.float32)
        self.depth_dense = np.empty((height, width), np.float32)
        self.confidence_dense = np.empty((height, width), np.float32)


def _marshal(bgrs, intrinsic_matrix, cam_to_worlds, height, width):
    bgrs = [np.ascontiguousarray(b, dtype=np.uint8) for b in bgrs]
    for b in bgrs:
        if b.size != height * width * 3:
            raise ValueError("DrMvsnet: image of %d bytes, expected %d x %d x 3" % (b.size, height, width))
    c2ws = [np.ascontiguousarray(c, dtype=np.float32) for c in cam_to_worlds]
    if any(c.size != 16 for c in c2ws):
# ... 70 lines not shown

    def GetResult(self):
        if self._hw is None:
            raise _lib.DrError(2, "GetResult before CallAsync")
        out = getattr(self, "_next_out", None)
        self._next_out = None
        if out is None or (out.height, out.width) != tuple(self._hw):
            out = DrMvsnetOutput(*self._hw)
        check(self._L.drm_get_result(self._h, fptr(out.depth), fptr(out.confidence), fptr(out.depth_dense),
                                        fptr(out.confidence_dense)))
        return out

    def GetResultView(self):
        if self._hw is None:
            raise _lib.DrError(2, "GetResult before CallAsync")
        p = [f32p() for _ in range(4)]
        check(self._L.drm_get_result_view(self._h, *[C.byref(q) for q in p]))
        out = DrMvsnetOutput.__new__(DrMvsnetOutput)
        out.height, out.width = self._hw
        n = self._hw[0] * self._hw[1] * 4
        out.depth, out.confidence, out.depth_dense, out.confidence_dense = [
            np.frombuffer(_view(q, n, self._engine), np.float32).reshape(self._hw) for q in p]
        return out

    def set_feature_cache(self, capacity):
        check(self._L.drm_set_feature_cache(self._h, int(capacity)))

    def feature_cache_stats(self):
        out = (C.c_uint64 * 6)()
        check(self._L.drm_feature_cache_stats(self._h, out))
        return dict(views_from_cache=int(out[0]), views_computed=int(out[1]), batch_windows=int(out[2]), key_collisions=int(out[3]),
                    single_view_plan=bool(out[4]), entries=int(out[5]))

    def alloc_images(self, view_num, height, width):
        n = view_num * height * width * 3
        ptr = self._L.drm_host_alloc(n)
        if not ptr:
            raise MemoryError("drm_host_alloc(%d)" % n)
        L = self._L
        flat = np.frombuffer(_view(ptr, n, _Owned(lambda q: L.drm_host_free(q), ptr)), np.uint8)
        return [flat[v * height * width * 3:(v + 1) * height * width * 3].reshape(height, width, 3) for v in range(view_num)]

    def upload(self, height, width, view_num, ref_index, bgrs, intrinsic_matrix, cam_to_worlds, depth_min, depth_max,
               discard_percentage):
        keep = _marshal(bgrs, intrinsic_matrix, cam_to_worlds, height, width)
        check(self._L.drm_upload(self._h, height, width, view_num, ref_index, keep[3], fptr(keep[2]), keep[4],
                                    depth_min, depth_max, discard_percentage))
        self._hw = (height, width)

    def forward(self, iters=1):
        ms = C.c_float()
        check(self._L.drm_forward(self._h, iters, C.byref(ms)))
        return ms.value

    def autotune(self, max_candidates=8):
        a, b = C.c_float(), C.c_float()
        check(self._L.drm_autotune(self._h, max_candidates, C.byref(a), C.byref(b)))
        return a.value, b.value

    def set_view_shard(self, nsrc_total):
        check(self._L.drm_set_view_shard(self._h, int(nsrc_total)))

    def forward_phase(self, phase):
        check(self._L.drm_forward_phase(self._h, int(phase)))

    @staticmethod
    def comm_available():
        return _lib.lib().drm_comm_available() == 0

    @staticmethod
    def comm_unique_id():
        buf = (C.c_uint8 * 128)()
        check(_lib.lib().drm_comm_unique_id(buf))
        return bytes(buf)

    def comm_init(self, rank, world, unique_id):
        buf = (C.c_uint8 * 128).from_buffer_copy(unique_id)
        check(self._L.drm_comm_init(self._h, int(rank), int(world), buf))

    def comm_destroy(self):
        check(self._L.drm_comm_destroy(self._h))

    def comm_count(self):
        n = C.c_int()
        check(self._L.drm_comm_count(self._h, C.byref(n)))
        return n.value

    def device_tensor(self, name):
        ptr, n = C.c_void_p(), C.c_size_t()
        check(self._L.drm_device_tensor(self._h, name.encode(), C.byref(ptr), C.byref(n)))
        return ptr.value, int(n.value)

    def download(self):
        out = DrMvsnetOutput(*self._hw)
        check(self._L.drm_download(self._h, fptr(out.depth), fptr(out.confidence), fptr(out.depth_dense),
                                      fptr(out.confidence_dense)))
        return out

    def stage_output(self, stage):
        sc = 2 ** (3 - stage)
        h, w = self._hw[0] // sc, self._hw[1] // sc
        d, c = np.empty((h, w), np.float32), np.empty((h, w), np.float32)
        check(self._L.drm_get_stage_output(self._h, stage, fptr(d), fptr(c)))
        return d, c

    def tensor(self, name):
        n, dims = C.c_size_t(), (C.c_int * 4)()
        check(self._L.drm_get_tensor(self._h, name.encode(), None, 0, C.byref(n), dims))
        out = np.empty(tuple(dims), np.float32)
        check(self._L.drm_get_tensor(self._h, name.encode(), fptr(out), n.value, C.byref(n), dims))
        return out

    def profile(self):
        names = C.create_string_buffer(1 << 16)
        ms = (C.c_float * 512)()
        cnt = C.c_int()
        check(self._L.drm_profile(self._h, names, len(names), ms, 512, C.byref(cnt)))
        rows = []
        for line, t in zip(names.value.decode().strip().split("\n"), list(ms)[:cnt.value]):
            op, kern, fl, by = line.split("\t")
            rows.append(dict(op=op, kernel=kern, flops=float(fl), bytes=float(by), ms=t))
        return rows

    def work(self):
        f, b = C.c_double(), C.c_double()
        check(self._L.drm_work(self._h, C.byref(f), C.byref(b)))
        return f.value, b.value


def debug_conv(x, weight, stride=(1, 1, 1), transposed=False, scale=None, bias=None, relu=False, add=None,
               add_up2=False, device=0):
    x = np.ascontiguousarray(x, np.float32)
    w = np.ascontiguousarray(weight, np.float32)
    D, H, W, Cin = x.shape
    up2 = transposed == "up2"
    transposed = 2 if up2 else int(bool(transposed))
    Cout = w.shape[1] if transposed == 1 else w.shape[0]
    kd, kh, kw = w.shape[2:]
    sd, sh, sw = stride
    oD, oH, oW = ((D * sd, H * sh, W * sw) if transposed == 1 else ((D, 2 * H, 2 * W) if up2 else
                  ((D + 2 * (kd // 2) - kd) // sd + 1, (H + 2 * (kh // 2) - kh) // sh + 1, (W + 2 * (kw // 2) - kw) // sw + 1)))
    out = np.empty((oD, oH, oW, Cout), np.float32)
    dims = (C.c_int * 3)()
    opt = lambda a: fptr(np.ascontiguousarray(a, np.float32)) if a is not None else None
    keep = [np.ascontiguousarray(a, np.float32) if a is not None else None for a in (scale, bias, add)]
    check(_lib.lib().drm_debug_conv(device, fptr(x), D, H, W, Cin, fptr(w), Cout, kd, kh, kw, sd, sh, sw,
                                    int(transposed), fptr(keep[0]) if keep[0] is not None else None,
                                    fptr(keep[1]) if keep[1] is not None else None, int(relu),
                                    fptr(keep[2]) if keep[2] is not None else None, int(add_up2), fptr(out), dims))
    assert tuple(dims) == (oD, oH, oW)
    return out


def debug_tail(x, skip, w_deconv, scale, bias, w_prob, qy=0, zchunk=0, form=1, device=0):
    x, skip = np.ascontiguousarray(x, np.float32), np.ascontiguousarray(skip, np.float32)
    D, h, w, _ = skip.shape
    assert x.shape == (D // 2, h // 2, w // 2, 16) and skip.shape[3] == 8
    wd, wp = np.ascontiguousarray(w_deconv, np.float32), np.ascontiguousarray(w_prob, np.float32)
    assert wd.shape == (16, 8, 3, 3, 3) and wp.shape == (1, 8, 3, 3, 3)
    sc, bi = np.ascontiguousarray(scale, np.float32), np.ascontiguousarray(bias, np.float32)
    out = np.empty((D, h, w), np.float32)
    check(_lib.lib().drm_debug_tail(device, fptr(x), fptr(skip), fptr(wd), fptr(sc), fptr(bi), fptr(wp), D, h, w, int(qy), int(zchunk), int(form), fptr(out)))
    return out
```

Baseline: 590.5 depth-maps/s.

## Chain the feature-net 1x1 output head into the preceding Winograd conv epilogue

Adds a chained variant of the Winograd 3x3 conv kernel whose epilogue also computes the following 1x1 projection (fn.out1) with MFMA on the register-resident outputs, including scale/bias and the optional upsampled add. This removes one kernel launch and the re-read of the intermediate activation by the 1x1 conv. The planner merges the two ops when their shapes match, keeps the autotune replan path consistent, and updates the feature-cache output pointer bookkeeping. The cost is extra registers and epilogue work in the producer kernel, which may lower occupancy. A debug entry point is added for parity checks.

```diff
diff --git a/include/dr_mi355x.h b/include/dr_mi355x.h
--- a/include/dr_mi355x.h
+++ b/include/dr_mi355x.h
@@ -60,6 +60,10 @@
 int drm_debug_conv(int device, const float *in, int D, int H, int W, int Cin, const float *weight, int Cout,
                    int kd, int kh, int kw, int sd, int sh, int sw, int transposed, const float *scale,
                    const float *bias, int relu, const float *add, int add_up2, float *out, int out_dims[3]);
+
+int drm_debug_conv_chain(int device, const float *in, int D, int H, int W, int Cin, const float *weight, int Cout, const float *scale, const float *bias,
+                         int relu, const float *weight1, int Cout1, const float *scale1, const float *bias1, const float *add_up2, int out_pad,
+                         float *out, float *out1, int *chained);
 
 int drm_debug_tail(int device, const float *x, const float *skip, const float *w_deconv, const float *scale8, const float *bias8, const float *w_prob, int D,
                    int h, int w, int qy, int zchunk, int form, float *out);
diff --git a/tandem_amd/_lib.py b/tandem_amd/_lib.py
--- a/tandem_amd/_lib.py
+++ b/tandem_amd/_lib.py
@@ -52,6 +52,8 @@
     "drm_debug_conv": (C.c_int, [C.c_int, f32p, C.c_int, C.c_int, C.c_int, C.c_int, f32p, C.c_int, C.c_int, C.c_int,
                                  C.c_int, C.c_int, C.c_int, C.c_int, C.c_int, f32p, f32p, C.c_int, f32p, C.c_int,
                                  f32p, C.POINTER(C.c_int)]),
+    "drm_debug_conv_chain": (C.c_int, [C.c_int, f32p, C.c_int, C.c_int, C.c_int, C.c_int, f32p, C.c_int, f32p, f32p, C.c_int, f32p, C.c_int, f32p, f32p,
+                                       f32p, C.c_int, f32p, f32p, C.POINTER(C.c_int)]),
     "drm_debug_tail": (C.c_int, [C.c_int, f32p, f32p, f32p, f32p, f32p, f32p, C.c_int, C.c_int, C.c_int, C.c_int, C.c_int, C.c_int, f32p]),
     "drm_autotune": (C.c_int, [vp, C.c_int, C.POINTER(C.c_float), C.POINTER(C.c_float)]),
     "drm_set_view_shard": (C.c_int, [vp, C.c_int]),
diff --git a/tandem_amd/csrc/conv_mfma.h b/tandem_amd/csrc/conv_mfma.h
--- a/tandem_amd/csrc/conv_mfma.h
+++ b/tandem_amd/csrc/conv_mfma.h
@@ -40,6 +40,12 @@
   int a_slots;
   int a_wbufs;
   int class_loop;
+  const float4 *ch_w;
+  const float *ch_scale, *ch_bias, *ch_add;
+  float *ch_out;
+  int ch_outH, ch_outW, ch_outC;
+  int ch_add_mode, ch_addH, ch_addW;
+  int ch_split;
 };
 
 constexpr int kConvThreads = 256;
@@ -737,6 +743,7 @@
   int nup = 0;
   int ncw = 8;
   int bf3 = 0;
+  int chain = 0;
   dim3 grid;
   size_t lds_bytes;
   double flops;
@@ -1444,6 +1451,28 @@
   return R;
 }
 
+inline bool conv_chain_instance_exists(int ci, int ct, int pt, int ch) { return ci == 16 && (ct == 1 || ct == 2) && (pt == 1 || pt == 2) && ch == 2; }
+inline bool conv_chain_attach(ConvLaunch &p, const ConvLaunch &c, const ConvLayer &LC) {
+  const ConvArgs &pa = p.args, &ca = c.args;
+  const int ch = ca.ctTot;
+  if (p.async != 4 || p.chain || p.bf3 || p.fz || pa.ctTot != p.ct || p.grid.z != 1 || !conv_chain_instance_exists(p.ci, p.ct, p.pt, ch)) return false;
+  if (pa.par_rows || pa.rows_valid != 16 * p.ct || pa.outC != pa.rows_valid || pa.sx != 1 || pa.omx != 1 || pa.omz != 1 || pa.outH != 2 * pa.nPH || pa.outW != pa.nPW) return false;
+  if (LC.kd != 1 || LC.kh != 1 || LC.kw != 1 || LC.sd != 1 || LC.sh != 1 || LC.sw != 1 || LC.transposed || LC.up2 || LC.relu || LC.Cin != pa.outC || LC.Cout != 16 * ch) return false;
+  if (c.bf3 || c.fz || c.chain || (c.async != 0 && c.async != 1) || c.ci != 16 || ca.class_loop || c.grid.y != 1) return false;
+  if (ca.in != pa.out || ca.inC != pa.outC || ca.pass_stride != 16 || ca.npass != p.ct || ca.inD != pa.outD || ca.inH != pa.outH || ca.inW != pa.outW) return false;
+  if (ca.par_rows || ca.rows_valid != 16 * ch || ca.outC != 16 * ch || ca.omx != 1 || ca.omy != 1 || ca.omz != 1 || ca.nPD != pa.outD || ca.nPH != pa.outH || ca.nPW != pa.outW) return false;
+  if (ca.add_mode != 0 && ca.add_mode != 2) return false;
+  ConvArgs &a = p.args;
+  a.ch_w = ca.wpk;
+  a.ch_scale = ca.scale; a.ch_bias = ca.bias; a.ch_add = ca.add; a.ch_out = ca.out;
+  a.ch_outH = ca.outH; a.ch_outW = ca.outW; a.ch_outC = ca.outC;
+  a.ch_add_mode = ca.add_mode; a.ch_addH = ca.addH; a.ch_addW = ca.addW;
+  a.ch_split = c.ct * c.pt == 1 ? 1 : 0;
+  p.chain = ch;
+  p.flops += c.flops;
+  return true;
+}
+
 inline void conv_allow_big_lds(const void *fn, std::atomic<unsigned long long> &done, size_t lds_bytes) {
   if (lds_bytes <= 64 * 1024) return;
   int dev = 0;
@@ -1479,11 +1508,11 @@
   conv_allow_big_lds(reinterpret_cast<const void *>(&k_conv_a<CI, CT, PT>), done, c.lds_bytes);
   hipLaunchKernelGGL((k_conv_a<CI, CT, PT>), c.grid, dim3(kConvAThreads), c.lds_bytes, st, c.args);
 }
-template <int CI, int CT, int PT>
+template <int CI, int CT, int PT, int CH = 0>
 inline void launch_conv_w_inst(const ConvLaunch &c, hipStream_t st) {
   static std::atomic<unsigned long long> done{0};
-  conv_allow_big_lds(reinterpret_cast<const void *>(&k_conv_w<CI, CT, PT>), done, c.lds_bytes);
-  hipLaunchKernelGGL((k_conv_w<CI, CT, PT>), c.grid, dim3(kConvThreads), c.lds_bytes, st, c.args);
+  conv_allow_big_lds(reinterpret_cast<const void *>(&k_conv_w<CI, CT, PT, CH>), done, c.lds_bytes);
+  hipLaunchKernelGGL((k_conv_w<CI, CT, PT, CH>), c.grid, dim3(kConvThreads), c.lds_bytes, st, c.args);
 }
 template <int CI, int NUP, int CT, int PT, int FZ = 0, int NCW = 8, int W = 0>
 inline void launch_conv_m_inst(const ConvLaunch &c, hipStream_t st) {
@@ -1536,6 +1565,12 @@
 #undef DR_X
     fail(DR_ERR_ARG, "launch_conv: no marching instance CI=%d NUP=%d CT=%d PT=%d waves=%d", c.ci, c.nup, c.ct, c.pt, c.ncw);
   }
+  if (c.chain) {
+#define DR_CONV_W_CASE(CT_, PT_) if (c.async == 4 && c.ci == 16 && c.ct == CT_ && c.pt == PT_ && c.chain == 2) { launch_conv_w_inst<16, CT_, PT_, 2>(c, st); return; }
+    DR_CONV_W_CASE(1, 1) DR_CONV_W_CASE(1, 2) DR_CONV_W_CASE(2, 1) DR_CONV_W_CASE(2, 2)
+#undef DR_CONV_W_CASE
+    fail(DR_ERR_ARG, "launch_conv: no chained instance kind=%d CI=%d CT=%d PT=%d CH=%d", c.async, c.ci, c.ct, c.pt, c.chain);
+  }
   if (c.async == 4) {
 #define DR_CONV_W_CASE(CI_, CT_, PT_) if (c.ci == CI_ && c.ct == CT_ && c.pt == PT_) { launch_conv_w_inst<CI_, CT_, PT_>(c, st); return; }
     DR_CONV_W_CASE(16, 1, 1) DR_CONV_W_CASE(16, 1, 2) DR_CONV_W_CASE(16, 2, 1) DR_CONV_W_CASE(16, 2, 2)
diff --git a/tandem_amd/csrc/conv_wino.h b/tandem_amd/csrc/conv_wino.h
--- a/tandem_amd/csrc/conv_wino.h
+++ b/tandem_amd/csrc/conv_wino.h
@@ -118,7 +118,114 @@
   }
 }
 
-template <int CI, int CT, int PT>
+__host__ __device__ inline size_t conv_chain_w_index(int ct, int cc, int CH, int lane) { return ((size_t)ct * CH + cc) * 64 + lane; }
+__host__ __device__ inline size_t conv_chain_out_index(const ConvArgs &a, int oz, int oy, int ox, int ch) {
+  return (((size_t)oz * a.ch_outH + oy) * a.ch_outW + ox) * a.ch_outC + ch;
+}
+__host__ __device__ inline size_t conv_chain_add_index(const ConvArgs &a, int oz, int oy, int ox, int ch) {
+  return (((size_t)oz * a.ch_addH + (oy >> 1)) * a.ch_addW + (ox >> 1)) * a.ch_outC + ch;
+}
+template <int CT, int PT, int CH>
+__device__ inline void conv_w_epilogue_chain(const ConvArgs &a, const ConvClass &cls, floatx4 (&acc)[4][CT][PT], const float4 (&scv)[CT], const float4 (&biv)[CT],
+                                             int wave, int lane, int pz0, int py0, int px0) {
+  const int j = lane & 15, g = lane >> 4;
+  float4 cw[CT][CH], csc[CH], cbi[CH];
+#pragma unroll
+  for (int ct = 0; ct < CT; ++ct)
+#pragma unroll
+    for (int cc = 0; cc < CH; ++cc) cw[ct][cc] = a.ch_w[conv_chain_w_index(ct, cc, CH, lane)];
+#pragma unroll
+  for (int cc = 0; cc < CH; ++cc) {
+    csc[cc] = *reinterpret_cast<const float4 *>(a.ch_scale + cc * 16 + 4 * g);
+    cbi[cc] = *reinterpret_cast<const float4 *>(a.ch_bias + cc * 16 + 4 * g);
+  }
+#pragma unroll
+  for (int pt = 0; pt < PT; ++pt) {
+    const int tau = wave * PT + pt;
+    const int xt = tau % a.TXT, yt = (tau / a.TXT) % a.TY, zt = tau / (a.TXT * a.TY);
+    const int qz = pz0 + zt, qy = py0 + yt, qx = px0 + xt * 16 + j;
+    const bool ok = qz < a.nPD && qy < a.nPH && qx < a.nPW;
+    const int oz = qz * a.omz + cls.ooz, ox = qx * a.omx + cls.oox;
+    size_t obase[2][CT];
+    float4 ad[2][CT], cad[CH];
+#pragma unroll
+    for (int r = 0; r < 2; ++r)
+#pragma unroll
+      for (int ct = 0; ct < CT; ++ct) {
+        const int oy = qy * 2 + r, c0 = ct * 16 + 4 * g;
+        obase[r][ct] = (((size_t)oz * a.outH + oy) * a.outW + ox) * a.outC + c0;
+        size_t abase = obase[r][ct];
+        if (a.add_mode == 2) abase = (((size_t)oz * a.addH + (oy >> 1)) * a.addW + (ox >> 1)) * a.outC + c0;
+        ad[r][ct] = make_float4(0.f, 0.f, 0.f, 0.f);
+        if (a.add_mode && ok) ad[r][ct] = *reinterpret_cast<const float4 *>(a.add + abase);
+      }
+#pragma unroll
+    for (int cc = 0; cc < CH; ++cc) {
+      cad[cc] = make_float4(0.f, 0.f, 0.f, 0.f);
+      if (a.ch_add_mode == 2 && ok) cad[cc] = *reinterpret_cast<const float4 *>(a.ch_add + conv_chain_add_index(a, oz, qy * 2, ox, cc * 16 + 4 * g));
+    }
+    float4 v[2][CT];
+#pragma unroll
+    for (int ct = 0; ct < CT; ++ct) {
+      const floatx4 m0 = acc[0][ct][pt], m1 = acc[1][ct][pt], m2 = acc[2][ct][pt], m3 = acc[3][ct][pt];
+      const floatx4 o[2] = {(m0 + m1) + m2, (m1 - m2) - m3};
+      const float4 sc = scv[ct], bi = biv[ct];
+#pragma unroll
+      for (int r = 0; r < 2; ++r) {
+        float4 w;
+        w.x = o[r][0] * sc.x + bi.x;
+        w.y = o[r][1] * sc.y + bi.y;
+        w.z = o[r][2] * sc.z + bi.z;
+        w.w = o[r][3] * sc.w + bi.w;
+        if (a.relu) { w.x = fmaxf(w.x, 0.f); w.y = fmaxf(w.y, 0.f); w.z = fmaxf(w.z, 0.f); w.w = fmaxf(w.w, 0.f); }
+        if (a.add_mode) { w.x += ad[r][ct].x; w.y += ad[r][ct].y; w.z += ad[r][ct].z; w.w += ad[r][ct].w; }
+        if (ok) *reinterpret_cast<float4 *>(a.out + obase[r][ct]) = w;
+        v[r][ct] = w;
+      }
+    }
+    floatx4 c[2][CH];
+#pragma unroll
+    for (int r = 0; r < 2; ++r)
+#pragma unroll
+      for (int cc = 0; cc < CH; ++cc) c[r][cc] = floatx4{0.f, 0.f, 0.f, 0.f};
+#define DR_CH_STEP(S, ACC)                                                                              \
+  _Pragma("unroll") for (int r = 0; r < 2; ++r) _Pragma("unroll") for (int cc = 0; cc < CH; ++cc)       \
+      ACC[r][cc] = __builtin_amdgcn_mfma_f32_16x16x4f32(cw[ct][cc].S, v[r][ct].S, ACC[r][cc], 0, 0, 0);
+    if (a.ch_split) {
+#pragma unroll
+      for (int ct = 0; ct < CT; ++ct) {
+        floatx4 c2[2][CH];
+#pragma unroll
+        for (int r = 0; r < 2; ++r)
+#pragma unroll
+          for (int cc = 0; cc < CH; ++cc) c2[r][cc] = floatx4{0.f, 0.f, 0.f, 0.f};
+        DR_CH_STEP(x, c) DR_CH_STEP(y, c2) DR_CH_STEP(z, c) DR_CH_STEP(w, c2)
+#pragma unroll
+        for (int r = 0; r < 2; ++r)
+#pragma unroll
+          for (int cc = 0; cc < CH; ++cc) c[r][cc] += c2[r][cc];
+      }
+    } else {
+#pragma unroll
+      for (int ct = 0; ct < CT; ++ct) { DR_CH_STEP(x, c) DR_CH_STEP(y, c) DR_CH_STEP(z, c) DR_CH_STEP(w, c) }
+    }
+#undef DR_CH_STEP
+#pragma unroll
+    for (int r = 0; r < 2; ++r)
+#pragma unroll
+      for (int cc = 0; cc < CH; ++cc) {
+        float4 w;
+        w.x = __builtin_fmaf(c[r][cc][0], csc[cc].x, cbi[cc].x);
+        w.y = __builtin_fmaf(c[r][cc][1], csc[cc].y, cbi[cc].y);
+        w.z = __builtin_fmaf(c[r][cc][2], csc[cc].z, cbi[cc].z);
+        w.w = __builtin_fmaf(c[r][cc][3], csc[cc].w, cbi[cc].w);
+        if (a.ch_add_mode) { w.x += cad[cc].x; w.y += cad[cc].y; w.z += cad[cc].z; w.w += cad[cc].w; }
+        if (ok) *reinterpret_cast<float4 *>(a.ch_out + conv_chain_out_index(a, oz, qy * 2 + r, ox, cc * 16 + 4 * g)) = w;
+      }
+  }
+}
+
+template <int CI, int CT, int PT, int CH = 0>
 __global__ __launch_bounds__(kConvThreads, (CT * PT == 1 ? 4 : (CT * PT == 2 ? 3 : 2))) void k_conv_w(const ConvArgs a) {
   extern __shared__ float4 lds4[];
   float *lds = reinterpret_cast<float *>(lds4);
@@ -194,7 +301,8 @@
   }
   float4 scv[CT], biv[CT];
   conv_load_affine<CT>(a, g, ct0, scv, biv);
-  conv_w_epilogue<CT, PT>(a, cls, acc, scv, biv, wave, j, g, ct0, pz0, py0, px0);
-}
-
-}
+  if constexpr (CH > 0) conv_w_epilogue_chain<CT, PT, CH>(a, cls, acc, scv, biv, wave, lane, pz0, py0, px0);
+  else conv_w_epilogue<CT, PT>(a, cls, acc, scv, biv, wave, j, g, ct0, pz0, py0, px0);
+}
+
+}
diff --git a/tandem_amd/csrc/dr_mvsnet.hip b/tandem_amd/csrc/dr_mvsnet.hip
--- a/tandem_amd/csrc/dr_mvsnet.hip
+++ b/tandem_amd/csrc/dr_mvsnet.hip
@@ -115,6 +115,7 @@
   FrontArgs front{};
   Head3Args head3{};
   std::function<ConvLaunch(int)> replan;
+  ConvLayer layer;
   std::string sig;
   int ncand = 0;
   int stage = 0, shift = 0, bits = 0;
@@ -200,6 +201,7 @@
   bool prob_launch_order = hon("DR_PROB_LAUNCH_ORDER"), prob_on_conv = hon("DR_PROB_ON_CONV");
   bool skip_on_conv = hon("DR_SKIP_ON_CONV"), no_skip_fusion = hon("DR_NO_SKIP_FUSION");
   bool out3_folded = hnum("DR_OUT3_FOLDED", 1) != 0;
+  bool neck_chain = !hon("DR_NO_NECK_CHAIN");
   bool d2h_copy = hook_env("DR_MVS_D2H") && !strcmp(hook_env("DR_MVS_D2H"), "copy");
   int cv5_rows = hnum("DR_CV5_ROWS", 0);
   bool cv5_reuse = hnum("DR_CV5_REUSE", 1) != 0;
@@ -547,7 +549,7 @@
       const Op &o = ops_[i];
       char kn[64] = "misc";
       if (o.kind == Op::CONV && o.conv.async == 2) snprintf(kn, sizeof kn, "k_conv_m<%d,%d,%d,%d,%d,%d,%d>", o.conv.ci, o.conv.nup, o.conv.ct, o.conv.pt, o.conv.fz, o.conv.ncw, o.conv.march.wino);
-      else if (o.kind == Op::CONV && o.conv.async == 4) snprintf(kn, sizeof kn, "k_conv_w<%d,%d,%d>", o.conv.ci, o.conv.ct, o.conv.pt);
+      else if (o.kind == Op::CONV && o.conv.async == 4) snprintf(kn, sizeof kn, "k_conv_w<%d,%d,%d,%d>", o.conv.ci, o.conv.ct, o.conv.pt, o.conv.chain);
       else if (o.kind == Op::CONV && o.conv.async) snprintf(kn, sizeof kn, "k_conv_a<%d,%d,%d>", o.conv.ci, o.conv.ct, o.conv.pt);
       else if (o.kind == Op::CONV && o.conv.bf3) snprintf(kn, sizeof kn, "k_conv_b<%d,%d,%d>", o.conv.ci, o.conv.ct, o.conv.pt);
       else if (o.kind == Op::CONV && o.conv.args.class_loop > 0) snprintf(kn, sizeof kn, "k_conv_c<%d,%d,%d>", o.conv.ci, o.conv.ct, o.conv.pt);
@@ -748,6 +750,7 @@
       Op o; o.kind = Op::CONV; o.conv = cl; o.name = opname + (P.launches.size() > 1 ? "." + std::to_string(idx) : "");
       if (P.launches.size() == 1) {
         o.replan = replan; o.ncand = ncand;
+        o.layer = L; o.layer.weight = nullptr;
         char sig[160];
         snprintf(sig, sizeof sig, "%d, %d, %d, %d, %d, %d, %d, %d, %d, %d, %d, %d, %d", L.Cin, L.Cout, k3d, kh, kw, L.sd, L.sh, L.sw, L.transposed ? 1 : (L.up2 ? 1 + L.up2 : 0),
                  (int)mode + (fused ? 8 : 0) + (iS ? 16 : 0), iD, iH, iW);
@@ -824,6 +827,32 @@
     }
     H_ = H; W_ = W; V_ = V;
   }
+  void chain_neck(size_t prod) {
+    if (!sw_.neck_chain || ops_.size() != prod + 2) return;
+    Op &p = ops_[prod];
+    const Op c = ops_.back();
+    if (p.kind != Op::CONV || c.kind != Op::CONV || !p.replan || !c.replan) return;
+    const std::string merged = p.name + "+" + c.name;
+    if (fn_batch_) {
+      const Op *b = nullptr;
+      for (const Op &o : *fn_batch_) if (o.name == merged) b = &o;
+      if (!b) return;
+      for (int r = 0; r < p.ncand && !same_kernel(p.conv, b->conv); ++r) {
+        const ConvLaunch k = p.replan(r);
+        if (same_kernel(k, b->conv)) p.conv = k;
+      }
+    }
+    ConvLaunch k = p.conv;
+    if (!conv_chain_attach(k, c.conv, c.layer)) return;
+    const std::function<ConvLaunch(int)> inner = p.replan;
+    const ConvLaunch head = c.conv;
+    const ConvLayer LC = c.layer;
+    p.replan = [inner, head, LC, k](int rank) { ConvLaunch n = inner(rank); return conv_chain_attach(n, head, LC) ? n : k; };
+    p.conv = k; p.name = merged;
+    p.flops += c.flops;
+    p.bytes += c.bytes - 4.0 * (double)k.args.outD * k.args.outH * k.args.outW * k.args.outC;
+    ops_.pop_back();
+  }
   void build_featurenet(int V, int H, int W) {
     const std::string fn = "feature_net.";
     DevTensor &c3 = front_block(fn, V, H, W);
@@ -834,7 +863,9 @@
     DevTensor &c1b = cbr2("fn.conv2.1", fn + "conv2.1", c1a, 3, 1, CONV_NORMAL);
     DevTensor &c1 = cbr2("fn.conv2.2", fn + "conv2.2", c1b, 3, 1, CONV_NORMAL);
     const int fpad = sw_.costvol_v1 ? 0 : 1;
+    const size_t neck1 = ops_.size() - 1;
     add_conv("fn.out1", fn + "out.stage1", "", false, false, c1, "feat1", 1, 1, 1, 1, 1, 1, false, CONV_NORMAL, nullptr, 0, nullptr, fpad);
+    chain_neck(neck1);
     fork_lo_ = ops_.size();
     DevTensor &i2 = add_skip("fn.skip2", fn + "skip.stage2", c2, "inter2", c1);
     add_conv("fn.out2", fn + "out.stage2", "", false, false, i2, "feat2", 1, 3, 3, 1, 1, 1, false, CONV_NORMAL, nullptr, 0, nullptr, fpad);
@@ -897,9 +928,12 @@
     fork_hi_ = ops_.size();
   }
 
-  struct FnOut { size_t op; int stage; size_t offset; };
+  struct FnOut { size_t op; int stage; size_t offset; bool chained; };
   struct FcEntry { uint64_t key[2] = {0, 0}; float *feat[3] = {nullptr, nullptr, nullptr}; uint8_t *bgr = nullptr; uint64_t used = 0; bool valid = false; };
   static bool same_instance(const ConvLaunch &a, const ConvLaunch &b) {
+    return same_kernel(a, b) && a.chain == b.chain;
+  }
+  static bool same_kernel(const ConvLaunch &a, const ConvLaunch &b) {
     return a.async == b.async && a.ci == b.ci && a.ct == b.ct && a.pt == b.pt && a.fz == b.fz && a.bf3 == b.bf3 && a.nup == b.nup && a.ncw == b.ncw &&
            a.march.wino == b.march.wino && a.march.rm == b.march.rm;
   }
@@ -910,7 +944,9 @@
     std::vector<Op> batch;
     batch.swap(ops_);
     tprefix_ = "c1.";
-    try { build_featurenet(1, H, W); } catch (...) { tprefix_.clear(); ops_.swap(batch); fork_lo_ = lo; fork_hi_ = hi; feat2_op_ = f2; throw; }
+    fn_batch_ = &batch;
+    try { build_featurenet(1, H, W); } catch (...) { fn_batch_ = nullptr; tprefix_.clear(); ops_.swap(batch); fork_lo_ = lo; fork_hi_ = hi; feat2_op_ = f2; throw; }
+    fn_batch_ = nullptr;
     tprefix_.clear();
     ops1_.swap(ops_); ops_.swap(batch);
     fork_lo_ = lo; fork_hi_ = hi; feat2_op_ = f2;
@@ -930,11 +966,12 @@
     fn1_out_.clear();
     for (size_t i = 0; i < ops1_.size(); ++i) {
       Op &o = ops1_[i];
-      float *out = o.kind == Op::CONV ? o.conv.args.out : (o.kind == Op::HEAD3 ? o.head3.out : nullptr);
-      for (int s = 0; s < 3 && out; ++s) {
-        const DevTensor &t = T("c1.feat" + std::to_string(s + 1));
-        if (out >= t.d && out < t.d + t.n()) fn1_out_.push_back({i, s, (size_t)(out - t.d)});
-      }
+      float *outs[2] = {o.kind == Op::CONV ? o.conv.args.out : (o.kind == Op::HEAD3 ? o.head3.out : nullptr), o.kind == Op::CONV && o.conv.chain ? o.conv.args.ch_out : nullptr};
+      for (int w = 0; w < 2; ++w)
+        for (int s = 0; s < 3 && outs[w]; ++s) {
+          const DevTensor &t = T("c1.feat" + std::to_string(s + 1));
+          if (outs[w] >= t.d && outs[w] < t.d + t.n()) fn1_out_.push_back({i, s, (size_t)(outs[w] - t.d), w == 1});
+        }
     }
     if (fn1_out_.size() != 3) { ops1_.clear(); fcache_.clear(); return; }
     fn1_ok_ = true;
@@ -1039,7 +1076,7 @@
       FcEntry &e = fcache_[fc_slot_[fc_miss_]];
       for (const FnOut &p : fn1_out_) {
         Op &o = ops1_[p.op];
-        (o.kind == Op::CONV ? o.conv.args.out : o.head3.out) = e.feat[p.stage] + p.offset;
+        (o.kind == Op::CONV ? (p.chained ? o.conv.args.ch_out : o.conv.args.out) : o.head3.out) = e.feat[p.stage] + p.offset;
       }
       for (Op &o : ops1_) {
         if (o.kind == Op::FRONT) o.front.bgr = d_bgr_ + fc_miss_ * img_bytes;
@@ -1591,6 +1628,7 @@
   hipEvent_t ev_fork_ = nullptr, ev_feat2_ = nullptr, ev_feat3_ = nullptr;
   bool side_enabled_ = true;
   size_t fork_lo_ = 0, fork_hi_ = 0, feat2_op_ = 0;
+  const std::vector<Op> *fn_batch_ = nullptr;
   int fcache_cap_ = 0;
   std::vector<FcEntry> fcache_;
   std::vector<Op> ops1_;
@@ -1802,6 +1840,48 @@
     }
     DR_HIP(hipMemcpy(out, d_out, on * 4, hipMemcpyDeviceToHost));
     if (out_dims) { out_dims[0] = oD; out_dims[1] = oH; out_dims[2] = oW; }
+  });
+}
+
+int drm_debug_conv_chain(int device, const float *in, int D, int H, int W, int Cin, const float *weight, int Cout, const float *scale, const float *bias, int relu,
+                         const float *weight1, int Cout1, const float *scale1, const float *bias1, const float *add_up2, int out_pad, float *out, float *out1,
+                         int *chained) {
+  return guarded([&] {
+    using namespace dr;
+    int n = 0;
+    if (hipGetDeviceCount(&n) != hipSuccess || n <= device) fail(DR_ERR_DEVICE, "no HIP device %d", device);
+    if (!in || !weight || !weight1 || !out || !out1 || out_pad < 0 || (add_up2 && ((H | W) & 1))) fail(DR_ERR_ARG, "drm_debug_conv_chain: bad argument");
+    DR_HIP(hipSetDevice(device));
+    DeviceArena arena;
+    arena.err_flag = arena.upload(std::vector<int>(1, 0));
+    ConvLayer L, L1;
+    L.Cin = Cin; L.Cout = Cout; L.kd = 1; L.kh = 3; L.kw = 3; L.weight = weight; L.relu = relu != 0;
+    if (scale) L.scale.assign(scale, scale + Cout);
+    if (bias) L.bias.assign(bias, bias + Cout);
+    L1.Cin = Cout; L1.Cout = Cout1; L1.weight = weight1; L1.out_pad = out_pad;
+    if (scale1) L1.scale.assign(scale1, scale1 + Cout1);
+    if (bias1) L1.bias.assign(bias1, bias1 + Cout1);
+    float *d_in = arena.upload(std::vector<float>(in, in + (size_t)D * H * W * Cin));
+    const size_t on = (size_t)D * H * W * Cout, Hp = H + 2 * out_pad, Wp = W + 2 * out_pad, on1 = (size_t)D * Hp * Wp * Cout1;
+    float *d_out = arena.upload(std::vector<float>(on, 0.f));
+    float *d_out1 = arena.upload(std::vector<float>(on1, -12345.f));
+    float *d_add = add_up2 ? arena.upload(std::vector<float>(add_up2, add_up2 + (size_t)D * (H / 2) * (W / 2) * Cout1)) : nullptr;
+    const char *rk = getenv("DR_CONV_RANK");
+    ConvLaunch p = plan_conv(L, CONV_NORMAL, d_in, D, H, W, Cin, d_out, nullptr, 0, arena, rk ? atoi(rk) : 0).launches.at(0);
+    const ConvLaunch c = plan_conv(L1, CONV_NORMAL, d_out, D, H, W, Cout, d_out1 + ((size_t)out_pad * Wp + out_pad) * Cout1, d_add, 2, arena, 0).launches.at(0);
+    const bool ch = !hook_env("DR_NO_NECK_CHAIN") && conv_chain_attach(p, c, L1);
+    launch_conv(p, nullptr);
+    if (!ch) launch_conv(c, nullptr);
+    DR_HIP(hipDeviceSynchronize());
+    DR_HIP(hipGetLastError());
+    int march_err = 0;
+    DR_HIP(hipMemcpy(&march_err, arena.err_flag, sizeof(int), hipMemcpyDeviceToHost));
+    if (march_err) fail(DR_ERR_DEVICE, "k_conv_m: a ring wait gave up (code %d)", march_err);
+    if (getenv("DR_CONV_PRINT"))
+      fprintf(stderr, "debug_conv_chain: %s<%d,%d,%d> %s, head %s<%d,%d,%d>\n", conv_kind_name(p), p.ci, p.ct, p.pt, ch ? "chained" : "two launches", conv_kind_name(c), c.ci, c.ct, c.pt);
+    DR_HIP(hipMemcpy(out, d_out, on * 4, hipMemcpyDeviceToHost));
+    DR_HIP(hipMemcpy(out1, d_out1, on1 * 4, hipMemcpyDeviceToHost));
+    if (chained) *chained = ch ? 1 : 0;
   });
 }
 
diff --git a/tandem_amd/dr_mvsnet.py b/tandem_amd/dr_mvsnet.py
--- a/tandem_amd/dr_mvsnet.py
+++ b/tandem_amd/dr_mvsnet.py
@@ -246,6 +246,22 @@
     return out
 
 
+def debug_conv_chain(x, weight, weight1, scale=None, bias=None, relu=False, scale1=None, bias1=None, add_up2=None, out_pad=0, device=0):
+    c = lambda a: None if a is None else np.ascontiguousarray(a, np.float32)
+    x, w, w1, scale, bias, scale1, bias1, add_up2 = (c(a) for a in (x, weight, weight1, scale, bias, scale1, bias1, add_up2))
+    D, H, W, Cin = x.shape
+    Cout, Cout1 = w.shape[0], w1.shape[0]
+    assert w.shape == (Cout, Cin, 1, 3, 3) and w1.shape == (Cout1, Cout, 1, 1, 1)
+    assert add_up2 is None or add_up2.shape == (D, H // 2, W // 2, Cout1)
+    out = np.empty((D, H, W, Cout), np.float32)
+    out1 = np.empty((D, H + 2 * out_pad, W + 2 * out_pad, Cout1), np.float32)
+    chained = C.c_int()
+    p = lambda a: None if a is None else fptr(a)
+    check(_lib.lib().drm_debug_conv_chain(device, fptr(x), D, H, W, Cin, fptr(w), Cout, p(scale), p(bias), int(relu), fptr(w1), Cout1, p(scale1), p(bias1),
+                                          p(add_up2), int(out_pad), fptr(out), fptr(out1), C.byref(chained)))
+    return out, out1, bool(chained.value)
+
+
 def debug_tail(x, skip, w_deconv, scale, bias, w_prob, qy=0, zchunk=0, form=1, device=0):
     x, skip = np.ascontiguousarray(x, np.float32), np.ascontiguousarray(skip, np.float32)
     D, h, w, _ = skip.shape
```

After: 591.8 depth-maps/s, median of 6. No clear change (+0.2%).
